# fgnt/pb_chime5

Measured on AMD Instinct MI355X. Metric: utterance-seconds enhanced/sec/GPU (24ch, 20 EM iters), higher is better.
Workload: dtype f64

## Files before the change

### pb_chime5_amd/csrc/cacgmm.hip

```cpp
#include <algorithm>
#include <cmath>
#include <cstdlib>

#include "gss_internal.h"
#include "dense_wave.h"
#include "jacobi.h"

namespace {

#ifndef GSS_CHOL_PRIO
#define GSS_CHOL_PRIO 1
#endif
#ifndef GSS_ESTEP_PRIO
#define GSS_ESTEP_PRIO 1
#endif
constexpr int EM_TILE = 64;
constexpr int EM_TS = EM_TILE + 1;

enum { MODE_FIRST = 0, MODE_EM = 1, MODE_PREDICT = 2 };

__device__ __forceinline__ void set_progress_priority(int done, int total) {
    const int q4 = 4 * done / total;
    if (q4 <= 0) __builtin_amdgcn_s_setprio(3);
    else if (q4 == 1) __builtin_amdgcn_s_setprio(2);
    else if (q4 == 2) __builtin_amdgcn_s_setprio(1);
    else __builtin_amdgcn_s_setprio(0);
}

struct MsegPlan {
    int S, ntile, base, rem, maxseg;
};
__host__ __device__ __forceinline__ int mseg_begin(const MsegPlan &p, int slot) {
    return slot * p.base + (slot < p.rem ? slot : p.rem);
}
__host__ __device__ __forceinline__ int mseg_slot_of(const MsegPlan &p, int item) {
    const int head = p.rem * (p.base + 1);
    return item < head ? item / (p.base + 1) : p.rem + (item - head) / p.base;
}
__host__ __device__ __forceinline__ int mseg_count(const MsegPlan &p, int f) {
    return mseg_slot_of(p, f * p.ntile + p.ntile - 1) - mseg_slot_of(p, f * p.ntile) + 1;
}

struct EmArgs {
    const cplx *Y;
    const uint8_t *act;
    int64_t act_stride, act_fstride;
    const double *init;
    int64_t init_stride, init_fstride;
    const double *logdet;
    const double *pi;
    double *W;
    cplx *Bp;
    double *Sg;
    double *gamma;
    int64_t T;
    int F, D, NE, nch, chunk_frames;
    int masked;
    double aff_eps;
    MsegPlan mseg;
};

template <bool NORMALISE, int NV = 8>
__device__ __forceinline__ void load_tile(const cplx *Yf, int D, int64_t t0, int64_t c1, int tl,
                                          int g, cplx *ys, double *scratch) {
    const int tid = g * EM_TILE + tl;
    const int nfr = (int)min((int64_t)EM_TILE, c1 - t0);
    const int total = nfr * D;
    const cplx *src = Yf + t0 * D;
    const int qf = 256 / D, rf = 256 - qf * D;
    cplx v[NV];
#pragma unroll
    for (int j = 0; j < NV; ++j) {
        const int idx = tid + 256 * j;
        v[j] = idx < total ? src[idx] : c_make(0.0, 0.0);
    }
    {
        int fr = tid / D, d = tid - fr * D;
#pragma unroll
        for (int j = 0; j < NV; ++j) {
            if (tid + 256 * j < EM_TILE * D) ys[d * EM_TS + fr] = v[j];
            fr += qf;
            d += rf;
            if (d >= D) {
                d -= D;
                ++fr;
            }
        }
    }
    if (NORMALISE) {
        __syncthreads();
        double nrm = 0.0;
#pragma unroll
        for (int j = 0; j < NV; ++j) {
            const int d = g + 4 * j;
            nrm += d < D ? c_abs2(ys[d * EM_TS + tl]) : 0.0;
        }
        scratch[g * EM_TILE + tl] = nrm;
        __syncthreads();
        nrm = scratch[tl] + scratch[EM_TILE + tl] + scratch[2 * EM_TILE + tl] +
              scratch[3 * EM_TILE + tl];
        nrm = sqrt(nrm);
        if (nrm < GSS_TINY) nrm = GSS_TINY;
#pragma unroll
        for (int j = 0; j < NV; ++j) {
            const int d = g + 4 * j;
            if (d < D) {
                const cplx y = ys[d * EM_TS + tl];
                ys[d * EM_TS + tl] = c_make(y.x / nrm, y.y / nrm);
            }
        }
    }
}

template <int K, int MODE>
__global__ __launch_bounds__(256) void em_estep_kernel(EmArgs a, const cplx *__restrict__ Mq) {
    extern __shared__ __attribute__((aligned(16))) char smem[];
    const int D = a.D, NE = a.NE;
    cplx *ys = reinterpret_cast<cplx *>(smem);
    double *qpart = reinterpret_cast<double *>(ys + D * EM_TS);
    double *lpS = qpart + 4 * K * EM_TILE;
    double *qqS = lpS + K * EM_TILE;
    double *ldet = qqS + K * EM_TILE;
    double *pis = ldet + K;
    double *vvS = qpart;

    int f, chunk;
    if (!xcd_group_map(a.nch, a.F, f, chunk)) return;
    const int tid = threadIdx.x;
    const int tl = tid & 63;
    const int g = __builtin_amdgcn_readfirstlane(tid >> 6);
    const int64_t T = a.T;
    const int64_t c0 = (int64_t)chunk * a.chunk_frames;
    const int64_t c1 = c0 + a.chunk_frames < T ? c0 + a.chunk_frames : T;
    const cplx *Yf = a.Y + (int64_t)f * T * D;
    const cplx *Mf = Mq + (int64_t)f * NE * K;
    const uint8_t *actf = a.act + (int64_t)f * a.act_fstride;

    if (MODE != MODE_FIRST && tid < K) {
        ldet[tid] = a.logdet[f * K + tid];
        pis[tid] = a.pi[f * K + tid];
    }
    constexpr int NS = (K + 3) / 4;
    double sg[NS];
#pragma unroll
    for (int s = 0; s < NS; ++s) sg[s] = 0.0;

    for (int64_t t0 = c0; t0 < c1; t0 += EM_TILE) {
        const int64_t t = t0 + tl;
        const bool valid = t < c1;
        if (MODE == MODE_FIRST) {
            if (a.init != nullptr) {
                const double *initf = a.init + (int64_t)f * a.init_fstride;
#pragma unroll
                for (int s = 0; s < NS; ++s) {
                    const int k = g + 4 * s;
                    if (k < K && valid) {
                        const double gk = initf[(int64_t)k * a.init_stride + t];
                        sg[s] += gk;
                        a.W[((int64_t)f * K + k) * T + t] = gk;
                    }
                }
                continue;
            }
            double ssum = 0.0;
#pragma unroll
            for (int k = 0; k < K; ++k)
                ssum += (valid && actf[(int64_t)k * a.act_stride + t]) ? 1.0 : 1e-10;
#pragma unroll
            for (int s = 0; s < NS; ++s) {
                const int k = g + 4 * s;
                if (k < K && valid) {
                    const double v = actf[(int64_t)k * a.act_stride + t] ? 1.0 : 1e-10;
                    const double gk = v / ssum;
                    sg[s] += gk;
                    a.W[((int64_t)f * K + k) * T + t] = gk;
                }
            }
            continue;
        }
        __syncthreads();
        load_tile<true>(Yf, D, t0, c1, tl, g, ys, qpart);
        __syncthreads();

        double q[K];
#pragma unroll
        for (int k = 0; k < K; ++k) q[k] = 0.0;
        const int npairs = (D + 1) / 2;
        for (int p = g; p < npairs; p += 4) {
#pragma unroll 1
            for (int side = 0; side < 2; ++side) {
                const int r = side == 0 ? p : D - 1 - p;
                if (side == 1 && r == p) break;
                const cplx y1 = ys[r * EM_TS + tl];
                const cplx *mrow = Mf + (int64_t)tri_index(r, r, D) * K;
                {
                    const double pr = y1.x * y1.x + y1.y * y1.y;
#pragma unroll
                    for (int k = 0; k < K; ++k) q[k] = fma(mrow[k].x, pr, q[k]);
                }
                for (int d2 = r + 1; d2 < D; ++d2) {
                    mrow += K;
                    const cplx y2 = ys[d2 * EM_TS + tl];
                    const double pr = y1.x * y2.x + y1.y * y2.y;
                    const double pim = y1.y * y2.x - y1.x * y2.y;
#pragma unroll
                    for (int k = 0; k < K; ++k) {
                        const cplx m = mrow[k];
                        q[k] = fma(m.x, pr, q[k]);
                        q[k] = fma(m.y, pim, q[k]);
                    }
                }
            }
        }
#pragma unroll
        for (int k = 0; k < K; ++k) qpart[(g * K + k) * EM_TILE + tl] = q[k];
        __syncthreads();
        double myq[NS];
#pragma unroll
        for (int s = 0; s < NS; ++s) myq[s] = 1.0;
#pragma unroll
        for (int s = 0; s < NS; ++s) {
            const int k = g + 4 * s;
            if (k < K) {
                double qv = qpart[k * EM_TILE + tl] + qpart[(K + k) * EM_TILE + tl] +
                            qpart[(2 * K + k) * EM_TILE + tl] + qpart[(3 * K + k) * EM_TILE + tl];
                qv = fmax(fabs(qv), GSS_TINY);
                myq[s] = qv;
                lpS[k * EM_TILE + tl] = -(double)D * log(qv) - ldet[k];
            }
        }
        __syncthreads();
        double mx = -INFINITY;
#pragma unroll
        for (int k = 0; k < K; ++k) mx = fmax(mx, lpS[k * EM_TILE + tl]);
#pragma unroll
        for (int s = 0; s < NS; ++s) {
            const int k = g + 4 * s;
            if (k < K) {
                double v = exp(lpS[k * EM_TILE + tl] - mx) * pis[k];
                if (a.masked) v *= (valid && actf[(int64_t)k * a.act_stride + t]) ? 1.0 : 0.0;
                vvS[k * EM_TILE + tl] = v;
            }
        }
        __syncthreads();
        double ssum = 0.0;
#pragma unroll
        for (int k = 0; k < K; ++k) ssum += vvS[k * EM_TILE + tl];
        ssum = fmax(ssum, GSS_TINY);
#pragma unroll
        for (int s = 0; s < NS; ++s) {
            const int k = g + 4 * s;
            if (k < K && valid) {
                double gam = vvS[k * EM_TILE + tl] / ssum;
                if (a.aff_eps != 0.0) gam = fmin(fmax(gam, a.aff_eps), 1.0 - a.aff_eps);
                if (MODE == MODE_PREDICT) {
                    a.gamma[((int64_t)f * K + k) * T + t] = gam;
                } else {
                    sg[s] += gam;
                    a.W[((int64_t)f * K + k) * T + t] = gam / fmax(myq[s], 10.0 * GSS_TINY);
                }
            }
        }
    }
    if (MODE == MODE_PREDICT) return;
#pragma unroll
    for (int s = 0; s < NS; ++s) {
        const int k = g + 4 * s;
        const double tot = wave_sum(sg[s]);
        if (k < K && tl == 0) a.Sg[((int64_t)f * a.nch + chunk) * K + k] = tot;
    }
}

template <int NV>
__global__ __launch_bounds__(256) void em_prepare_kernel(const cplx *__restrict__ Y, int F,
                                                         int64_t T, int D,
                                                         cplx *__restrict__ Yn,
                                                         int *__restrict__ zero_tiles) {
    extern __shared__ __attribute__((aligned(16))) char smem[];
    cplx *ys = reinterpret_cast<cplx *>(smem);
    double *scratch = reinterpret_cast<double *>(ys + D * EM_TS);
    int f, tile;
    const int ntile = (int)((T + EM_TILE - 1) / EM_TILE);
    if (!xcd_group_map(ntile, F, f, tile)) return;
    const int tid = threadIdx.x, tl = tid & 63, g = tid >> 6;
    const int64_t t0 = (int64_t)tile * EM_TILE;
    load_tile<true, NV>(Y + (int64_t)f * T * D, D, t0, T, tl, g, ys, scratch);
    __syncthreads();
    const int64_t t = t0 + tl;
    bool nonzero = false;
    if (t < T)
        for (int d = g; d < D; d += 4) {
            const cplx v = ys[d * EM_TS + tl];
            Yn[((int64_t)f * D + d) * T + t] = v;
            nonzero = nonzero || v.x != 0.0 || v.y != 0.0;
        }
    scratch[g * EM_TILE + tl] = nonzero ? 1.0 : 0.0;
    __syncthreads();
    const bool zero_frame = t < T && g == 0 &&
                            scratch[tl] + scratch[EM_TILE + tl] + scratch[2 * EM_TILE + tl] +
                                    scratch[3 * EM_TILE + tl] == 0.0;
    const int any_zero = __syncthreads_or(zero_frame ? 1 : 0);
    if (tid == 0) zero_tiles[(int64_t)f * ntile + tile] = any_zero;
}

__device__ __forceinline__ bool frequency_has_zero_frames(const int *__restrict__ zero_tiles,
                                                          int ntile, int f, int lane) {
    int z = 0;
    for (int i = lane; i < ntile; i += 64) z |= zero_tiles[(int64_t)f * ntile + i];
    return __any(z != 0);
}

template <int K, int D, int MODE>
__global__ __launch_bounds__(256) void em_estep_reg_kernel(EmArgs a, const cplx *__restrict__ Mq,
                                                           const cplx *__restrict__ Yn) {
    constexpr int NE = D * (D + 1) / 2;
    const int64_t T = a.T;
    const int wpb = blockDim.x >> 6;
    const int ntile = (int)((T + 64 * wpb - 1) / (64 * wpb));
    int f, tile;
    if (!xcd_group_map(ntile, a.F, f, tile)) return;
    const int lane = threadIdx.x & 63;
    const int wave = __builtin_amdgcn_readfirstlane(threadIdx.x >> 6);
    const int64_t t = ((int64_t)tile * wpb + wave) * 64 + lane;
    const bool valid = t < T;
    const int64_t tc = valid ? t : T - 1;
    const cplx *Mf = Mq + (int64_t)f * NE * K;
    const cplx *yf = Yn + (int64_t)f * D * T + tc;

#if GSS_ESTEP_PRIO
    __builtin_amdgcn_s_setprio(3);
#endif
    cplx y[D];
#pragma unroll
    for (int d = 0; d < D; ++d) y[d] = yf[(int64_t)d * T];

    double q[K];
#pragma unroll
    for (int k = 0; k < K; ++k) q[k] = 0.0;
    constexpr int P = 2, RING = P + 1;
    cplx ring[RING][K];
#pragma unroll
    for (int j = 0; j < P; ++j)
#pragma unroll
        for (int k = 0; k < K; ++k) ring[j][k] = Mf[j * K + k];
    int e = 0;
#pragma unroll
    for (int d1 = 0; d1 < D; ++d1) {
#pragma unroll
        for (int d2 = d1; d2 < D; ++d2) {
            if (e + P < NE) {
#pragma unroll
                for (int k = 0; k < K; ++k) ring[(e + P) % RING][k] = Mf[(e + P) * K + k];
            }
            const double pr = y[d1].x * y[d2].x + y[d1].y * y[d2].y;
            if (d1 == d2) {
#pragma unroll
                for (int k = 0; k < K; ++k) q[k] = fma(ring[e % RING][k].x, pr, q[k]);
            } else {
                const double pim = y[d1].y * y[d2].x - y[d1].x * y[d2].y;
#pragma unroll
                for (int k = 0; k < K; ++k) {
                    const cplx m = ring[e % RING][k];
                    q[k] = fma(m.x, pr, q[k]);
                    q[k] = fma(m.y, pim, q[k]);
                }
            }
            __builtin_amdgcn_sched_barrier(0);
            ++e;
#if GSS_ESTEP_PRIO
            if (e == NE / 4) __builtin_amdgcn_s_setprio(2);
            if (e == NE / 2) __builtin_amdgcn_s_setprio(1);
            if (e == 3 * NE / 4) __builtin_amdgcn_s_setprio(0);
#endif
        }
    }
    const int dep = q[0] != q[0] ? 1 : 0;
    const int tcl = (int)tc - dep;
    auto lane_bcast = [](double x, int k) {
        const unsigned long long u = __double_as_longlong(x);
        const unsigned lo = __builtin_amdgcn_readlane((int)(unsigned)u, k);
        const unsigned hi = __builtin_amdgcn_readlane((int)(unsigned)(u >> 32), k);
        return __longlong_as_double(((unsigned long long)hi << 32) | lo);
    };
    double cls, ldl, pil;
    {
        const int kk = (lane < K ? lane : K - 1) - (lane > 0 ? dep : 0);
        ldl = a.logdet[f * K + kk];
        pil = a.pi[f * K + kk];
        double ldmin = INFINITY;
#pragma unroll
        for (int k = 0; k < K; ++k) ldmin = fmin(ldmin, lane_bcast(ldl, k));
        cls = pil * exp(ldmin - ldl);
    }
    double qmin = INFINITY;
#pragma unroll
    for (int k = 0; k < K; ++k) {
        q[k] = fmax(fabs(q[k]), GSS_TINY);
        qmin = fmin(qmin, q[k]);
    }
    uint8_t act[K];
#pragma unroll
    for (int k = 0; k < K; ++k)
        act[k] = a.act[(int64_t)f * a.act_fstride + (int64_t)k * a.act_stride + (tcl < 0 ? 0 : tcl)];
    double v[K], iq[K], ssum = 0.0;
#pragma unroll
    for (int k = 0; k < K; ++k) {
        iq[k] = 1.0 / q[k];
        const double r = qmin * iq[k];
        double p = 1.0, b = r;
#pragma unroll
        for (int bit = D; bit > 0; bit >>= 1) {
            if (bit & 1) p = p * b;
            b = b * b;
        }
        v[k] = p * lane_bcast(cls, k);
        v[k] = (!a.masked || (valid && act[k])) ? v[k] : 0.0;
        ssum += v[k];
    }
    if (ssum < 1e-280) {
        double lp[K], mx = -INFINITY;
        ssum = 0.0;
#pragma unroll
        for (int k = 0; k < K; ++k) {
            lp[k] = -(double)D * log(q[k]) - lane_bcast(ldl, k);
            mx = fmax(mx, lp[k]);
        }
#pragma unroll
        for (int k = 0; k < K; ++k) {
            v[k] = exp(lp[k] - mx) * lane_bcast(pil, k);
            v[k] = (!a.masked || (valid && act[k])) ? v[k] : 0.0;
            ssum += v[k];
        }
    }
    const double is = 1.0 / fmax(ssum, GSS_TINY);
#pragma unroll
    for (int k = 0; k < K; ++k) {
        double gam = v[k] * is;
        if (a.aff_eps != 0.0) gam = fmin(fmax(gam, a.aff_eps), 1.0 - a.aff_eps);
        if (MODE == MODE_PREDICT) {
            if (valid) a.gamma[((int64_t)f * K + k) * T + t] = gam;
        } else {
            if (valid)
                a.W[((int64_t)f * K + k) * T + t] =
                    gam * (q[k] < 10.0 * GSS_TINY ? 1.0 / (10.0 * GSS_TINY) : iq[k]);
            const double tot = wave_sum(valid ? gam : 0.0);
            if (lane == 0) a.Sg[(((int64_t)f * ntile + tile) * wpb + wave) * K + k] = tot;
        }
    }
}

struct WcovLds {
    int Dp, nblk, nfg, red_groups;
    size_t ys, wk, scratch, blk, total;
};

__host__ __device__ inline WcovLds wcov_lds_layout(int D, int KW) {
    WcovLds L;
    L.Dp = D + (D & 1);
    const int nb2 = L.Dp / 2;
    L.nblk = nb2 * (nb2 + 1) / 2;
    int nfg = 256 / L.nblk;
    if (nfg > EM_TILE) nfg = EM_TILE;
    if (nfg < 1) nfg = 1;
    L.nfg = nfg;
    size_t off = 0;
    const size_t ys_bytes = sizeof(cplx) * (size_t)L.Dp * EM_TS;
    const size_t group_bytes = sizeof(cplx) * (size_t)L.nblk * 4 * KW;
    int rg = (int)((32 * 1024) / group_bytes);
    if (rg > nfg - 1) rg = nfg - 1;
    if (rg < 1) rg = 1;
    L.red_groups = rg;
    const size_t red_bytes = group_bytes * rg;
    L.ys = off;
    off += ys_bytes > red_bytes ? ys_bytes : red_bytes;
    L.wk = off;      off += sizeof(double) * KW * EM_TILE;
    L.scratch = off; off += sizeof(double) * 4 * EM_TILE;
    L.blk = off;     off += 2 * (size_t)L.nblk;
    L.total = (off + 15) / 16 * 16;
    return L;
}

#ifdef GSS_WCOV_TRACE
__device__ long long g_wcov_phase[8192 * 6];
extern "C" int gss_debug_wcov_phase(long long *host, int entries) {
    return (int)hipMemcpyFromSymbol(host, HIP_SYMBOL(g_wcov_phase), sizeof(long long) * 6 * entries);
}
#define WCOV_T(var) const long long var = __builtin_readcyclecounter()
#else
#define WCOV_T(var)
#endif

template <int KW, bool NORMALISE, bool SRC_FDT, bool PREFETCH = false, int YP = 8, bool YEXACT = false>
__global__ __launch_bounds__(256) void wcov_kernel(const cplx *__restrict__ Y,
                                                   const double *__restrict__ W, int F,
                                                   int64_t T, int D, int NE, int nch,
                                                   int chunk_frames, cplx *__restrict__ part,
                                                   int Ktot, int k0, MsegPlan plan) {
    extern __shared__ __attribute__((aligned(16))) char smem[];
    const WcovLds L = wcov_lds_layout(D, KW);
    const int Dp = L.Dp;
    cplx *ys = reinterpret_cast<cplx *>(smem + L.ys);
    double *wk = reinterpret_cast<double *>(smem + L.wk);
    double *scratch = reinterpret_cast<double *>(smem + L.scratch);
    unsigned char *blk = reinterpret_cast<unsigned char *>(smem + L.blk);

    int f = 0, chunk = 0, item = 0, item_end = 1;
    if (plan.S > 0) {
        item = mseg_begin(plan, blockIdx.x);
        item_end = mseg_begin(plan, blockIdx.x + 1);
    }
    const int item_begin = item;
    if (plan.S > 0) {
    } else if (!xcd_group_map(nch, F, f, chunk)) {
        return;
    }
    W += (int64_t)blockIdx.y * F * Ktot * T;
    part += (int64_t)blockIdx.y * F * nch * Ktot * NE;
    const int tid = threadIdx.x;
    const int tl = tid & 63, g = tid >> 6;
#ifdef GSS_WCOV_TRACE
    long long tr_stage = 0, tr_acc = 0;
    const long long tr_wall0 = __builtin_amdgcn_s_memrealtime();
#endif
    WCOV_T(tr_c0);
#ifdef GSS_WCOV_TRACE
    long long tr_red = 0;
#endif

    {
        const int nb2 = Dp / 2;
        for (int bi = tid; bi < nb2; bi += blockDim.x) {
            int idx = bi * nb2 - (bi * (bi - 1)) / 2;
            for (int bj = bi; bj < nb2; ++bj, ++idx) {
                blk[2 * idx] = (unsigned char)bi;
                blk[2 * idx + 1] = (unsigned char)bj;
            }
        }
    }
    const int mb = tid % L.nblk, fg = tid / L.nblk;
    const bool m_active = fg < L.nfg;
  for (bool first_seg = true; item < item_end; first_seg = false) {
    if (Dp != D) {
        if (!first_seg) __syncthreads();
        for (int j = tid; j < EM_TS; j += blockDim.x) ys[D * EM_TS + j] = c_make(0.0, 0.0);
    }
    int64_t c0, c1;
    int nch_f = nch;
    if (plan.S > 0) {
        f = item / plan.ntile;
        const int tile0 = item - f * plan.ntile;
        const int ntl = min(plan.ntile - tile0, item_end - item);
        c0 = (int64_t)tile0 * EM_TILE;
        c1 = min(T, (int64_t)(tile0 + ntl) * EM_TILE);
        chunk = (int)blockIdx.x - mseg_slot_of(plan, f * plan.ntile);
        nch_f = plan.maxseg;
        item += ntl;
    } else {
        c0 = (int64_t)chunk * chunk_frames;
        c1 = c0 + chunk_frames < T ? c0 + chunk_frames : T;
        item = item_end;
    }
    const cplx *Yf = Y + (int64_t)f * T * D;
    const double *Wf = W + ((int64_t)f * Ktot + k0) * T;
    cplx acc[4][KW];
#pragma unroll
    for (int s = 0; s < 4; ++s)
#pragma unroll
        for (int k = 0; k < KW; ++k) acc[s][k] = c_make(0.0, 0.0);

    constexpr int WPRE = (KW * EM_TILE + 255) / 256;
    cplx ypre[YP];
    double wpre[WPRE];
    auto prefetch = [&](int64_t t0) {
        const cplx *src = Y + (int64_t)f * D * T;
#pragma unroll
        for (int j = 0; j < YP; ++j) {
            const int d = g + 4 * j;
            ypre[j] = ((YEXACT || d < D) && t0 + tl < c1) ? src[(int64_t)d * T + t0 + tl] : c_make(0.0, 0.0);
        }
#pragma unroll
        for (int j = 0; j < WPRE; ++j) {
            const int idx = tid + 256 * j;
            const int k = idx / EM_TILE, jj = idx - k * EM_TILE;
            wpre[j] = (idx < KW * EM_TILE && t0 + jj < c1) ? Wf[(int64_t)k * T + t0 + jj] : 0.0;
        }
    };
    if (SRC_FDT && PREFETCH) prefetch(c0);
    for (int64_t t0 = c0; t0 < c1; t0 += EM_TILE) {
        WCOV_T(tr_a);
        if (plan.S > 0) {
            set_progress_priority(item - (int)((c1 - t0 + EM_TILE - 1) / EM_TILE) - item_begin,
                                  item_end - item_begin);
        }
        __syncthreads();
        if (SRC_FDT) {
            if (!PREFETCH) prefetch(t0);
#pragma unroll
            for (int j = 0; j < YP; ++j) {
                const int d = g + 4 * j;
                if (YEXACT || d < D) ys[d * EM_TS + tl] = ypre[j];
            }
#pragma unroll
            for (int j = 0; j < WPRE; ++j) {
                const int idx = tid + 256 * j;
                if (idx < KW * EM_TILE) wk[idx] = wpre[j];
            }
            __syncthreads();
            if (PREFETCH && t0 + EM_TILE < c1) prefetch(t0 + EM_TILE);
        } else {
            load_tile<NORMALISE, YP>(Yf, D, t0, c1, tl, g, ys, scratch);
            for (int idx = tid; idx < KW * EM_TILE; idx += blockDim.x) {
                const int k = idx / EM_TILE, j = idx - k * EM_TILE;
                wk[idx] = t0 + j < c1 ? Wf[(int64_t)k * T + t0 + j] : 0.0;
            }
            __syncthreads();
        }
        WCOV_T(tr_b);
        if (m_active) {
            const int nfr = (int)min((int64_t)EM_TILE, c1 - t0);
            const int bi = blk[2 * mb], bj = blk[2 * mb + 1];
            const cplx *ra0 = ys + (2 * bi) * EM_TS, *ra1 = ra0 + EM_TS;
            const cplx *rb0 = ys + (2 * bj) * EM_TS, *rb1 = rb0 + EM_TS;
            for (int j = fg; j < nfr; j += L.nfg) {
                const cplx a0 = ra0[j], a1 = ra1[j], b0 = rb0[j], b1 = rb1[j];
                double pr[4], pim[4];
                pr[0] = a0.x * b0.x + a0.y * b0.y;  pim[0] = a0.y * b0.x - a0.x * b0.y;
                pr[1] = a0.x * b1.x + a0.y * b1.y;  pim[1] = a0.y * b1.x - a0.x * b1.y;
                pr[2] = a1.x * b0.x + a1.y * b0.y;  pim[2] = a1.y * b0.x - a1.x * b0.y;
                pr[3] = a1.x * b1.x + a1.y * b1.y;  pim[3] = a1.y * b1.x - a1.x * b1.y;
#pragma unroll
                for (int k = 0; k < KW; ++k) {
                    const double w = wk[k * EM_TILE + j];
#pragma unroll
                    for (int s = 0; s < 4; ++s) {
                        acc[s][k].x = fma(w, pr[s], acc[s][k].x);
                        acc[s][k].y = fma(w, pim[s], acc[s][k].y);
                    }
                }
            }
        }
#ifdef GSS_WCOV_TRACE
        {
            WCOV_T(tr_c);
            tr_stage += tr_b - tr_a;
            tr_acc += tr_c - tr_b;
        }
#endif
    }
    WCOV_T(tr_c1);
    cplx *red = reinterpret_cast<cplx *>(smem + L.ys);
    const int gstride = L.nblk * 4 * KW;
    for (int r0 = 1; r0 < L.nfg; r0 += L.red_groups) {
        __syncthreads();
        if (m_active && fg >= r0 && fg < r0 + L.red_groups) {
            cplx *dst = red + (size_t)(fg - r0) * gstride;
#pragma unroll
            for (int s = 0; s < 4; ++s)
#pragma unroll
                for (int k = 0; k < KW; ++k) dst[(mb * 4 + s) * KW + k] = acc[s][k];
        }
        __syncthreads();
        if (fg == 0) {
            for (int r = r0; r < r0 + L.red_groups && r < L.nfg; ++r) {
                const cplx *src = red + (size_t)(r - r0) * gstride;
#pragma unroll
                for (int s = 0; s < 4; ++s)
#pragma unroll
                    for (int k = 0; k < KW; ++k)
                        acc[s][k] = c_add(acc[s][k], src[(mb * 4 + s) * KW + k]);
            }
        }
    }
    if (fg == 0) {
        cplx *pp = part + (((int64_t)f * nch_f + chunk) * Ktot + k0) * NE;
        const int bi = blk[2 * mb], bj = blk[2 * mb + 1];
#pragma unroll
        for (int s = 0; s < 4; ++s) {
            const int d1 = 2 * bi + (s >> 1), d2 = 2 * bj + (s & 1);
            if (d1 <= d2 && d2 < D) {
                const int e = tri_index(d1, d2, D);
#pragma unroll
                for (int k = 0; k < KW; ++k) pp[k * NE + e] = acc[s][k];
            }
        }
    }
#ifdef GSS_WCOV_TRACE
    {
        WCOV_T(tr_c2s);
        tr_red += tr_c2s - tr_c1;
    }
#endif
  }
#ifdef GSS_WCOV_TRACE
    {
        WCOV_T(tr_c2);
        if (tid == 0 && blockIdx.x < 8192) {
            long long *o = g_wcov_phase + 6 * blockIdx.x;
            o[0] = tr_wall0;
            o[1] = __builtin_amdgcn_s_memrealtime();
            o[2] = tr_stage;
            o[3] = tr_acc;
            o[4] = tr_red;
            o[5] = tr_c2 - tr_c0;
        }
    }
#endif
}

template <int K, int D>
__global__ __launch_bounds__(64) void mstep_reg_kernel(const cplx *__restrict__ Yn,
                                                       const double *__restrict__ W, int F,
                                                       int64_t T, int nch, int chunk_frames,
                                                       cplx *__restrict__ part) {
    constexpr int NE = D * (D + 1) / 2;
    int f, chunk;
    if (!xcd_group_map(nch, F, f, chunk)) return;
    const int lane = threadIdx.x;
    const int64_t c0 = (int64_t)chunk * chunk_frames;
    const int64_t c1 = c0 + chunk_frames < T ? c0 + chunk_frames : T;
    const cplx *yf = Yn + (int64_t)f * D * T;
    const double *wf = W + (int64_t)f * K * T;

    double are[K][NE], aim[K][NE];
#pragma unroll
    for (int k = 0; k < K; ++k)
#pragma unroll
        for (int e = 0; e < NE; ++e) are[k][e] = aim[k][e] = 0.0;

    cplx y[D], yn[D];
    double w[K], wn[K];
    auto fetch = [&](int64_t t, cplx (&yy)[D], double (&ww)[K]) {
        const bool ok = t < c1;
        const int64_t tc = ok ? t : c1 - 1;
#pragma unroll
        for (int d = 0; d < D; ++d) yy[d] = yf[(int64_t)d * T + tc];
#pragma unroll
        for (int k = 0; k < K; ++k) ww[k] = ok ? wf[(int64_t)k * T + tc] : 0.0;
    };
    fetch(c0 + lane, yn, wn);
    for (int64_t tb = c0; tb < c1; tb += 64) {
#pragma unroll
        for (int d = 0; d < D; ++d) y[d] = yn[d];
#pragma unroll
        for (int k = 0; k < K; ++k) w[k] = wn[k];
        if (tb + 64 < c1) fetch(tb + 64 + lane, yn, wn);
        int e = 0;
#pragma unroll
        for (int d1 = 0; d1 < D; ++d1) {
#pragma unroll
            for (int d2 = d1; d2 < D; ++d2, ++e) {
                const double pr = y[d1].x * y[d2].x + y[d1].y * y[d2].y;
#pragma unroll
                for (int k = 0; k < K; ++k) are[k][e] = fma(w[k], pr, are[k][e]);
                if (d2 != d1) {
                    const double pim = y[d1].y * y[d2].x - y[d1].x * y[d2].y;
#pragma unroll
                    for (int k = 0; k < K; ++k) aim[k][e] = fma(w[k], pim, aim[k][e]);
                }
            }
        }
    }
// ... 679 lines not shown
                }
            }
#ifdef GSS_EM4_TRACE
            {
                EM4_T(c_e);
                EM4_ADD(0, c_b - c_a);
                EM4_ADD(2, c_d - c_b);
                EM4_ADD(3, c_e - c_d);
            }
#endif
        }
        if (predict) break;
        EM4_T(c_f);

#pragma unroll
        for (int k = 0; k < K; ++k) {
            const double tot = quad_sum(acc[k]);
            if (msl == 0) (&ldsS[wave][0][0])[k * NP + mi] = tot;
            const double g = wave_sum(sg[k]);
            if (lane == 0) sgS[wave][k] = g;
        }
        __syncthreads();
        static_assert(K * NP <= 2 * OC_LD, "the wave sums fit the first rows");
        if (tid < K * NP) {
            const int k = tid / NP;
            const double sgk = (sgS[0][k] + sgS[1][k]) + (sgS[2][k] + sgS[3][k]);
            const double tot = ((&ldsS[0][0][0])[tid] + (&ldsS[1][0][0])[tid]) +
                               ((&ldsS[2][0][0])[tid] + (&ldsS[3][0][0])[tid]);
            bS[k][tid % NP] = ((double)D * tot) / fmax(sgk, GSS_TINY);
        }
        if (tid == 0) flagS = 0;
        __syncthreads();
        EM4_T(c_u0);
        if (wave == 0 && lane < K) {
            const int k = lane;
            const double sgk = (sgS[0][k] + sgS[1][k]) + (sgS[2][k] + sgS[3][k]);
            piS[k] = sgk / (double)T;
            double b[NP], m[NP], ld;
#pragma unroll
            for (int i = 0; i < NP; ++i) b[i] = bS[k][i];
            const bool fast = class_update4_lane(b, a.eig_floor, m, ld) && !force_exact;
            if (fast) {
#pragma unroll
                for (int i = 0; i < NP; ++i) mR[i][k] = m[i];
                logdetS[k] = ld;
            } else {
                atomicOr(&flagS, 1 << k);
            }
        }
#ifdef GSS_EM4_TRACE
        {
            EM4_T(c_u1);
            EM4_ADD(1, c_u1 - c_u0);
        }
#endif
        __syncthreads();
        if (flagS != 0) {
            const int flags = flagS;
            for (int k = wave; k < K; k += 4) {
                if (!(flags >> k & 1)) continue;
                cplx vals[COV_SLOTS];
#pragma unroll
                for (int s2 = 0; s2 < COV_SLOTS; ++s2) vals[s2] = c_make(0.0, 0.0);
                int d1 = 0, d2 = 0;
                if (lane < NE) {
                    const int p = ts.d12[0];
                    d1 = p >> 8, d2 = p & 255;
                    if (d1 == d2) {
                        vals[0] = c_make(bS[k][d1], 0.0);
                    } else {
                        const int off = lane - d1 - 1;
                        vals[0] = c_make(bS[k][D + off], bS[k][D + 6 + off]);
                    }
                }
                cplx *A = reinterpret_cast<cplx *>(&ldsS[wave][0][0]);
                cplx *basis = A + 80;
                cplx *basis_g = a.basis + ((int64_t)f * K + k) * 16;
                if (!a.cold_eigh && basis_validS[k] && lane < 16) basis[lane] = basis_g[lane];
                wave_sync();
                class_update_eigh(vals, D, K, a.eig_floor, A, lane, MqS + k, logdetS + k, ts,
                                  a.cold_eigh ? nullptr : basis, basis_validS + k);
                if (!a.cold_eigh && lane < 16) basis_g[lane] = basis[lane];
                wave_sync();
                if (lane < NE) {
                    const cplx v = MqS[lane * K + k];
                    if (d1 == d2) {
                        mR[d1][k] = v.x;
                    } else {
                        mR[D + lane - d1 - 1][k] = v.x;
                        mR[D + 6 + lane - d1 - 1][k] = v.y;
                    }
                }
            }
            __syncthreads();
        }
        if (tid < K) {
            double ldmin = INFINITY;
            for (int k = 0; k < K; ++k) ldmin = fmin(ldmin, logdetS[k]);
            cS[tid] = piS[tid] * exp(ldmin - logdetS[tid]);
        }
        __syncthreads();
#ifdef GSS_EM4_TRACE
        {
            EM4_T(c_g);
            EM4_ADD(4, c_g - c_f);
        }
#endif
    }
#ifdef GSS_EM4_TRACE
    {
        EM4_T(c_end);
        EM4_ADD(5, c_end - c_start);
        if (tid == 0 && blockIdx.x < 1024)
            for (int i = 0; i < 6; ++i) g_em4_phase[blockIdx.x * 6 + i] = em4_acc[i];
    }
#endif
}

template <int K>
int launch_onchip4(gss_ctx *ctx, const OnchipArgs &a) {
    GSS_PROF(ctx, "em_onchip");
    hipLaunchKernelGGL(em_onchip4_kernel<K>, dim3(a.F), dim3(256), 0, ctx->stream, a);
    GSS_LAUNCH_CHECK(ctx, "em_onchip4_kernel");
    return GSS_OK;
}

size_t em_estep_lds(int D, int K) {
    size_t b = sizeof(cplx) * (size_t)D * EM_TS;
    b += sizeof(double) * ((size_t)4 * K * EM_TILE + 2 * (size_t)K * EM_TILE + 2 * K);
    return (b + 15) / 16 * 16;
}

int em_chunks(int F, int64_t T, int D, int *chunk_frames) {
    int64_t tiles = (T + EM_TILE - 1) / EM_TILE;
    const int forced = gss_variant("em_wgs", 0);
    const int target = forced > 0 ? forced : (D <= 12 ? 1536 : 3072);
    int64_t want = (target + F - 1) / F;
    if (want < 1) want = 1;
    int64_t tiles_per_chunk = (tiles + want - 1) / want;
    if (tiles_per_chunk < 1) tiles_per_chunk = 1;
    *chunk_frames = (int)(tiles_per_chunk * EM_TILE);
    return (int)((tiles + tiles_per_chunk - 1) / tiles_per_chunk);
}

template <typename Kern>
int raise_lds_limit(gss_ctx *ctx, Kern kern, size_t lds) {
    if (lds > 64 * 1024)
        GSS_HIP_CHECK(ctx, hipFuncSetAttribute(reinterpret_cast<const void *>(kern),
                                               hipFuncAttributeMaxDynamicSharedMemorySize,
                                               (int)lds));
    return GSS_OK;
}

template <int K>
int launch_estep(gss_ctx *ctx, int mode, const EmArgs &a, const cplx *Mq, int F) {
    const size_t lds = em_estep_lds(a.D, K);
    dim3 grid(xcd_grid(a.nch, F)), block(256);
    if (mode == MODE_FIRST) {
        GSS_PROF(ctx, "em_estep");
        hipLaunchKernelGGL((em_estep_kernel<K, MODE_FIRST>), grid, block, 0, ctx->stream, a, Mq);
    } else if (mode == MODE_EM) {
        GSS_TRY(raise_lds_limit(ctx, em_estep_kernel<K, MODE_EM>, lds));
        GSS_PROF(ctx, "em_estep");
        hipLaunchKernelGGL((em_estep_kernel<K, MODE_EM>), grid, block, lds, ctx->stream, a, Mq);
    } else {
        GSS_TRY(raise_lds_limit(ctx, em_estep_kernel<K, MODE_PREDICT>, lds));
        GSS_PROF(ctx, "em_predict");
        hipLaunchKernelGGL((em_estep_kernel<K, MODE_PREDICT>), grid, block, lds, ctx->stream, a,
                           Mq);
    }
    GSS_LAUNCH_CHECK(ctx, "em_estep_kernel");
    return GSS_OK;
}

int estep_waves_per_block(int F, int64_t T) {
    auto eff = [&](int wpb) {
        const double wgs = (double)((T + 64 * wpb - 1) / (64 * wpb)) * F;
        const double rounds = wgs / (256.0 * (16 / wpb));
        return rounds / std::ceil(rounds);
    };
    const int forced = gss_variant("estep_wpb", 0);
    if (forced == 1 || forced == 4) return forced;
    return eff(1) > eff(4) ? 1 : 4;
}

template <int K, int D>
int launch_estep_reg(gss_ctx *ctx, int mode, const EmArgs &a, const cplx *Mq, const cplx *Yn,
                     int F) {
    const int wpb = estep_waves_per_block(F, a.T);
    const dim3 grid(xcd_grid((int)((a.T + 64 * wpb - 1) / (64 * wpb)), F)), block(64 * wpb);
    if (mode == MODE_EM) {
        GSS_PROF(ctx, "em_estep");
        hipLaunchKernelGGL((em_estep_reg_kernel<K, D, MODE_EM>), grid, block, 0, ctx->stream, a,
                           Mq, Yn);
    } else {
        GSS_PROF(ctx, "em_predict");
        hipLaunchKernelGGL((em_estep_reg_kernel<K, D, MODE_PREDICT>), grid, block, 0, ctx->stream,
                           a, Mq, Yn);
    }
    GSS_LAUNCH_CHECK(ctx, "em_estep_reg_kernel");
    return GSS_OK;
}

bool estep_reg_supported(int D, int K) {
    return (D == 24 || D == 20 || D == 12 || D == 10 || D == 4) && K >= 2 && K <= 6;
}

template <int D>
int launch_estep_reg_k(gss_ctx *ctx, int K, int mode, const EmArgs &a, const cplx *Mq,
                       const cplx *Yn, int F) {
    switch (K) {
        case 2: return launch_estep_reg<2, D>(ctx, mode, a, Mq, Yn, F);
        case 3: return launch_estep_reg<3, D>(ctx, mode, a, Mq, Yn, F);
        case 4: return launch_estep_reg<4, D>(ctx, mode, a, Mq, Yn, F);
        case 5: return launch_estep_reg<5, D>(ctx, mode, a, Mq, Yn, F);
        case 6: return launch_estep_reg<6, D>(ctx, mode, a, Mq, Yn, F);
    }
    return gss_fail(ctx, GSS_ERR_UNSUPPORTED, "cacgmm: K=%d", K);
}

static int mstep_prefetch_max_d();
using wcov_fn_t = void (*)(const cplx *, const double *, int, int64_t, int, int, int, int, cplx *, int,
                           int, MsegPlan);
template <int KW>
wcov_fn_t mstep_kernel(int D) {
    const bool generic = gss_variant_set("mstep_generic");
    if (D <= mstep_prefetch_max_d()) {
        if (D == 12 && !generic) return wcov_kernel<KW, false, true, true, 3, true>;
        if (D <= 12 && !generic) return wcov_kernel<KW, false, true, true, 3>;
        return wcov_kernel<KW, false, true, true>;
    }
    if (D == 24 && !generic) return wcov_kernel<KW, false, true, false, 6, true>;
    if (D == 20 && !generic) return wcov_kernel<KW, false, true, false, 5, true>;
    return wcov_kernel<KW, false, true>;
}

template <int KW>
int mstep_resident_slots(gss_ctx *ctx, int D, int *slots) {
    const size_t lds = wcov_lds_layout(D, KW).total;
    const void *fn = reinterpret_cast<const void *>(mstep_kernel<KW>(D));
    if (lds > 64 * 1024)
        GSS_HIP_CHECK(ctx, hipFuncSetAttribute(fn, hipFuncAttributeMaxDynamicSharedMemorySize, (int)lds));
    int per_cu = 0, cus = 0;
    GSS_HIP_CHECK(ctx, hipOccupancyMaxActiveBlocksPerMultiprocessor(&per_cu, fn, 256, lds));
    GSS_HIP_CHECK(ctx, hipDeviceGetAttribute(&cus, hipDeviceAttributeMultiprocessorCount, ctx->device));
    *slots = std::max(per_cu, 1) * cus;
    return GSS_OK;
}
static int mstep_prefetch_max_d() {
    const int v = gss_variant("mstep_prefetch_d", 12);
    return v;
}

template <int KW>
int launch_mstep(gss_ctx *ctx, const EmArgs &a, const cplx *Yn, int F, int K, int k0) {
    const size_t lds = wcov_lds_layout(a.D, KW).total;
    GSS_PROF(ctx, "em_mstep");
    if (Yn && a.D == 4 && KW == K && K >= 2 && K <= 6 && !gss_variant_set("mstep_tiled")) {
        hipLaunchKernelGGL((mstep_reg_kernel<(KW >= 2 && KW <= 6 ? KW : 2), 4>),
                           dim3(xcd_grid(a.nch, F)), dim3(64), 0, ctx->stream, Yn, a.W, F, a.T,
                           a.nch, a.chunk_frames, a.Bp);
        GSS_LAUNCH_CHECK(ctx, "mstep_reg_kernel");
        return GSS_OK;
    }
    if (Yn) {
        const wcov_fn_t fn = mstep_kernel<KW>(a.D);
        GSS_TRY(raise_lds_limit(ctx, fn, lds));
        hipLaunchKernelGGL(fn, dim3(a.mseg.S > 0 ? a.mseg.S : xcd_grid(a.nch, F)), dim3(256), lds,
                           ctx->stream, Yn, a.W, F, a.T, a.D, a.NE, a.nch, a.chunk_frames, a.Bp, K, k0,
                           a.mseg);
        GSS_LAUNCH_CHECK(ctx, "wcov_kernel");
        return GSS_OK;
    }
    GSS_TRY(raise_lds_limit(ctx, wcov_kernel<KW, true, false>, lds));
    hipLaunchKernelGGL((wcov_kernel<KW, true, false>), dim3(xcd_grid(a.nch, F)), dim3(256), lds,
                       ctx->stream, a.Y, a.W, F, a.T, a.D, a.NE, a.nch, a.chunk_frames, a.Bp, K, k0,
                       MsegPlan{});
    GSS_LAUNCH_CHECK(ctx, "wcov_kernel");
    return GSS_OK;
}

#define GSS_K_CASE(N, CALL) case N: { constexpr int KK = N; return CALL; }
#define GSS_K_SWITCH8(K, CALL)                                             \
    switch (K) {                                                           \
        GSS_K_CASE(1, CALL) GSS_K_CASE(2, CALL) GSS_K_CASE(3, CALL) GSS_K_CASE(4, CALL)     \
        GSS_K_CASE(5, CALL) GSS_K_CASE(6, CALL) GSS_K_CASE(7, CALL) GSS_K_CASE(8, CALL)     \
    }
#define GSS_K_SWITCH19(K, CALL)                                            \
    switch (K) {                                                           \
        GSS_K_CASE(1, CALL) GSS_K_CASE(2, CALL) GSS_K_CASE(3, CALL) GSS_K_CASE(4, CALL)     \
        GSS_K_CASE(5, CALL) GSS_K_CASE(6, CALL) GSS_K_CASE(7, CALL) GSS_K_CASE(8, CALL)     \
        GSS_K_CASE(9, CALL) GSS_K_CASE(10, CALL) GSS_K_CASE(11, CALL) GSS_K_CASE(12, CALL) \
        GSS_K_CASE(13, CALL) GSS_K_CASE(14, CALL) GSS_K_CASE(15, CALL) GSS_K_CASE(16, CALL) \
        GSS_K_CASE(17, CALL) GSS_K_CASE(18, CALL) GSS_K_CASE(19, CALL)                     \
    }

int launch_estep_k(gss_ctx *ctx, int K, int mode, const EmArgs &a, const cplx *Mq, int F) {
    GSS_K_SWITCH19(K, launch_estep<KK>(ctx, mode, a, Mq, F));
    return gss_fail(ctx, GSS_ERR_UNSUPPORTED, "cacgmm: K=%d", K);
}

int launch_mstep_group(gss_ctx *ctx, int KW, const EmArgs &a, const cplx *Yn, int F, int K,
                       int k0) {
    GSS_K_SWITCH8(KW, launch_mstep<KK>(ctx, a, Yn, F, K, k0));
    return gss_fail(ctx, GSS_ERR_UNSUPPORTED, "cacgmm: class group of %d", KW);
}

int launch_mstep_k(gss_ctx *ctx, int K, const EmArgs &a, const cplx *Yn, int F) {
    const int ngroups = (K + 7) / 8, per = (K + ngroups - 1) / ngroups;
    for (int k0 = 0; k0 < K; k0 += per)
        GSS_TRY(launch_mstep_group(ctx, std::min(per, K - k0), a, Yn, F, K, k0));
    return GSS_OK;
}

int mstep_resident_slots_k(gss_ctx *ctx, int KW, int D, int *slots) {
    GSS_K_SWITCH8(KW, mstep_resident_slots<KK>(ctx, D, slots));
    return gss_fail(ctx, GSS_ERR_UNSUPPORTED, "cacgmm: KW=%d", KW);
}

static int mstep_maxseg_limit() { return std::min(std::max(gss_variant("mstep_maxseg", 8), 1), 32); }

int mstep_plan(gss_ctx *ctx, int F, int64_t T, int D, int K, MsegPlan *plan) {
    *plan = MsegPlan{};
    const int min_d = gss_variant("mstep_plan_min_d", 5);
    if (D < min_d || D <= 4 || gss_variant_set("mstep_chunked")) return GSS_OK;
    const int ngroups = (K + 7) / 8, per = (K + ngroups - 1) / ngroups;
    int slots = 0;
    GSS_TRY(mstep_resident_slots_k(ctx, per, D, &slots));
    if (gss_variant("mstep_slots", 0) > 0) slots = gss_variant("mstep_slots", 0);
    const int64_t ntile = (T + EM_TILE - 1) / EM_TILE, N = ntile * F;
    if (N >= (1LL << 30) || ntile < 1) return GSS_OK;
    plan->ntile = (int)ntile;
    plan->S = (int)std::min<int64_t>(slots, N);
    plan->base = (int)(N / plan->S);
    plan->rem = (int)(N % plan->S);
    for (int f = 0; f < F; ++f) plan->maxseg = std::max(plan->maxseg, mseg_count(*plan, f));
    if (plan->maxseg > mstep_maxseg_limit()) *plan = MsegPlan{};
    return GSS_OK;
}


struct EmBlockPlan {
    int fb, nblocks, streams;
};
EmBlockPlan em_block_plan(int F, int64_t T, int D, int K) {
    EmBlockPlan p{F, 1, 1};
    const double per_f = (16.0 * D + 8.0 * K) * (double)T;
    const double mb = 1024.0 * 1024.0;
    const int fit = gss_variant("em_l3_fit_mb", 230), budget = gss_variant("em_l3_mb", 0);
    if (budget <= 0 || F <= 8 || per_f * F <= fit * mb) return p;
    p.streams = gss_variant("em_streams", 2) >= 2 ? 2 : 1;
    int fb = (int)(budget * mb / p.streams / per_f) / 8 * 8;
    if (fb < 8) fb = 8;
    int nb = (F + fb - 1) / fb;
    if (p.streams == 2 && (nb & 1)) ++nb;
    fb = ((F + nb - 1) / nb + 7) / 8 * 8;
    nb = (F + fb - 1) / fb;
    if (nb <= 1) return EmBlockPlan{F, 1, 1};
    p.fb = fb;
    p.nblocks = nb;
    return p;
}
int em_block_size(const EmBlockPlan &p, int F, int b) { return std::min(p.fb, F - b * p.fb); }

struct EmStrides {
    int nch, bp_nch, reg_nch;
};
EmStrides em_strides(const EmBlockPlan &p, int F, int64_t T, int D) {
    EmStrides s{0, 0, 0};
    for (int b : {0, p.nblocks - 1}) {
        const int Fb = em_block_size(p, F, b);
        int cf;
        const int nch = em_chunks(Fb, T, D, &cf);
        const int wpb = estep_waves_per_block(Fb, T);
        s.nch = std::max(s.nch, nch);
        s.reg_nch = std::max(s.reg_nch, wpb * (int)((T + 64 * wpb - 1) / (64 * wpb)));
    }
    s.bp_nch = std::max(s.nch, mstep_maxseg_limit());
    return s;
}

}

int psd_partials_run(gss_ctx *ctx, const cplx *Y, int F, int64_t T, int D, const double *W2,
                     int nch, int chunk_frames, cplx *part, int S) {
    const size_t lds = wcov_lds_layout(D, 2).total;
    const wcov_fn_t fn = D <= 4 ? wcov_kernel<2, false, false, false, 1>
                         : D <= 12 ? wcov_kernel<2, false, false, false, 3>
                         : D <= 24 ? wcov_kernel<2, false, false, false, 6> : wcov_kernel<2, false, false>;
    GSS_TRY(raise_lds_limit(ctx, fn, lds));
    hipLaunchKernelGGL(fn, dim3(xcd_grid(nch, F), S), dim3(256), lds,
                       ctx->stream, Y, W2, F, T, D, tri_count(D), nch, chunk_frames, part, 2, 0,
                       MsegPlan{});
    GSS_LAUNCH_CHECK(ctx, "wcov_kernel");
    return GSS_OK;
}

size_t cacgmm_workspace_bytes(int F, int64_t T, int D, int K) {
    const size_t NE = tri_count(D);
    const EmBlockPlan bp = em_block_plan(F, T, D, K);
    const EmStrides st = em_strides(bp, F, T, D);
    size_t b = 0;
    b += align_up(sizeof(cplx) * (size_t)F * NE * K);
    b += 2 * align_up(sizeof(double) * (size_t)F * K);
    b += align_up(sizeof(double) * (size_t)F * K * T);
    b += align_up(sizeof(cplx) * (size_t)F * st.bp_nch * K * NE);
    b += align_up(sizeof(double) * (size_t)F * st.nch * K);
    b += align_up(sizeof(int) * (size_t)F * K);
    b += align_up(sizeof(int) * 2 * NE);
    b += align_up(sizeof(cplx) * (size_t)F * D * T);
    b += align_up(sizeof(double) * (size_t)F * st.reg_nch * K);
    b += align_up(sizeof(cplx) * (size_t)F * K * 16);
    b += align_up(sizeof(int) * (size_t)F * ((T + EM_TILE - 1) / EM_TILE));
    return b + 4096;
}

namespace {
struct EmBlock {
    EmArgs a;
    int F;
    cplx *Mq, *Yn;
    int *need_eigh, *zero_tiles;
    double *Sg_lds, *Sg_reg;
    int nch_lds, reg_nch, bp_nch, sg_nch;
    hipStream_t stream;
};
struct StreamRestore {
    gss_ctx *ctx;
    hipStream_t s;
    ~StreamRestore() { ctx->stream = s; }
};
}

int cacgmm_run(gss_ctx *ctx, const cplx *Y, int F, int64_t T, int D, const EmGuide &guide, int K,
               int iterations, int iterations_post, double *gamma) {
    const int NE = tri_count(D);
    const bool reg = estep_reg_supported(D, K) && !gss_variant_set("estep_lds");
    const bool onchip = D == 4 && K >= 2 && K <= 6 && reg && iterations > 0 &&
                        !gss_variant_set("em_unfused");
    const EmBlockPlan bplan = onchip ? EmBlockPlan{F, 1, 1} : em_block_plan(F, T, D, K);
    const EmStrides st = em_strides(bplan, F, T, D);

    cplx *Mq = arena_alloc_t<cplx>(ctx, (size_t)F * NE * K);
    double *logdet = arena_alloc_t<double>(ctx, (size_t)F * K);
    double *pi = arena_alloc_t<double>(ctx, (size_t)F * K);
    double *W = arena_alloc_t<double>(ctx, (size_t)F * K * T);
    cplx *Bp = arena_alloc_t<cplx>(ctx, (size_t)F * st.bp_nch * K * NE);
    double *Sg_lds = arena_alloc_t<double>(ctx, (size_t)F * st.nch * K);
    cplx *Yn = arena_alloc_t<cplx>(ctx, (size_t)F * D * T);
    double *Sg_reg = arena_alloc_t<double>(ctx, (size_t)F * st.reg_nch * K);
    int *need_eigh = arena_alloc_t<int>(ctx, (size_t)F * K);
    const int ntile = (int)((T + EM_TILE - 1) / EM_TILE);
    int *zero_tiles = arena_alloc_t<int>(ctx, (size_t)F * ntile);
    int *tri_tab = arena_alloc_t<int>(ctx, 2 * (size_t)NE);
    GSS_REQUIRE(ctx, Mq && logdet && pi && W && Bp && Sg_lds && Yn && Sg_reg && need_eigh && tri_tab &&
                         zero_tiles,
                GSS_ERR_NOMEM, "cacgmm workspace");
    GSS_REQUIRE(ctx, em_estep_lds(D, K) <= 160 * 1024 &&
                         wcov_lds_layout(D, std::min(K, 8)).total <= 160 * 1024,
                GSS_ERR_UNSUPPORTED, "cacgmm: D=%d K=%d LDS", D, K);
    const bool has_mask = guide.mask != nullptr;
    const uint8_t *const act = has_mask ? guide.mask : reinterpret_cast<const uint8_t *>(Yn);
    const int64_t act_stride = has_mask ? guide.mask_k_stride : 0;
    const int64_t act_fstride = has_mask ? guide.mask_f_stride : 0;
    const int m = D + (D & 1);
    const size_t eigh_lds = (sizeof(cplx) * 2 * m * m + sizeof(double) * m + 15) / 16 * 16;
    const int force_eigh = gss_variant_set("force_eigh");
    if (!onchip) {
        hipLaunchKernelGGL(tri_table_kernel, dim3(1), dim3(256), 0, ctx->stream, D, tri_tab);
        GSS_LAUNCH_CHECK(ctx, "tri_table_kernel");
    }

    auto make_block = [&](int f0, int Fb, hipStream_t stream, EmBlock *blk) -> int {
        EmBlock &b = *blk;
        b = EmBlock{};
        b.F = Fb;
        b.stream = stream;
        EmArgs &a = b.a;
        a.Y = Y + (int64_t)f0 * T * D;
        a.act = act + (int64_t)f0 * act_fstride;
        a.act_stride = act_stride;
        a.act_fstride = act_fstride;
        a.init = guide.init ? guide.init + (int64_t)f0 * guide.init_f_stride : nullptr;
        a.init_stride = guide.init_k_stride;
        a.init_fstride = guide.init_f_stride;
        a.T = T;
        a.F = Fb;
        a.D = D;
        a.NE = NE;
        a.nch = em_chunks(Fb, T, D, &a.chunk_frames);
        GSS_TRY(mstep_plan(ctx, Fb, T, D, K, &a.mseg));
        b.bp_nch = a.mseg.S > 0 ? a.mseg.maxseg : a.nch;
        b.nch_lds = a.nch;
        const int wpb = estep_waves_per_block(Fb, T);
        b.reg_nch = wpb * (int)((T + 64 * wpb - 1) / (64 * wpb));
        GSS_REQUIRE(ctx, b.bp_nch <= st.bp_nch && b.nch_lds <= st.nch && b.reg_nch <= st.reg_nch,
                    GSS_ERR_INVALID, "cacgmm: block strides");
        b.Mq = Mq + (int64_t)f0 * NE * K;
        a.logdet = logdet + (int64_t)f0 * K;
        a.pi = pi + (int64_t)f0 * K;
        a.W = W + (int64_t)f0 * K * T;
        a.Bp = Bp + (int64_t)f0 * st.bp_nch * K * NE;
        b.Sg_lds = Sg_lds + (int64_t)f0 * st.nch * K;
        b.Sg_reg = Sg_reg + (int64_t)f0 * st.reg_nch * K;
        a.Sg = b.Sg_lds;
        a.gamma = gamma + (int64_t)f0 * K * T;
        b.Yn = Yn + (int64_t)f0 * D * T;
        b.need_eigh = need_eigh + (int64_t)f0 * K;
        b.zero_tiles = zero_tiles + (int64_t)f0 * ntile;
        b.sg_nch = b.nch_lds;
        return GSS_OK;
    };
    auto prepare = [&](EmBlock &b) -> int {
        GSS_PROF(ctx, "em_prepare");
        const size_t plds = sizeof(cplx) * (size_t)D * EM_TS + sizeof(double) * 4 * EM_TILE;
        const auto prep = D <= 4 ? em_prepare_kernel<1> : D <= 12 ? em_prepare_kernel<3>
                          : D <= 24 ? em_prepare_kernel<6> : em_prepare_kernel<8>;
        hipLaunchKernelGGL(prep,
                           dim3(xcd_grid((int)((T + EM_TILE - 1) / EM_TILE), b.F)), dim3(256), plds,
                           ctx->stream, b.a.Y, b.F, T, D, b.Yn, b.zero_tiles);
        GSS_LAUNCH_CHECK(ctx, "em_prepare_kernel");
        return GSS_OK;
    };
    auto estep = [&](EmBlock &b, int mode) -> int {
        EmArgs &a = b.a;
        if (reg && mode != MODE_FIRST) {
            a.Sg = b.Sg_reg;
            switch (D) {
                case 24: return launch_estep_reg_k<24>(ctx, K, mode, a, b.Mq, b.Yn, b.F);
                case 20: return launch_estep_reg_k<20>(ctx, K, mode, a, b.Mq, b.Yn, b.F);
                case 12: return launch_estep_reg_k<12>(ctx, K, mode, a, b.Mq, b.Yn, b.F);
                case 10: return launch_estep_reg_k<10>(ctx, K, mode, a, b.Mq, b.Yn, b.F);
                default: return launch_estep_reg_k<4>(ctx, K, mode, a, b.Mq, b.Yn, b.F);
            }
        }
        a.Sg = b.Sg_lds;
        return launch_estep_k(ctx, K, mode, a, b.Mq, b.F);
    };
    auto eig = [&](EmBlock &b) -> int {
        EmArgs &a = b.a;
        {
            GSS_PROF(ctx, "em_chol");
            const int nr = (D + 7) / 8;
            const size_t lds = sizeof(cplx) * (size_t)D * (8 * nr + 1) + sizeof(double) * D;
            auto kern = nr <= 1 ? em_chol_kernel<1> : nr == 2 ? em_chol_kernel<2>
                        : nr == 3 ? em_chol_kernel<3> : em_chol_kernel<4>;
            hipLaunchKernelGGL(kern, dim3(K, b.F), dim3(64), lds, ctx->stream, a.Bp, a.Sg, b.bp_nch,
                               b.sg_nch, D, K, T, 1e-10, force_eigh, b.Mq,
                               const_cast<double *>(a.logdet), const_cast<double *>(a.pi),
                               b.need_eigh, tri_tab, a.mseg, b.zero_tiles, ntile);
            GSS_LAUNCH_CHECK(ctx, "em_chol_kernel");
        }
        {
            GSS_PROF(ctx, "em_eigh");
            hipLaunchKernelGGL(em_eigh_kernel, dim3(K, b.F), dim3(64), eigh_lds, ctx->stream, a.Bp,
                               a.Sg, b.bp_nch, b.sg_nch, D, K, 1e-10, b.need_eigh, b.Mq,
                               const_cast<double *>(a.logdet), tri_tab, a.mseg);
            GSS_LAUNCH_CHECK(ctx, "em_eigh_kernel");
        }
        return GSS_OK;
    };

    if (onchip) {
        EmBlock b;
        GSS_TRY(make_block(0, F, ctx->stream, &b));
        GSS_TRY(prepare(b));
        OnchipArgs o{};
        o.basis = arena_alloc_t<cplx>(ctx, (size_t)F * K * 16);
        GSS_REQUIRE(ctx, o.basis, GSS_ERR_NOMEM, "cacgmm workspace");
        o.Yn = Yn;
        o.act = act;
        o.act_stride = act_stride;
        o.act_fstride = act_fstride;
        o.init = guide.init;
        o.init_stride = guide.init_k_stride;
        o.init_fstride = guide.init_f_stride;
        o.unmasked = has_mask ? 0 : 1;
        o.T = T;
        o.F = F;
        o.iterations = iterations;
        o.iterations_post = iterations_post;
        o.force_eigh = force_eigh;
        o.zero_tiles = b.zero_tiles;
        o.ntile = ntile;
        o.cold_eigh = gss_variant_set("em4_cold_eigh");
        o.eig_floor = 1e-10;
        o.gamma = gamma;
        switch (K) {
            case 2: return launch_onchip4<2>(ctx, o);
            case 3: return launch_onchip4<3>(ctx, o);
            case 4: return launch_onchip4<4>(ctx, o);
            case 5: return launch_onchip4<5>(ctx, o);
            default: return launch_onchip4<6>(ctx, o);
        }
    }

    auto em_iteration = [&](EmBlock &b, bool first) -> int {
        GSS_TRY(estep(b, first ? MODE_FIRST : MODE_EM));
        b.sg_nch = (reg && !first) ? b.reg_nch : b.nch_lds;
        GSS_TRY(launch_mstep_k(ctx, K, b.a, b.Yn, b.F));
        return eig(b);
    };

    hipStream_t const main_stream = ctx->stream;
    StreamRestore restore{ctx, main_stream};
    const int group = bplan.streams;
    if (group > 1) {
        GSS_TRY(aux_stream_ready(ctx));
        GSS_HIP_CHECK(ctx, hipEventRecord(ctx->ev_fork, main_stream));
        GSS_HIP_CHECK(ctx, hipStreamWaitEvent(ctx->aux_stream, ctx->ev_fork, 0));
    }
    for (int b0 = 0; b0 < bplan.nblocks; b0 += group) {
        EmBlock blk[2];
        const int nb = std::min(group, bplan.nblocks - b0);
        for (int j = 0; j < nb; ++j)
            GSS_TRY(make_block((b0 + j) * bplan.fb, em_block_size(bplan, F, b0 + j),
                               j == 0 ? main_stream : ctx->aux_stream, &blk[j]));
        auto each = [&](auto &&fn) -> int {
            for (int j = 0; j < nb; ++j) {
                ctx->stream = blk[j].stream;
                GSS_TRY(fn(blk[j]));
            }
            return GSS_OK;
        };
        GSS_TRY(each([&](EmBlock &b) { return prepare(b); }));
        for (int it = 0; it < iterations; ++it)
            GSS_TRY(each([&](EmBlock &b) {
                b.a.masked = has_mask ? 1 : 0;
                b.a.aff_eps = 1e-10;
                return em_iteration(b, it == 0);
            }));
        for (int it = 0; it < iterations_post - 1; ++it)
            GSS_TRY(each([&](EmBlock &b) {
                b.a.masked = 0;
                b.a.aff_eps = 1e-10;
                return em_iteration(b, false);
            }));
        GSS_TRY(each([&](EmBlock &b) {
            b.a.masked = has_mask && iterations_post == 0 ? 1 : 0;
// ... 12 lines not shown
```

### pb_chime5_amd/csrc/gss_api.hip

```cpp
#include <cmath>
#include <cstdarg>
#include <cstdlib>
#include <cstring>
#include <mutex>

#include "gss_internal.h"

#define GSS_ENTER(ctx)                                   \
    if (!(ctx)) return GSS_ERR_INVALID;                  \
    GSS_HIP_CHECK((ctx), hipSetDevice((ctx)->device))
#define GSS_ENTER_VARIANTS(ctx) \
    GSS_ENTER(ctx);             \
    GSS_TRY(variant_refresh(ctx))
static int variant_refresh(gss_ctx *ctx);

static std::mutex g_error_lock;

int gss_fail(gss_ctx *ctx, int code, const char *fmt, ...) {
    char buf[1024];
    va_list ap;
    va_start(ap, fmt);
    vsnprintf(buf, sizeof(buf), fmt, ap);
    va_end(ap);
    if (ctx) {
        std::lock_guard<std::mutex> guard(g_error_lock);
        ctx->error = buf;
    }
    return code;
}

static thread_local std::string g_create_error;

namespace {
const char *const kVariantKeys[] = {
    "corr_ts", "corr_nw", "corr_blocked", "corr_p_tiles", "chol_diag_unfolded", "apply_ph",
    "apply_generic", "prof_detail", "corr_stg8", "corr_ksplit", "apply_gglobal", "wpe_halves",
    "em_wgs", "estep_wpb", "estep_lds", "mstep_prefetch_d", "mstep_tiled", "mstep_plan_min_d",
    "mstep_chunked", "mstep_slots", "force_eigh", "em_unfused", "em_l3_mb", "em_l3_fit_mb",
    "em_streams", "mstep_maxseg", "em4_cold_eigh", "mstep_generic"};
struct VariantTable {
    std::mutex lock;
    std::string text;
    bool parsed = false;
    std::map<std::string, int> values;
};
VariantTable &variant_table() {
    static VariantTable t;
    return t;
}
}

static int variant_refresh(gss_ctx *ctx) {
    const char *env = getenv("GSS_VARIANT");
    VariantTable &t = variant_table();
    std::lock_guard<std::mutex> guard(t.lock);
    if (t.parsed && t.text == (env ? env : "")) return GSS_OK;
    t.text = env ? env : "";
    t.parsed = true;
    t.values.clear();
    std::string unknown;
    size_t pos = 0;
    while (pos < t.text.size()) {
        size_t end = t.text.find_first_of(", ", pos);
        if (end == std::string::npos) end = t.text.size();
        const std::string tok = t.text.substr(pos, end - pos);
        pos = end + 1;
        if (tok.empty()) continue;
        const size_t eq = tok.find('=');
        const std::string name = tok.substr(0, eq);
        bool known = false;
        for (const char *k : kVariantKeys) known = known || name == k;
        if (!known) {
            unknown = name;
            continue;
        }
        t.values[name] = eq == std::string::npos ? 1 : atoi(tok.c_str() + eq + 1);
    }
    if (!unknown.empty()) {
        t.values.clear();
        t.parsed = false;
        return gss_fail(ctx, GSS_ERR_INVALID, "GSS_VARIANT names no switch '%s'", unknown.c_str());
    }
    return GSS_OK;
}

int gss_variant(const char *key, int dflt) {
    VariantTable &t = variant_table();
    std::lock_guard<std::mutex> guard(t.lock);
    const auto it = t.values.find(key);
    return it == t.values.end() ? dflt : it->second;
}

extern "C" const char *gss_last_error(gss_ctx *ctx) {
    if (!ctx) return g_create_error.c_str();
    static thread_local std::string copy;
    std::lock_guard<std::mutex> guard(g_error_lock);
    copy = ctx->error;
    return copy.c_str();
}

extern "C" const char *gss_version(void) {
#ifdef GSS_EXPERIMENT_BUILD
    return "pb_chime5_amd/libgss_hip 0.4 EXPERIMENT BUILD (gfx950, f64)";
#else
    return "pb_chime5_amd/libgss_hip 0.4 (gfx950, f64)";
#endif
}

extern "C" int gss_abi_version(void) { return GSS_ABI_VERSION; }

extern "C" int gss_device_count(void) {
    int count = 0;
    if (hipGetDeviceCount(&count) != hipSuccess) return 0;
    return count;
}

extern "C" int gss_device_pci_bus_id(int device_id, char *buf, int len) {
    if (!buf || len < 16) return GSS_ERR_INVALID;
    buf[0] = 0;
    int count = 0;
    if (hipGetDeviceCount(&count) != hipSuccess || device_id < 0 || device_id >= count)
        return GSS_ERR_INVALID;
    return hipDeviceGetPCIBusId(buf, len, device_id) == hipSuccess ? GSS_OK : GSS_ERR_HIP;
}

extern "C" int gss_create(int device_id, gss_ctx **out) {
    if (!out) return GSS_ERR_INVALID;
    *out = nullptr;
    int count = 0;
    hipError_t e = hipGetDeviceCount(&count);
    if (e != hipSuccess || count == 0) {
        g_create_error = "no HIP device available: ";
        g_create_error += hipGetErrorString(e);
        return GSS_ERR_HIP;
    }
    if (device_id < 0 || device_id >= count) {
        g_create_error = "device_id out of range";
        return GSS_ERR_INVALID;
    }
    e = hipSetDevice(device_id);
    if (e != hipSuccess) {
        g_create_error = hipGetErrorString(e);
        return GSS_ERR_HIP;
    }
    gss_ctx *ctx = new gss_ctx();
    ctx->device = device_id;
    e = hipStreamCreateWithFlags(&ctx->own_stream, hipStreamNonBlocking);
    if (e != hipSuccess) {
        g_create_error = hipGetErrorString(e);
        delete ctx;
        return GSS_ERR_HIP;
    }
    ctx->stream = ctx->own_stream;
    e = hipHostMalloc(reinterpret_cast<void **>(&ctx->status_host), GSS_STATUS_BYTES,
                      hipHostMallocMapped);
    if (e == hipSuccess)
        e = hipHostGetDevicePointer(reinterpret_cast<void **>(&ctx->status_dev), ctx->status_host, 0);
    if (e != hipSuccess) {
        g_create_error = hipGetErrorString(e);
        (void)hipStreamDestroy(ctx->own_stream);
        delete ctx;
        return GSS_ERR_HIP;
    }
    ctx->status_host[0] = INT32_MIN;
    ctx->status_host[2] = 0;
    *out = ctx;
    return GSS_OK;
}

static void free_tables(gss_ctx *ctx) {
    if (ctx->win_analysis) (void)hipFree(ctx->win_analysis);
    if (ctx->win_synthesis) (void)hipFree(ctx->win_synthesis);
    if (ctx->twiddle) (void)hipFree(ctx->twiddle);
    ctx->win_analysis = ctx->win_synthesis = nullptr;
    ctx->twiddle = nullptr;
}

extern "C" int gss_destroy(gss_ctx *ctx) {
    if (!ctx) return GSS_OK;
    (void)hipSetDevice(ctx->device);
    (void)hipStreamSynchronize(ctx->stream);
    free_tables(ctx);
    if (ctx->arena) (void)hipFree(ctx->arena);
    if (ctx->wpe_tiles) (void)hipFree(ctx->wpe_tiles);
    if (ctx->status_host) (void)hipHostFree(ctx->status_host);
    for (auto &p : ctx->prof_pending) {
        (void)hipEventDestroy(p.start);
        (void)hipEventDestroy(p.stop);
    }
    for (auto ev : ctx->event_pool) (void)hipEventDestroy(ev);
    if (ctx->ev_fork) (void)hipEventDestroy(ctx->ev_fork);
    if (ctx->ev_join) (void)hipEventDestroy(ctx->ev_join);
    if (ctx->aux_stream) {
        (void)hipStreamSynchronize(ctx->aux_stream);
        (void)hipStreamDestroy(ctx->aux_stream);
    }
    if (ctx->own_stream) (void)hipStreamDestroy(ctx->own_stream);
    delete ctx;
    return GSS_OK;
}

int aux_stream_ready(gss_ctx *ctx) {
    if (!ctx->aux_stream)
        GSS_HIP_CHECK(ctx, hipStreamCreateWithFlags(&ctx->aux_stream, hipStreamNonBlocking));
    if (!ctx->ev_fork) GSS_HIP_CHECK(ctx, hipEventCreateWithFlags(&ctx->ev_fork, hipEventDisableTiming));
    if (!ctx->ev_join) GSS_HIP_CHECK(ctx, hipEventCreateWithFlags(&ctx->ev_join, hipEventDisableTiming));
    return GSS_OK;
}

extern "C" int gss_set_stream(gss_ctx *ctx, void *hip_stream) {
    GSS_ENTER(ctx);
    GSS_HIP_CHECK(ctx, hipStreamSynchronize(ctx->stream));
    ctx->stream = hip_stream ? reinterpret_cast<hipStream_t>(hip_stream) : ctx->own_stream;
    return GSS_OK;
}

extern "C" int gss_set_utterances_in_flight(gss_ctx *ctx, int n) {
    if (!ctx) return GSS_ERR_INVALID;
    GSS_REQUIRE(ctx, n >= 0, GSS_ERR_INVALID, "gss_set_utterances_in_flight: n=%d", n);
    ctx->utterances_in_flight = n;
    return GSS_OK;
}

extern "C" int gss_synchronize(gss_ctx *ctx) {
    if (!ctx) return GSS_ERR_INVALID;
    GSS_HIP_CHECK(ctx, hipSetDevice(ctx->device));
    GSS_HIP_CHECK(ctx, hipStreamSynchronize(ctx->stream));
    return GSS_OK;
}

extern "C" int gss_dev_malloc(gss_ctx *ctx, size_t bytes, void **dev_ptr) {
    if (!ctx || !dev_ptr) return GSS_ERR_INVALID;
    GSS_HIP_CHECK(ctx, hipSetDevice(ctx->device));
    *dev_ptr = nullptr;
    if (bytes == 0) bytes = 16;
    hipError_t e = hipMalloc(dev_ptr, bytes);
    if (e != hipSuccess)
        return gss_fail(ctx, GSS_ERR_NOMEM, "hipMalloc(%zu) failed: %s", bytes,
                        hipGetErrorString(e));
    return GSS_OK;
}

extern "C" int gss_dev_free(gss_ctx *ctx, void *dev_ptr) {
    if (!ctx) return GSS_ERR_INVALID;
    if (!dev_ptr) return GSS_OK;
    GSS_HIP_CHECK(ctx, hipSetDevice(ctx->device));
    GSS_HIP_CHECK(ctx, hipStreamSynchronize(ctx->stream));
    GSS_HIP_CHECK(ctx, hipFree(dev_ptr));
    return GSS_OK;
}

extern "C" int gss_memcpy_h2d(gss_ctx *ctx, void *dst, const void *src, size_t bytes) {
    GSS_ENTER(ctx);
    if (bytes == 0) return GSS_OK;
    GSS_HIP_CHECK(ctx, hipMemcpyAsync(dst, src, bytes, hipMemcpyHostToDevice, ctx->stream));
    GSS_HIP_CHECK(ctx, hipStreamSynchronize(ctx->stream));
    return GSS_OK;
}

extern "C" int gss_memcpy_d2h(gss_ctx *ctx, void *dst, const void *src, size_t bytes) {
    GSS_ENTER(ctx);
    if (bytes == 0) return GSS_OK;
    GSS_HIP_CHECK(ctx, hipMemcpyAsync(dst, src, bytes, hipMemcpyDeviceToHost, ctx->stream));
    GSS_HIP_CHECK(ctx, hipStreamSynchronize(ctx->stream));
    return GSS_OK;
}

extern "C" int gss_host_malloc(gss_ctx *ctx, size_t bytes, void **host_ptr) {
    if (!ctx || !host_ptr) return GSS_ERR_INVALID;
    GSS_HIP_CHECK(ctx, hipSetDevice(ctx->device));
    *host_ptr = nullptr;
    if (bytes == 0) bytes = 16;
    hipError_t e = hipHostMalloc(host_ptr, bytes, hipHostMallocDefault);
    if (e != hipSuccess)
        return gss_fail(ctx, GSS_ERR_NOMEM, "hipHostMalloc(%zu) failed: %s", bytes,
                        hipGetErrorString(e));
    return GSS_OK;
}

extern "C" int gss_host_free(gss_ctx *ctx, void *host_ptr) {
    if (!ctx) return GSS_ERR_INVALID;
    if (!host_ptr) return GSS_OK;
    GSS_HIP_CHECK(ctx, hipSetDevice(ctx->device));
    GSS_HIP_CHECK(ctx, hipHostFree(host_ptr));
    return GSS_OK;
}

extern "C" int gss_memcpy_h2d_async(gss_ctx *ctx, void *dst, const void *src, size_t bytes) {
    GSS_ENTER(ctx);
    if (bytes == 0) return GSS_OK;
    GSS_HIP_CHECK(ctx, hipMemcpyAsync(dst, src, bytes, hipMemcpyHostToDevice, ctx->stream));
    return GSS_OK;
}

extern "C" int gss_memcpy_d2h_async(gss_ctx *ctx, void *dst, const void *src, size_t bytes) {
    GSS_ENTER(ctx);
    if (bytes == 0) return GSS_OK;
    GSS_HIP_CHECK(ctx, hipMemcpyAsync(dst, src, bytes, hipMemcpyDeviceToHost, ctx->stream));
    return GSS_OK;
}

extern "C" int gss_memset(gss_ctx *ctx, void *dst, int value, size_t bytes) {
    GSS_ENTER(ctx);
    if (bytes == 0) return GSS_OK;
    GSS_HIP_CHECK(ctx, hipMemsetAsync(dst, value, bytes, ctx->stream));
    return GSS_OK;
}

void arena_reset(gss_ctx *ctx) { ctx->arena_off = 0; }

int arena_reserve(gss_ctx *ctx, size_t bytes) {
    bytes = align_up(bytes + 4096, 1 << 20);
    ctx->arena_off = 0;
    if (bytes <= ctx->arena_size) return GSS_OK;
    GSS_HIP_CHECK(ctx, hipStreamSynchronize(ctx->stream));
    if (ctx->arena) {
        GSS_HIP_CHECK(ctx, hipFree(ctx->arena));
        ctx->arena = nullptr;
        ctx->arena_size = 0;
    }
    hipError_t e = hipMalloc(reinterpret_cast<void **>(&ctx->arena), bytes);
    if (e != hipSuccess)
        return gss_fail(ctx, GSS_ERR_NOMEM, "workspace hipMalloc(%zu) failed: %s", bytes,
                        hipGetErrorString(e));
    ctx->arena_size = bytes;
    return GSS_OK;
}

void *arena_alloc(gss_ctx *ctx, size_t bytes) {
    size_t off = align_up(ctx->arena_off, 256);
    if (off + bytes > ctx->arena_size) return nullptr;
    ctx->arena_off = off + bytes;
    if (ctx->arena_off > ctx->arena_peak) ctx->arena_peak = ctx->arena_off;
    return ctx->arena + off;
}

extern "C" size_t gss_workspace_bytes(gss_ctx *ctx) { return ctx ? ctx->arena_peak : 0; }
// ... 384 lines not shown
                    reinterpret_cast<cplx *>(Xhat), nullptr, 1);
}

extern "C" int gss_selftest_mfma(gss_ctx *ctx) {
    GSS_ENTER(ctx);
    return selftest_mfma_run(ctx);
}

static int check_params(gss_ctx *ctx, const gss_params *p) {
    GSS_REQUIRE(ctx, p, GSS_ERR_INVALID, "params is NULL");
    GSS_REQUIRE(ctx, p->stft_size == ctx->stft_size && p->stft_shift == ctx->stft_shift,
                GSS_ERR_INVALID, "params stft %d/%d differ from gss_set_windows() %d/%d",
                p->stft_size, p->stft_shift, ctx->stft_size, ctx->stft_shift);
    GSS_REQUIRE(ctx, p->bf >= 0 && p->bf <= 3, GSS_ERR_UNSUPPORTED, "bf=%d", p->bf);
    GSS_REQUIRE(ctx, p->postfilter >= 0 && p->postfilter <= 1, GSS_ERR_UNSUPPORTED,
                "postfilter=%d", p->postfilter);
    GSS_REQUIRE(ctx, p->wpe_psd_context >= 0, GSS_ERR_INVALID, "wpe_psd_context=%d",
                p->wpe_psd_context);
    return GSS_OK;
}

static int wpe_arrays_of(const gss_params *p) { return p->wpe_arrays > 1 ? p->wpe_arrays : 1; }

static int check_wpe_arrays(gss_ctx *ctx, const gss_params *p, int D) {
    GSS_REQUIRE(ctx, p->wpe_arrays >= 0 && D % wpe_arrays_of(p) == 0, GSS_ERR_INVALID,
                "wpe_arrays=%d does not divide the %d channels into arrays of equal size",
                p->wpe_arrays, D);
    return GSS_OK;
}

static int pipeline_wpe(gss_ctx *ctx, const gss_params *p, const cplx *Y, int Fv, int64_t T,
                        int Dv, cplx *X) {
    const int array_bins = wpe_arrays_of(p) > 1 ? Fv : 0;
    const int halves = gss_variant("wpe_halves", ctx->utterances_in_flight == 1 ? 1 : 0);
    if (!(halves > 0 && Fv >= 32 && p->wpe_iterations > 0))
        return wpe_run(ctx, Y, Fv, T, Dv, p->wpe_taps, p->wpe_delay, p->wpe_iterations,
                       p->wpe_psd_context, X, -1, array_bins);
    GSS_TRY(aux_stream_ready(ctx));
    hipStream_t const main_stream = ctx->stream;
    const int F0 = halves > 1 ? std::min(halves * 8, Fv - 8) : (Fv / 2 + 7) / 8 * 8, F1 = Fv - F0;
    const size_t off = (size_t)F0 * T * Dv;
    int st = wpe_run(ctx, Y, F0, T, Dv, p->wpe_taps, p->wpe_delay, p->wpe_iterations,
                     p->wpe_psd_context, X, 0, array_bins);
    if (st == GSS_OK) {
        GSS_HIP_CHECK(ctx, hipStreamWaitEvent(ctx->aux_stream, ctx->ev_fork, 0));
        ctx->stream = ctx->aux_stream;
        st = wpe_run(ctx, Y + off, F1, T, Dv, p->wpe_taps, p->wpe_delay, p->wpe_iterations,
                     p->wpe_psd_context, X + off, 1, array_bins);
        ctx->stream = main_stream;
        GSS_HIP_CHECK(ctx, hipEventRecord(ctx->ev_join, ctx->aux_stream));
        GSS_HIP_CHECK(ctx, hipStreamWaitEvent(main_stream, ctx->ev_join, 0));
    }
    GSS_TRY(st);
    return wpe_copy_zero_pivots(ctx);
}

static size_t front_buffer_bytes(int F, int64_t T, int64_t T_act, int D, int K) {
    size_t b = 0;
    size_t ftd = align_up(sizeof(cplx) * (size_t)F * T * D);
    b += 2 * ftd;
    b += align_up((size_t)K * T_act);
    b += align_up(sizeof(double) * (size_t)F * K * T);
    return b;
}

static size_t front_stage_bytes(const gss_params *p, int F, int64_t T, int D, int K) {
    const int A = wpe_arrays_of(p);
    size_t stage = 0;
    if (p->wpe)
        stage = std::max(stage, wpe_workspace_bytes(F * A, T, D / A, p->wpe_taps, p->wpe_delay) + (1 << 16));
    stage = std::max(stage, cacgmm_workspace_bytes(F, T, D, K));
    return stage;
}

static size_t pipeline_workspace(const gss_params *p, int F, int64_t T, int64_t T_act, int D,
                                 int K) {
    size_t b = front_buffer_bytes(F, T, T_act, D, K);
    b += 2 * align_up(sizeof(double) * (size_t)F * T);
    b += align_up(sizeof(cplx) * (size_t)F * T);
    b += 4096;
    size_t stage = front_stage_bytes(p, F, T, D, K);
    stage = std::max(stage, mvdr_workspace_bytes(F, T, D));
    stage = std::max(stage, stft_workspace_bytes(T, p->stft_size));
    return b + stage + (1 << 16);
}

static size_t targets_workspace(const gss_params *p, int F, int64_t T, int64_t T_act, int D,
                                int K, int S) {
    size_t b = front_buffer_bytes(F, T, T_act, D, K);
    b += 2 * align_up(sizeof(double) * (size_t)S * F * T);
    b += align_up(sizeof(cplx) * (size_t)S * F * T);
    b += align_up(sizeof(int32_t) * 4 * (size_t)S);
    b += 4096;
    size_t stage = front_stage_bytes(p, F, T, D, K);
    stage = std::max(stage, mvdr_workspace_bytes(F, T, D, S));
    stage = std::max(stage, align_up(sizeof(cplx) * (size_t)F * T) + 4096);
    stage = std::max(stage, stft_workspace_bytes((int64_t)S * T, p->stft_size));
    return b + stage + (1 << 16);
}

static int check_pipeline_front(gss_ctx *ctx, const gss_params *p, const void *obs, int D,
                                int64_t N, const void *act, const void *out, const char *what) {
    GSS_TRY(check_windows(ctx));
    GSS_TRY(check_params(ctx, p));
    GSS_REQUIRE(ctx, obs && act && out && N >= 1, GSS_ERR_INVALID, "%s: bad arguments", what);
    GSS_REQUIRE(ctx, D >= 1 && D <= GSS_MAX_CHANNELS, GSS_ERR_UNSUPPORTED, "D=%d", D);
    return GSS_OK;
}

static int check_pipeline_rest(gss_ctx *ctx, const gss_params *p, int D, int64_t N, int K,
                               int64_t N_act, int64_t *T_out, int64_t *T_act_out) {
    GSS_TRY(check_cacgmm_args(ctx, D, K, p->bss_iterations, p->bss_iterations_post));
    if (p->wpe) GSS_TRY(check_wpe_arrays(ctx, p, D));
    if (p->bf == 0 || p->bf == 3)
        GSS_REQUIRE(ctx, D < 30, GSS_ERR_INVALID, "assert D < 30 failed: D=%d", D);
    if (p->bf == 1)
        GSS_REQUIRE(ctx, D > 2, GSS_ERR_INVALID, "bf='ch2' needs more than 2 channels");

    const int size = p->stft_size, shift = p->stft_shift, fading = p->stft_fading;
    const int F = size / 2 + 1;
    const int64_t T = gss_stft_num_frames(N, size, shift, fading);
    const int64_t T_act = gss_stft_num_frames(N_act, size, shift, fading);
    GSS_REQUIRE(ctx, T_act >= T, GSS_ERR_INVALID,
                "activity covers %lld frames but the observation has %lld",
                (long long)T_act, (long long)T);

    GSS_REQUIRE(ctx, (int64_t)F * T * D < (1LL << 31), GSS_ERR_UNSUPPORTED,
                "F * T * D = %lld STFT bins: 2^31 or more are not supported (some kernels index "
                "the tensor with 32 bits)", (long long)((int64_t)F * T * D));
    *T_out = T;
    *T_act_out = T_act;
    return GSS_OK;
}

struct PipelineFront {
    cplx *Y, *X;
    uint8_t *actf;
    double *gamma;
};

static int alloc_front(gss_ctx *ctx, const gss_params *p, int F, int64_t T, int64_t T_act, int D,
                       int K, PipelineFront *fr) {
    fr->Y = arena_alloc_t<cplx>(ctx, (size_t)F * T * D);
    fr->X = p->wpe ? arena_alloc_t<cplx>(ctx, (size_t)F * T * D) : fr->Y;
    fr->actf = arena_alloc_t<uint8_t>(ctx, (size_t)K * T_act);
    fr->gamma = arena_alloc_t<double>(ctx, (size_t)F * K * T);
    GSS_REQUIRE(ctx, fr->Y && fr->X && fr->actf && fr->gamma, GSS_ERR_NOMEM, "workspace sizing bug");
    return GSS_OK;
}

static int run_front(gss_ctx *ctx, const gss_params *p, const void *obs, int obs_type, int D,
                     int64_t N, const uint8_t *act, int K, int64_t N_act, int F, int64_t T,
                     int64_t T_act, const PipelineFront &fr, size_t mark,
                     const EmGuide *guide = nullptr) {
    cplx *const Y = fr.Y, *const X = fr.X;
    GSS_TRY(stft_run(ctx, obs, obs_type, D, N, p->stft_fading, Y));
    if (!p->wpe)
        GSS_HIP_CHECK(ctx, hipMemsetAsync(ctx->status_dev + 2, 0, sizeof(int32_t), ctx->stream));
    const int A = wpe_arrays_of(p);
    if (p->wpe && A == 1) {
        GSS_TRY(pipeline_wpe(ctx, p, Y, F, T, D, X));
        ctx->arena_off = mark;
    } else if (p->wpe) {
        GSS_TRY(wpe_arrays_regroup_run(ctx, Y, F, T, A, D / A, true, X));
        GSS_TRY(pipeline_wpe(ctx, p, X, F * A, T, D / A, Y));
        GSS_TRY(wpe_arrays_regroup_run(ctx, Y, F, T, A, D / A, false, X));
        ctx->arena_off = mark;
    }
    if (!guide) GSS_TRY(activity_run(ctx, act, K, N_act, p->stft_fading, fr.actf));
    GSS_TRY(cacgmm_run(ctx, X, F, T, D, guide ? *guide : em_guide_from_activity(fr.actf, T_act), K,
                       p->bss_iterations, p->bss_iterations_post, fr.gamma));
    ctx->arena_off = mark;
    return GSS_OK;
}

static int copy_tap(gss_ctx *ctx, void *dst, const void *src, size_t bytes) {
    if (!dst) return GSS_OK;
    GSS_HIP_CHECK(ctx, hipMemcpyAsync(dst, src, bytes, hipMemcpyDeviceToDevice, ctx->stream));
    return GSS_OK;
}

static int copy_front_taps(gss_ctx *ctx, const gss_debug_taps *taps, const PipelineFront &fr,
                           int F, int64_t T, int64_t T_act, int D, int K) {
    GSS_TRY(copy_tap(ctx, taps->Obs_ftd, fr.X, sizeof(cplx) * (size_t)F * T * D));
    if (taps->act_frames)
        GSS_HIP_CHECK(ctx, hipMemcpy2DAsync(taps->act_frames, (size_t)T, fr.actf, (size_t)T_act,
                                            (size_t)T, (size_t)K, hipMemcpyDeviceToDevice,
                                            ctx->stream));
    GSS_TRY(copy_tap(ctx, taps->gamma, fr.gamma, sizeof(double) * (size_t)F * K * T));
    return GSS_OK;
}

static int enhance_observation_impl(gss_ctx *ctx, const gss_params *p, const void *obs,
                                    int obs_type, int D, int64_t N, const uint8_t *act, int K,
                                    int64_t N_act, int target, int64_t start_ctx, int64_t end_ctx,
                                    double *out, const gss_debug_taps *taps,
                                    bool guided = false,
                                    const gss_guidance *guidance = nullptr) {
    GSS_REQUIRE(ctx, !guided || guidance, GSS_ERR_INVALID,
                "gss_enhance_observation_guided: guidance is NULL");
    GSS_TRY(check_pipeline_front(ctx, p, obs, D, N, guided ? (const void *)guidance : act, out,
                                 guided ? "gss_enhance_observation_guided"
                                        : "gss_enhance_observation"));
    GSS_REQUIRE(ctx, !guided || !taps || !taps->act_frames, GSS_ERR_INVALID,
                "gss_enhance_observation_guided: taps->act_frames must be NULL (a guided call "
                "has no frame activity)");
    GSS_REQUIRE(ctx, target >= 0 && target < K, GSS_ERR_INVALID,
                "target_index %d outside [0, %d)", target, K);
    GSS_REQUIRE(ctx, start_ctx >= 0 && end_ctx >= 0, GSS_ERR_INVALID,
                "assert context samples >= 0 failed: %lld %lld", (long long)start_ctx,
                (long long)end_ctx);
    int64_t T, T_act;
    GSS_TRY(check_pipeline_rest(ctx, p, D, N, K, N_act, &T, &T_act));
    const int size = p->stft_size, shift = p->stft_shift, fading = p->stft_fading;
    const int F = size / 2 + 1;
    EmGuide guide{};
    if (guided) GSS_TRY(check_guidance(ctx, guidance, K, T, &guide));

    GSS_TRY(arena_reserve(ctx, pipeline_workspace(p, F, T, T_act, D, K)));
    PipelineFront fr;
    GSS_TRY(alloc_front(ctx, p, F, T, T_act, D, K, &fr));
    double *mx = arena_alloc_t<double>(ctx, (size_t)F * T);
    double *mn = arena_alloc_t<double>(ctx, (size_t)F * T);
    cplx *Xhat = arena_alloc_t<cplx>(ctx, (size_t)F * T);
    int32_t *ref = arena_alloc_t<int32_t>(ctx, 4);
    GSS_REQUIRE(ctx, mx && mn && Xhat && ref, GSS_ERR_NOMEM, "workspace sizing bug");
    const size_t mark = ctx->arena_off;
    GSS_TRY(run_front(ctx, p, obs, obs_type, D, N, act, K, N_act, F, T, T_act, fr, mark,
                      guided ? &guide : nullptr));
    cplx *const X = fr.X;

    int64_t sf = 0, ef = 0;
    if (p->bf_drop_context) {
        sf = gss_samples_to_stft_frames(start_ctx, size, shift, fading);
        ef = gss_samples_to_stft_frames(end_ctx, size, shift, fading);
    }
    GSS_TRY(masks_from_posteriors_run(ctx, fr.gamma, F, K, T, target, p->bf_drop_context, sf, ef,
                                      mx, mn));
    if (p->bf == 0 || p->bf == 3) {
        GSS_TRY(mvdr_run(ctx, X, F, T, D, mx, mn, 1, Xhat, ref, p->bf == 3));
        ctx->arena_off = mark;
    } else {
        GSS_TRY(channel_pick_run(ctx, X, F, T, D, p->bf, Xhat));
    }
    if (p->postfilter == 1) GSS_TRY(mask_mul_run(ctx, Xhat, mx, F, T));
    GSS_TRY(istft_run(ctx, Xhat, T, fading, out));

    if (taps) {
        GSS_TRY(copy_front_taps(ctx, taps, fr, F, T, T_act, D, K));
        GSS_TRY(copy_tap(ctx, taps->target_mask, mx, sizeof(double) * (size_t)F * T));
        GSS_TRY(copy_tap(ctx, taps->distortion_mask, mn, sizeof(double) * (size_t)F * T));
        GSS_TRY(copy_tap(ctx, taps->Xhat, Xhat, sizeof(cplx) * (size_t)F * T));
        if (p->bf == 0 || p->bf == 3) GSS_TRY(copy_tap(ctx, taps->ref_channel, ref, sizeof(int32_t)));
    }
    return GSS_OK;
}

static int enhance_observation_targets_impl(gss_ctx *ctx, const gss_params *p, const void *obs,
                                            int obs_type, int D, int64_t N, const uint8_t *act,
                                            int K, int64_t N_act, int S, const int32_t *targets,
                                            const int64_t *start_ctx, const int64_t *end_ctx,
                                            double *out, const gss_debug_taps *taps) {
    ctx->last_targets = 0;
    GSS_TRY(check_pipeline_front(ctx, p, obs, D, N, act, out, "gss_enhance_observation_targets"));
    GSS_REQUIRE(ctx, targets && start_ctx && end_ctx, GSS_ERR_INVALID,
                "gss_enhance_observation_targets: NULL target or context array");
    GSS_REQUIRE(ctx, K >= 1 && K <= GSS_MAX_CLASSES, GSS_ERR_INVALID,
                "cacgmm: assert 1 <= K < 20 failed: K=%d", K);
    GSS_REQUIRE(ctx, S >= 1 && S <= K, GSS_ERR_INVALID,
                "%d targets of %d classes: need 1 <= S <= K", S, K);
    uint32_t seen = 0;
    for (int s = 0; s < S; ++s) {
        GSS_REQUIRE(ctx, targets[s] >= 0 && targets[s] < K, GSS_ERR_INVALID,
                    "target_index[%d] = %d outside [0, %d)", s, targets[s], K);
        GSS_REQUIRE(ctx, !(seen >> targets[s] & 1u), GSS_ERR_INVALID,
                    "target_index[%d] = %d is given twice", s, targets[s]);
        seen |= 1u << targets[s];
        GSS_REQUIRE(ctx, start_ctx[s] >= 0 && end_ctx[s] >= 0, GSS_ERR_INVALID,
                    "assert context samples >= 0 failed: %lld %lld (target %d)",
                    (long long)start_ctx[s], (long long)end_ctx[s], s);
    }
    int64_t T, T_act;
    GSS_TRY(check_pipeline_rest(ctx, p, D, N, K, N_act, &T, &T_act));
    const int size = p->stft_size, shift = p->stft_shift, fading = p->stft_fading;
    const int F = size / 2 + 1;

    GSS_TRY(arena_reserve(ctx, targets_workspace(p, F, T, T_act, D, K, S)));
    PipelineFront fr;
    GSS_TRY(alloc_front(ctx, p, F, T, T_act, D, K, &fr));
    double *mx = arena_alloc_t<double>(ctx, (size_t)S * F * T);
    double *mn = arena_alloc_t<double>(ctx, (size_t)S * F * T);
    cplx *Xhat = arena_alloc_t<cplx>(ctx, (size_t)S * F * T);
    int32_t *ref = arena_alloc_t<int32_t>(ctx, 4 * (size_t)S);
    GSS_REQUIRE(ctx, mx && mn && Xhat && ref, GSS_ERR_NOMEM, "workspace sizing bug");
    const size_t mark = ctx->arena_off;
    GSS_TRY(run_front(ctx, p, obs, obs_type, D, N, act, K, N_act, F, T, T_act, fr, mark));
    cplx *const X = fr.X;

    int64_t sf[GSS_MAX_CLASSES] = {}, ef[GSS_MAX_CLASSES] = {};
    if (p->bf_drop_context) {
        for (int s = 0; s < S; ++s) {
            sf[s] = gss_samples_to_stft_frames(start_ctx[s], size, shift, fading);
            ef[s] = gss_samples_to_stft_frames(end_ctx[s], size, shift, fading);
        }
    }
    GSS_TRY(masks_targets_run(ctx, fr.gamma, F, K, T, S, targets, p->bf_drop_context, sf, ef, mx,
                              mn));
    const bool beamformer = p->bf == 0 || p->bf == 3;
    if (beamformer) {
        GSS_TRY(mvdr_run(ctx, X, F, T, D, mx, mn, 1, Xhat, ref, p->bf == 3,
                         -1, S, true));
        ctx->arena_off = mark;
        if (p->postfilter == 1)
            GSS_TRY(mask_mul_targets_run(ctx, Xhat, (int64_t)F * T, Xhat, mx, F, T, S, 1));
    } else {
        cplx *X1 = arena_alloc_t<cplx>(ctx, (size_t)F * T);
        GSS_REQUIRE(ctx, X1, GSS_ERR_NOMEM, "workspace sizing bug");
        GSS_TRY(channel_pick_run(ctx, X, F, T, D, p->bf, X1));
        GSS_TRY(mask_mul_targets_run(ctx, X1, 0, Xhat, mx, F, T, S, p->postfilter == 1));
        ctx->arena_off = mark;
    }
    GSS_TRY(istft_run(ctx, Xhat, T, fading, out, S));

    if (taps) {
        GSS_TRY(copy_front_taps(ctx, taps, fr, F, T, T_act, D, K));
        GSS_TRY(copy_tap(ctx, taps->target_mask, mx, sizeof(double) * (size_t)S * F * T));
        GSS_TRY(copy_tap(ctx, taps->distortion_mask, mn, sizeof(double) * (size_t)S * F * T));
        GSS_TRY(copy_tap(ctx, taps->Xhat, Xhat, sizeof(cplx) * (size_t)S * F * T));
        if (beamformer && taps->ref_channel)
            GSS_HIP_CHECK(ctx, hipMemcpyAsync(taps->ref_channel, ref, sizeof(int32_t) * S,
                                              hipMemcpyDeviceToDevice, ctx->stream));
    }
    return GSS_OK;
}

extern "C" int gss_enhance_observation(gss_ctx *ctx, const gss_params *p, const double *obs,
                                       int D, int64_t N, const uint8_t *act, int K,
                                       int64_t N_act, int target, int64_t start_ctx,
                                       int64_t end_ctx, double *out,
                                       const gss_debug_taps *taps) {
    GSS_ENTER_VARIANTS(ctx);
    return enhance_observation_impl(ctx, p, obs, 0, D, N, act, K, N_act, target, start_ctx, end_ctx,
                                    out, taps);
}

extern "C" int gss_enhance_observation_guided(gss_ctx *ctx, const gss_params *p,
                                              const double *obs, int D, int64_t N,
                                              const gss_guidance *guidance, int K, int target,
                                              int64_t start_ctx, int64_t end_ctx, double *out,
                                              const gss_debug_taps *taps) {
    GSS_ENTER_VARIANTS(ctx);
    return enhance_observation_impl(ctx, p, obs, 0, D, N, nullptr, K, N, target, start_ctx,
                                    end_ctx, out, taps, true, guidance);
}

extern "C" int gss_enhance_observation_pcm16(gss_ctx *ctx, const gss_params *p,
                                             const int16_t *obs, int D, int64_t N,
                                             const uint8_t *act, int K, int64_t N_act, int target,
                                             int64_t start_ctx, int64_t end_ctx, double *out,
                                             const gss_debug_taps *taps) {
    GSS_ENTER_VARIANTS(ctx);
    return enhance_observation_impl(ctx, p, obs, 1, D, N, act, K, N_act, target, start_ctx, end_ctx,
                                    out, taps);
}

extern "C" int gss_enhance_observation_targets(gss_ctx *ctx, const gss_params *p,
                                               const double *obs, int D, int64_t N,
                                               const uint8_t *act, int K, int64_t N_act, int S,
                                               const int32_t *targets, const int64_t *start_ctx,
                                               const int64_t *end_ctx, double *out,
                                               const gss_debug_taps *taps) {
    GSS_ENTER_VARIANTS(ctx);
    return enhance_observation_targets_impl(ctx, p, obs, 0, D, N, act, K, N_act, S, targets,
                                            start_ctx, end_ctx, out, taps);
}

extern "C" int gss_enhance_observation_targets_pcm16(gss_ctx *ctx, const gss_params *p,
                                                     const int16_t *obs, int D, int64_t N,
                                                     const uint8_t *act, int K, int64_t N_act,
                                                     int S, const int32_t *targets,
                                                     const int64_t *start_ctx,
                                                     const int64_t *end_ctx, double *out,
                                                     const gss_debug_taps *taps) {
    GSS_ENTER_VARIANTS(ctx);
    return enhance_observation_targets_impl(ctx, p, obs, 1, D, N, act, K, N_act, S, targets,
                                            start_ctx, end_ctx, out, taps);
}

extern "C" int gss_enhance_observation_host(gss_ctx *ctx, const gss_params *p,
                                            const double *obs, int D, int64_t N,
                                            const uint8_t *act, int K, int64_t N_act,
                                            int target, int64_t start_ctx, int64_t end_ctx,
                                            double *out) {
    GSS_ENTER_VARIANTS(ctx);
    GSS_REQUIRE(ctx, p && obs && act && out && N >= 1 && D >= 1 && K >= 1, GSS_ERR_INVALID,
                "gss_enhance_observation_host: bad arguments");
    const int64_t T = gss_stft_num_frames(N, p->stft_size, p->stft_shift, p->stft_fading);
    const int64_t n_out = gss_istft_num_samples(T, p->stft_size, p->stft_shift, p->stft_fading);
    double *obs_d = nullptr, *out_d = nullptr;
    uint8_t *act_d = nullptr;
    int st = gss_dev_malloc(ctx, sizeof(double) * (size_t)D * N, (void **)&obs_d);
    if (st == GSS_OK) st = gss_dev_malloc(ctx, (size_t)K * N_act, (void **)&act_d);
    if (st == GSS_OK) st = gss_dev_malloc(ctx, sizeof(double) * (size_t)n_out, (void **)&out_d);
    if (st == GSS_OK) st = gss_memcpy_h2d(ctx, obs_d, obs, sizeof(double) * (size_t)D * N);
    if (st == GSS_OK) st = gss_memcpy_h2d(ctx, act_d, act, (size_t)K * N_act);
    if (st == GSS_OK)
        st = gss_enhance_observation(ctx, p, obs_d, D, N, act_d, K, N_act, target, start_ctx,
                                     end_ctx, out_d, nullptr);
    if (st == GSS_OK) st = gss_memcpy_d2h(ctx, out, out_d, sizeof(double) * (size_t)n_out);
    std::string keep = ctx->error;
    (void)hipStreamSynchronize(ctx->stream);
    if (obs_d) (void)hipFree(obs_d);
    if (act_d) (void)hipFree(act_d);
    if (out_d) (void)hipFree(out_d);
    ctx->error = keep;
    return st;
}
```

### pb_chime5_amd/csrc/gss_internal.h

```cpp
#pragma once
#include <hip/hip_runtime.h>

#include <cstdint>
#include <cstdio>
#include <map>
#include <string>
#include <vector>

#include "../../include/gss_hip.h"

typedef double2 cplx;

int gss_variant(const char *key, int dflt);
inline bool gss_variant_set(const char *key) { return gss_variant(key, 0) != 0; }

#if (defined(GSS_CORR_TRACE) || defined(GSS_WCOV_TRACE) || defined(GSS_EM4_TRACE) || \
     defined(GSS_CHOL_TRACE)) && !defined(GSS_EXPERIMENT_BUILD)
#error "trace instrumentation needs -DGSS_EXPERIMENT_BUILD=1 (tools/build_variant.sh)"
#endif

#define GSS_TINY 2.2250738585072014e-308

__device__ __forceinline__ cplx c_make(double r, double i) { return make_double2(r, i); }
__device__ __forceinline__ cplx c_add(cplx a, cplx b) { return make_double2(a.x + b.x, a.y + b.y); }
__device__ __forceinline__ cplx c_sub(cplx a, cplx b) { return make_double2(a.x - b.x, a.y - b.y); }
__device__ __forceinline__ cplx c_mul(cplx a, cplx b) {
    return make_double2(a.x * b.x - a.y * b.y, a.x * b.y + a.y * b.x);
}
__device__ __forceinline__ cplx c_mulc(cplx a, cplx b) {
    return make_double2(a.x * b.x + a.y * b.y, a.y * b.x - a.x * b.y);
}
__device__ __forceinline__ cplx c_cmul(cplx a, cplx b) {
    return make_double2(a.x * b.x + a.y * b.y, a.x * b.y - a.y * b.x);
}
__device__ __forceinline__ cplx c_scale(cplx a, double s) { return make_double2(a.x * s, a.y * s); }
__device__ __forceinline__ cplx c_conj(cplx a) { return make_double2(a.x, -a.y); }
__device__ __forceinline__ double c_abs2(cplx a) { return a.x * a.x + a.y * a.y; }
__device__ __forceinline__ void c_fma(cplx &acc, cplx a, cplx b) {
    acc.x = fma(a.x, b.x, acc.x);
    acc.x = fma(-a.y, b.y, acc.x);
    acc.y = fma(a.x, b.y, acc.y);
    acc.y = fma(a.y, b.x, acc.y);
}
__device__ __forceinline__ void c_fmac(cplx &acc, cplx a, cplx b) {
    acc.x = fma(a.x, b.x, acc.x);
    acc.x = fma(a.y, b.y, acc.x);
    acc.y = fma(a.y, b.x, acc.y);
    acc.y = fma(-a.x, b.y, acc.y);
}
__device__ __forceinline__ void c_cfma(cplx &acc, cplx a, cplx b) {
    acc.x = fma(a.x, b.x, acc.x);
    acc.x = fma(a.y, b.y, acc.x);
    acc.y = fma(a.x, b.y, acc.y);
    acc.y = fma(-a.y, b.x, acc.y);
}

__device__ __forceinline__ void wave_sync() {
    __builtin_amdgcn_fence(__ATOMIC_RELEASE, "wavefront");
    __builtin_amdgcn_wave_barrier();
    __builtin_amdgcn_fence(__ATOMIC_ACQUIRE, "wavefront");
}

template <int CTRL, int ROW_MASK, int BANK_MASK>
__device__ __forceinline__ double dpp_shifted(double v) {
    const unsigned long long u = __double_as_longlong(v);
    const int lo = __builtin_amdgcn_update_dpp(0, (int)(unsigned)u, CTRL, ROW_MASK, BANK_MASK, true);
    const int hi = __builtin_amdgcn_update_dpp(0, (int)(unsigned)(u >> 32), CTRL, ROW_MASK, BANK_MASK, true);
    return __longlong_as_double(((unsigned long long)(unsigned)hi << 32) | (unsigned)lo);
}
__device__ __forceinline__ double wave_sum(double v) {
    double s = v + dpp_shifted<0x111, 0xf, 0xf>(v);
    s += dpp_shifted<0x112, 0xf, 0xf>(v);
    s += dpp_shifted<0x113, 0xf, 0xf>(v);
    s += dpp_shifted<0x114, 0xf, 0xe>(s);
    s += dpp_shifted<0x118, 0xf, 0xc>(s);
    s += dpp_shifted<0x142, 0xa, 0xf>(s);
    s += dpp_shifted<0x143, 0xc, 0xf>(s);
    const unsigned long long u = __double_as_longlong(s);
    const unsigned lo = __builtin_amdgcn_readlane((int)(unsigned)u, 63);
    const unsigned hi = __builtin_amdgcn_readlane((int)(unsigned)(u >> 32), 63);
    return __longlong_as_double(((unsigned long long)hi << 32) | lo);
}
__device__ __forceinline__ double wave_max(double v) {
#pragma unroll
    for (int o = 32; o > 0; o >>= 1) v = fmax(v, __shfl_xor(v, o, 64));
    return v;
}

__device__ __forceinline__ bool xcd_group_map(int nsub, int F, int &f, int &sub) {
    const int L = blockIdx.x;
    const int sg = L / (8 * nsub), rem = L - sg * 8 * nsub;
    sub = rem >> 3;
    f = sg * 8 + (rem & 7);
    return f < F;
}
static inline unsigned xcd_grid(int nsub, int F) { return (unsigned)(nsub * ((F + 7) / 8 * 8)); }

__host__ __device__ __forceinline__ int tri_index(int d1, int d2, int D) {
    return d1 * D - (d1 * (d1 - 1)) / 2 + (d2 - d1);
}
__host__ __device__ __forceinline__ int tri_count(int D) { return D * (D + 1) / 2; }

struct ProfEntry {
    std::string name;
    hipEvent_t start, stop;
};

struct gss_ctx {
    int device = 0;
    hipStream_t own_stream = nullptr;
    hipStream_t stream = nullptr;
    hipStream_t aux_stream = nullptr;
    hipEvent_t ev_fork = nullptr, ev_join = nullptr;
    int utterances_in_flight = 0;
    std::string error;

    char *arena = nullptr;
    size_t arena_size = 0;
    size_t arena_off = 0;
    size_t arena_peak = 0;

    int stft_size = 0, stft_shift = 0;
    double *win_analysis = nullptr;
    double *win_synthesis = nullptr;
    cplx *twiddle = nullptr;

    int32_t *status_host = nullptr;
    int32_t *status_dev = nullptr;
    int last_targets = 0;

    void *wpe_tiles = nullptr;
    int wpe_tiles_key[4] = {-1, -1, -1, -1};

    bool profiling = false;
    std::vector<ProfEntry> prof_pending;
    std::vector<hipEvent_t> event_pool;
    std::map<std::string, std::pair<long, double>> prof_acc;
    std::string prof_filter;
};

#define GSS_STATUS_TARGETS 16
#define GSS_STATUS_BYTES (4 * (GSS_STATUS_TARGETS + GSS_MAX_CLASSES + 1))

int gss_fail(gss_ctx *ctx, int code, const char *fmt, ...);

#define GSS_HIP_CHECK(ctx, expr)                                                   \
    do {                                                                           \
        hipError_t _e = (expr);                                                    \
        if (_e != hipSuccess)                                                      \
            return gss_fail((ctx), GSS_ERR_HIP, "%s failed: %s (%s:%d)", #expr,    \
                            hipGetErrorString(_e), __FILE__, __LINE__);            \
    } while (0)

#define GSS_REQUIRE(ctx, cond, code, ...)                      \
    do {                                                       \
        if (!(cond)) return gss_fail((ctx), (code), __VA_ARGS__); \
    } while (0)

#define GSS_TRY(expr)              \
    do {                           \
        int _s = (expr);           \
        if (_s != GSS_OK) return _s; \
    } while (0)

int arena_reserve(gss_ctx *ctx, size_t bytes);
void arena_reset(gss_ctx *ctx);
void *arena_alloc(gss_ctx *ctx, size_t bytes);
template <typename T>
static inline T *arena_alloc_t(gss_ctx *ctx, size_t count) {
    return reinterpret_cast<T *>(arena_alloc(ctx, count * sizeof(T)));
}
static inline size_t align_up(size_t v, size_t a = 256) { return (v + a - 1) / a * a; }

struct ProfScope {
    gss_ctx *ctx;
    ProfEntry e;
    bool active;
    ProfScope(gss_ctx *c, const char *name);
    ~ProfScope();
};
#define GSS_PROF(ctx, name) ProfScope _prof_scope_##__LINE__((ctx), (name))

#define GSS_LAUNCH_CHECK(ctx, name)                                               \
    do {                                                                          \
        hipError_t _e = hipGetLastError();                                        \
        if (_e != hipSuccess)                                                     \
            return gss_fail((ctx), GSS_ERR_HIP, "launch of %s failed: %s", (name), \
                            hipGetErrorString(_e));                               \
    } while (0)

size_t wpe_workspace_bytes(int F, int64_t T, int D, int taps, int delay);
int wpe_inverse_power_run(gss_ctx *ctx, const cplx *Y, int F, int64_t T, int D, int psd_context,
                          double *w);
int wpe_run(gss_ctx *ctx, const cplx *Y, int F, int64_t T, int D, int taps, int delay,
            int iterations, int psd_context, cplx *X, int part = -1, int array_bins = 0);
int wpe_copy_zero_pivots(gss_ctx *ctx);
int wpe_arrays_regroup_run(gss_ctx *ctx, const cplx *src, int F, int64_t T, int A, int C,
                           bool to_arrays, cplx *dst);
int aux_stream_ready(gss_ctx *ctx);

size_t cacgmm_workspace_bytes(int F, int64_t T, int D, int K);
struct EmGuide {
    const double *init;
    const uint8_t *mask;
    int64_t init_f_stride, init_k_stride, mask_f_stride, mask_k_stride;
};
static inline EmGuide em_guide_from_activity(const uint8_t *act, int64_t act_stride) {
    return EmGuide{nullptr, act, 0, 0, 0, act_stride};
}
int cacgmm_run(gss_ctx *ctx, const cplx *Y, int F, int64_t T, int D, const EmGuide &guide, int K,
               int iterations, int iterations_post, double *gamma);

int psd_partials_run(gss_ctx *ctx, const cplx *Y, int F, int64_t T, int D, const double *W2,
                     int nch, int chunk_frames, cplx *part, int S = 1);

size_t mvdr_workspace_bytes(int F, int64_t T, int D, int S = 1);
int mvdr_run(gss_ctx *ctx, const cplx *Y, int F, int64_t T, int D, const double *mx,
             const double *mn, int ban, cplx *Xhat, int32_t *ref_channel, int gev = 0,
             int forced_ref = -1, int S = 1, bool targets = false);
struct TargetMaskArgs {
    int S;
    int target[GSS_MAX_CLASSES];
    int64_t zero_lo_end[GSS_MAX_CLASSES], zero_hi_begin[GSS_MAX_CLASSES];
};
int masks_targets_run(gss_ctx *ctx, const double *gamma, int F, int K, int64_t T, int S,
                      const int32_t *targets, int drop, const int64_t *sf, const int64_t *ef,
                      double *mx, double *mn);
int masks_from_posteriors_run(gss_ctx *ctx, const double *gamma, int F, int K, int64_t T,
                              int target, int drop, int64_t start_frames,
                              int64_t end_frames, double *mx, double *mn);

size_t stft_workspace_bytes(int64_t T, int size);
int stft_run(gss_ctx *ctx, const void *x, int in_type, int D, int64_t N, int fading, cplx *Y);
int istft_run(gss_ctx *ctx, const cplx *X, int64_t T, int fading, double *x, int S = 1);
int activity_run(gss_ctx *ctx, const uint8_t *act, int K, int64_t N, int fading,
                 uint8_t *out);
int channel_pick_run(gss_ctx *ctx, const cplx *Y, int F, int64_t T, int D, int mode,
                     cplx *Xhat);
int mask_mul_run(gss_ctx *ctx, cplx *Xhat, const double *mask_ft, int F, int64_t T);
int mask_mul_targets_run(gss_ctx *ctx, const cplx *src, int64_t src_stride, cplx *dst,
                         const double *mx, int F, int64_t T, int S, int apply_mask);

int selftest_mfma_run(gss_ctx *ctx);
```

### pb_chime5_amd/csrc/mvdr.hip

```cpp
#include "dense_wave.h"
#include "gss_internal.h"
#include "jacobi.h"

namespace {

constexpr int PSD_TILE = 64;

__global__ void masks_kernel(const double *__restrict__ gamma, int F, int K, int64_t T,
                             int target, int64_t zero_lo_end, int64_t zero_hi_begin,
                             double *__restrict__ mx, double *__restrict__ mn) {
    const int64_t idx = (int64_t)blockIdx.x * blockDim.x + threadIdx.x;
    if (idx >= (int64_t)F * T) return;
    const int f = idx / T;
    const int64_t t = idx - (int64_t)f * T;
    double x = 0.0, n = 0.0;
    if (t >= zero_lo_end && t < zero_hi_begin) {
        const double *g = gamma + (int64_t)f * K * T + t;
        x = g[(int64_t)target * T];
        for (int k = 0; k < K; ++k)
            if (k != target) n += g[(int64_t)k * T];
    }
    mx[idx] = x;
    mn[idx] = n;
}
// ... 506 lines not shown
        Xhat[t * F + f] = v;
    }
}

template <int SB>
__global__ __launch_bounds__(256) void mvdr_apply_targets_kernel(
    const cplx *__restrict__ Y, const cplx *__restrict__ W, const cplx *__restrict__ Phi,
    const int32_t *__restrict__ ref, int F, int64_t T, int D, int S, int ban, int chunk_frames,
    cplx *__restrict__ Xhat, int32_t *__restrict__ ref_out, int32_t *__restrict__ status,
    int32_t *__restrict__ status0) {
    __shared__ cplx w[SB][GSS_MAX_CHANNELS];
    __shared__ cplx t1[SB][GSS_MAX_CHANNELS];
    __shared__ cplx t2[SB][GSS_MAX_CHANNELS];
    __shared__ double s_norm[SB];
    __shared__ int s_ref[SB];
    const int f = blockIdx.y, tid = threadIdx.x;
    if (tid < S) {
        const int r = ref[4 * tid];
        s_ref[tid] = r;
        if (blockIdx.x == 0 && f == 0) {
            const int code = r == -2 ? -2 - ref[4 * tid + 1] : r;
            if (ref_out) ref_out[tid] = code;
            if (status) __hip_atomic_store(status + tid, code, __ATOMIC_RELAXED, __HIP_MEMORY_SCOPE_SYSTEM);
            if (status0 && tid == 0)
                __hip_atomic_store(status0, code, __ATOMIC_RELAXED, __HIP_MEMORY_SCOPE_SYSTEM);
        }
    }
    __syncthreads();
    for (int i = tid; i < SB * D; i += blockDim.x) {
        const int s = i / D, d = i - s * D;
        const int r = s < S ? s_ref[s] : -1;
        w[s][d] = r >= 0 ? W[(((int64_t)s * F + f) * D + d) * D + r] : c_make(0.0, 0.0);
    }
    __syncthreads();
    if (ban) {
        for (int i = tid; i < S * D; i += blockDim.x) {
            const int s = i / D, a = i - s * D;
            if (s_ref[s] < 0) continue;
            const cplx *PhiN = Phi + (((int64_t)s * F + f) * 2 + 1) * D * D;
            cplx v = c_make(0.0, 0.0);
            for (int e = 0; e < D; ++e) c_fma(v, PhiN[a * D + e], w[s][e]);
            t1[s][a] = v;
            cplx u = c_make(0.0, 0.0);
            for (int d = 0; d < D; ++d) c_cfma(u, w[s][d], PhiN[d * D + a]);
            t2[s][a] = u;
        }
        __syncthreads();
        if (tid < S && s_ref[tid] >= 0) {
            const int s = tid;
            cplx nom = c_make(0.0, 0.0), den = c_make(0.0, 0.0);
            for (int a = 0; a < D; ++a) {
                c_fma(nom, t2[s][a], t1[s][a]);
                c_cfma(den, w[s][a], t1[s][a]);
            }
            const double n = sqrt(hypot(nom.x, nom.y));
            const double dd = hypot(den.x, den.y);
            s_norm[s] = n / dd;
        }
        __syncthreads();
        for (int i = tid; i < S * D; i += blockDim.x) {
            const int s = i / D, d = i - s * D;
            if (s_ref[s] >= 0) w[s][d] = c_scale(w[s][d], s_norm[s]);
        }
        __syncthreads();
    }
    const int64_t c0 = (int64_t)blockIdx.x * chunk_frames;
    const int64_t c1 = c0 + chunk_frames < T ? c0 + chunk_frames : T;
    const double qnan = __longlong_as_double(0x7ff8000000000000LL);
    const cplx *Yf = Y + (int64_t)f * T * D;
    for (int64_t t = c0 + tid; t < c1; t += blockDim.x) {
        const cplx *y = Yf + t * D;
        cplx v[SB];
#pragma unroll
        for (int s = 0; s < SB; ++s) v[s] = c_make(0.0, 0.0);
        for (int d = 0; d < D; ++d) {
            const cplx yd = y[d];
#pragma unroll
            for (int s = 0; s < SB; ++s) c_cfma(v[s], w[s][d], yd);
        }
#pragma unroll
        for (int s = 0; s < SB; ++s)
            if (s < S)
                Xhat[((int64_t)s * T + t) * F + f] = s_ref[s] >= 0 ? v[s] : c_make(qnan, qnan);
    }
}

int psd_chunks(int F, int64_t T, int *chunk_frames) {
    int64_t tiles = (T + PSD_TILE - 1) / PSD_TILE;
    int64_t want = (2048 + F - 1) / F;
    int64_t tpc = (tiles + want - 1) / want;
    if (tpc < 1) tpc = 1;
    *chunk_frames = (int)(tpc * PSD_TILE);
    return (int)((tiles + tpc - 1) / tpc);
}

}

int masks_from_posteriors_run(gss_ctx *ctx, const double *gamma, int F, int K, int64_t T,
                              int target, int drop, int64_t sf, int64_t ef, double *mx,
                              double *mn) {
    int64_t lo_end = 0, hi_begin = T;
    if (drop) {
        lo_end = sf >= 0 ? (sf < T ? sf : T) : (T + sf > 0 ? T + sf : 0);
        if (ef > 0) hi_begin = T - ef > 0 ? T - ef : 0;
    }
    GSS_PROF(ctx, "masks");
    const int64_t total = (int64_t)F * T;
    hipLaunchKernelGGL(masks_kernel, dim3((unsigned)((total + 255) / 256)), dim3(256), 0,
                       ctx->stream, gamma, F, K, T, target, lo_end, hi_begin, mx, mn);
    GSS_LAUNCH_CHECK(ctx, "masks_kernel");
    return GSS_OK;
}

int masks_targets_run(gss_ctx *ctx, const double *gamma, int F, int K, int64_t T, int S,
                      const int32_t *targets, int drop, const int64_t *sf, const int64_t *ef,
                      double *mx, double *mn) {
    TargetMaskArgs a{};
    a.S = S;
    for (int s = 0; s < S; ++s) {
        int64_t lo_end = 0, hi_begin = T;
        if (drop) {
            lo_end = sf[s] >= 0 ? (sf[s] < T ? sf[s] : T) : (T + sf[s] > 0 ? T + sf[s] : 0);
            if (ef[s] > 0) hi_begin = T - ef[s] > 0 ? T - ef[s] : 0;
        }
        a.target[s] = targets[s];
        a.zero_lo_end[s] = lo_end;
        a.zero_hi_begin[s] = hi_begin;
    }
    GSS_PROF(ctx, "masks_targets");
    const int64_t total = (int64_t)F * T;
    hipLaunchKernelGGL(masks_targets_kernel, dim3((unsigned)((total + 255) / 256)), dim3(256), 0,
                       ctx->stream, gamma, F, K, T, a, mx, mn);
    GSS_LAUNCH_CHECK(ctx, "masks_targets_kernel");
    return GSS_OK;
}

size_t mvdr_workspace_bytes(int F, int64_t T, int D, int S) {
    const size_t NE = tri_count(D);
    int cf;
    const int nch = psd_chunks(F, T, &cf);
    size_t b = 0;
    b += align_up(sizeof(cplx) * (size_t)S * F * nch * 2 * NE);
    b += align_up(sizeof(double) * (size_t)S * F * 2);
    b += align_up(sizeof(double) * (size_t)S * F * 2 * T);
    b += align_up(sizeof(cplx) * (size_t)S * F * 2 * D * D);
    b += align_up(sizeof(cplx) * (size_t)S * F * D * D);
    b += align_up(sizeof(cplx) * (size_t)S * F * D * 2);
    b += align_up(sizeof(int32_t) * 4 * (size_t)S);
    return b + 4096;
}

int mvdr_run(gss_ctx *ctx, const cplx *Y, int F, int64_t T, int D, const double *mx,
             const double *mn, int ban, cplx *Xhat, int32_t *ref_channel, int gev,
             int forced_ref, int S, bool targets) {
    const int NE = tri_count(D);
    int cf;
    const int nch = psd_chunks(F, T, &cf);
    cplx *part = arena_alloc_t<cplx>(ctx, (size_t)S * F * nch * 2 * NE);
    double *msum = arena_alloc_t<double>(ctx, (size_t)S * F * 2);
    double *W2 = arena_alloc_t<double>(ctx, (size_t)S * F * 2 * T);
    cplx *Phi = arena_alloc_t<cplx>(ctx, (size_t)S * F * 2 * D * D);
    cplx *W = arena_alloc_t<cplx>(ctx, (size_t)S * F * D * D);
    cplx *snr = arena_alloc_t<cplx>(ctx, (size_t)S * F * D * 2);
    int32_t *ref = arena_alloc_t<int32_t>(ctx, 4 * (size_t)S);
    GSS_REQUIRE(ctx, part && msum && W2 && Phi && W && snr && ref, GSS_ERR_NOMEM,
                "mvdr workspace");
    ctx->last_targets = targets ? S : 0;
    {
        GSS_PROF(ctx, targets ? "psd_targets" : "psd");
        hipLaunchKernelGGL(mask_pack_kernel, dim3(F, S), dim3(256), 0, ctx->stream, mx, mn, T, W2,
                           msum);
        GSS_LAUNCH_CHECK(ctx, "mask_pack_kernel");
        GSS_TRY(psd_partials_run(ctx, Y, F, T, D, W2, nch, cf, part, S));
    }
    if (gev) {
        GSS_PROF(ctx, targets ? "gev_solve_targets" : "gev_solve");
        const int m = D + (D & 1);
        const size_t lds = (sizeof(cplx) * 4 * (size_t)m * m + 15) / 16 * 16;
        if (lds > 64 * 1024)
            GSS_HIP_CHECK(ctx, hipFuncSetAttribute(
                                   reinterpret_cast<const void *>(gev_solve_kernel),
                                   hipFuncAttributeMaxDynamicSharedMemorySize, (int)lds));
        if (S == 1) {
            GSS_HIP_CHECK(ctx, hipMemsetAsync(ref, 0, sizeof(int32_t), ctx->stream));
            GSS_HIP_CHECK(ctx, hipMemsetAsync(ref + 1, 0x7f, sizeof(int32_t), ctx->stream));
        } else {
            GSS_HIP_CHECK(ctx, hipMemset2DAsync(ref, 4 * sizeof(int32_t), 0, sizeof(int32_t), S,
                                                ctx->stream));
            GSS_HIP_CHECK(ctx, hipMemset2DAsync(ref + 1, 4 * sizeof(int32_t), 0x7f,
                                                sizeof(int32_t), S, ctx->stream));
        }
        hipLaunchKernelGGL(gev_solve_kernel, dim3(F, S), dim3(64), lds, ctx->stream, part, msum,
                           nch, D, Phi, W, ref);
        GSS_LAUNCH_CHECK(ctx, "gev_solve_kernel");
    } else {
        {
            GSS_PROF(ctx, targets ? "mvdr_solve_targets" : "mvdr_solve");
            const int m = D + (D & 1);
            const size_t lds = (sizeof(cplx) * ((size_t)D * 2 * D + 2 * (size_t)m * m) +
                                32 + 15) / 16 * 16;
            if (lds > 64 * 1024)
                GSS_HIP_CHECK(ctx, hipFuncSetAttribute(
                                       reinterpret_cast<const void *>(mvdr_solve_kernel),
                                       hipFuncAttributeMaxDynamicSharedMemorySize, (int)lds));
            hipLaunchKernelGGL(mvdr_solve_kernel, dim3(F, S), dim3(MVDR_NT), lds, ctx->stream, part,
                               msum, nch, D, 1e-10, Phi, W, snr);
            GSS_LAUNCH_CHECK(ctx, "mvdr_solve_kernel");
        }
        {
            GSS_PROF(ctx, targets ? "mvdr_ref_targets" : "mvdr_ref");
            hipLaunchKernelGGL(mvdr_ref_kernel, dim3(S), dim3(MVDR_REF_NT),
                               sizeof(cplx) * MVDR_REF_CHUNK * (size_t)D * 2, ctx->stream, snr, F, D, 1e-10,
                               forced_ref, ref);
            GSS_LAUNCH_CHECK(ctx, "mvdr_ref_kernel");
        }
    }
    const int chunk = 256;
    const dim3 grid((unsigned)((T + chunk - 1) / chunk), F);
    if (!targets) {
        GSS_PROF(ctx, "mvdr_apply");
        hipLaunchKernelGGL(mvdr_apply_kernel, grid, dim3(256), 0, ctx->stream, Y, W, Phi, ref, F, T,
                           D, ban, chunk, Xhat, ref_channel, ctx->status_dev);
        GSS_LAUNCH_CHECK(ctx, "mvdr_apply_kernel");
        return GSS_OK;
    }
    GSS_PROF(ctx, "mvdr_apply_targets");
    int32_t *const status = ctx->status_dev + GSS_STATUS_TARGETS;
#define GSS_APPLY_TARGETS(SB)                                                                    \
    hipLaunchKernelGGL(mvdr_apply_targets_kernel<SB>, grid, dim3(256), 0, ctx->stream, Y, W, Phi, \
                       ref, F, T, D, S, ban, chunk, Xhat, ref_channel, status, ctx->status_dev)
    if (S <= 2) GSS_APPLY_TARGETS(2);
    else if (S <= 4) GSS_APPLY_TARGETS(4);
    else if (S <= 8) GSS_APPLY_TARGETS(8);
    else GSS_APPLY_TARGETS(GSS_MAX_CLASSES);
#undef GSS_APPLY_TARGETS
    GSS_LAUNCH_CHECK(ctx, "mvdr_apply_targets_kernel");
    return GSS_OK;
}
```

### pb_chime5_amd/csrc/wpe.hip

```cpp
#include <algorithm>
#include <cmath>
#include <cstdlib>

#include "gss_internal.h"
#include <type_traits>
#include "dense_wave.h"

typedef double v4d __attribute__((ext_vector_type(4)));

namespace {

constexpr int POW_FRAMES = 256;
__global__ __launch_bounds__(POW_FRAMES) void wpe_power_kernel(const cplx *__restrict__ X,
                                                               int64_t T, int D, int psd_context,
                                                               double *__restrict__ raw,
                                                               double *__restrict__ w) {
    extern __shared__ __attribute__((aligned(16))) char smem[];
    double *ps = reinterpret_cast<double *>(smem);
    __shared__ double red[POW_FRAMES / 64];
    const int f = blockIdx.x, tid = threadIdx.x;
    const cplx *Xf = X + (int64_t)f * T * D;
    double *wout = w + (int64_t)f * T;
    double *wf = psd_context > 0 ? raw + (int64_t)f * T : wout;
    const int DP = D + 1;
    double mx = 0.0;
    for (int64_t t0 = 0; t0 < T; t0 += POW_FRAMES) {
        const int nfr = (int)min((int64_t)POW_FRAMES, T - t0);
        const int total = nfr * D;
        const cplx *src = Xf + t0 * D;
        __syncthreads();
        {
            constexpr int LB = 8;
            const int qf = POW_FRAMES / D, rf = POW_FRAMES - qf * D;
            int fr = tid / D, d = tid - fr * D;
            for (int base = tid; base < total; base += LB * POW_FRAMES) {
                cplx v[LB];
#pragma unroll
                for (int j = 0; j < LB; ++j) {
                    const int idx = base + j * POW_FRAMES;
                    v[j] = idx < total ? src[idx] : c_make(0.0, 0.0);
                }
#pragma unroll
                for (int j = 0; j < LB; ++j) {
                    if (base + j * POW_FRAMES < total) ps[fr * DP + d] = c_abs2(v[j]);
                    fr += qf;
                    d += rf;
                    if (d >= D) {
                        d -= D;
                        ++fr;
                    }
                }
            }
        }
        __syncthreads();
        if (tid < nfr) {
            double p = 0.0;
            for (int d = 0; d < D; ++d) p += ps[tid * DP + d];
            p = p / (double)D;
            wf[t0 + tid] = p;
            mx = fmax(mx, p);
        }
    }
    if (psd_context > 0) {
        __syncthreads();
        mx = 0.0;
        if (psd_context <= 16) {
            for (int64_t t = tid; t < T; t += POW_FRAMES) {
                const int64_t lo = t - psd_context > 0 ? t - psd_context : 0;
                const int64_t hi = t + psd_context < T - 1 ? t + psd_context : T - 1;
                double sum = 0.0;
                for (int64_t u = lo; u <= hi; ++u) sum += wf[u];
                const double p = sum / (double)(hi - lo + 1);
                wout[t] = p;
                mx = fmax(mx, p);
            }
        } else {
            const int64_t run = (T + POW_FRAMES - 1) / POW_FRAMES;
            const int64_t t_beg = (int64_t)tid * run, t_end = t_beg + run < T ? t_beg + run : T;
            double sum = 0.0, carry = 0.0;
            auto add = [&](double x) {
                const double s = sum + x;
                const double bb = s - sum;
                const double err = (sum - (s - bb)) + (x - bb);
                carry += err;
                sum = s;
            };
            int64_t lo = 0, hi = -1;
            for (int64_t t = t_beg; t < t_end; ++t) {
                const int64_t nlo = t - psd_context > 0 ? t - psd_context : 0;
                const int64_t nhi = t + psd_context < T - 1 ? t + psd_context : T - 1;
                if (t == t_beg) {
                    for (int64_t u = nlo; u <= nhi; ++u) add(wf[u]);
                } else {
                    if (nhi > hi) add(wf[nhi]);
                    if (nlo > lo) add(-wf[lo]);
                }
                lo = nlo;
                hi = nhi;
                const double p = (sum + carry) / (double)(hi - lo + 1);
                wout[t] = p;
                mx = fmax(mx, p);
            }
        }
    }
    mx = wave_max(mx);
    if ((tid & 63) == 0) red[tid >> 6] = mx;
    __syncthreads();
    mx = fmax(fmax(red[0], red[1]), fmax(red[2], red[3]));
    const double eps = 1e-10 * mx;
    for (int64_t t = tid; t < T; t += POW_FRAMES) wout[t] = 1.0 / fmax(wout[t], eps);
}

#ifndef GSS_CORR_KT
#define GSS_CORR_KT 64
#endif
constexpr int CORR_KT = GSS_CORR_KT;
constexpr int CORR_FINE_MAX_SUBTILES = 48;

struct CorrTile {
    int row_off, col_off, is_p, mask;
};

template <int TS, int MASK, int KSTEPS = CORR_KT / 4>
__device__ __forceinline__ void corr_chunk(const cplx *S, const double *wS, int D,
                                           const CorrTile &tl, v4d (&t1)[TS][TS],
                                           v4d (&t2)[TS][TS], v4d (&t3)[TS][TS]) {
    const int lane = threadIdx.x & 63;
    const int li = lane & 15, lk = lane >> 4;
    auto need = [](int a, int b) { return ((MASK >> (a * TS + b)) & 1) != 0; };
    auto need_row = [&](int a) {
        bool r = false;
        for (int b = 0; b < TS; ++b) r = r || need(a, b);
        return r;
    };
    auto need_col = [&](int b) {
        bool r = false;
        for (int a = 0; a < TS; ++a) r = r || need(a, b);
        return r;
    };
    const int ksteps = KSTEPS;
    cplx a_cur[TS], b_cur[TS], a_nxt[TS], b_nxt[TS];
    double w_cur, w_nxt = 0.0;
    {
        const cplx *base = S + lk * D + li;
        w_cur = wS[lk];
#pragma unroll
        for (int m = 0; m < TS; ++m) {
            a_cur[m] = base[tl.row_off + 16 * m];
            b_cur[m] = base[tl.col_off + 16 * m];
        }
    }
    constexpr int KU = TS == 1 || KSTEPS < 16 ? 4 : 16;
#pragma unroll KU
    for (int ks = 0; ks < ksteps; ++ks) {
        if (ks + 1 < ksteps) {
            const int kf = 4 * (ks + 1) + lk;
            const cplx *base = S + kf * D + li;
            w_nxt = wS[kf];
#pragma unroll
            for (int m = 0; m < TS; ++m) {
                a_nxt[m] = need_row(m) ? base[tl.row_off + 16 * m] : c_make(0.0, 0.0);
                b_nxt[m] = need_col(m) ? base[tl.col_off + 16 * m] : c_make(0.0, 0.0);
            }
        }
        double ar[TS], ai[TS], as[TS], br[TS], bi[TS], bd[TS];
#pragma unroll
        for (int m = 0; m < TS; ++m) {
            ar[m] = a_cur[m].x * w_cur;
            ai[m] = a_cur[m].y * w_cur;
            as[m] = ar[m] + ai[m];
            br[m] = b_cur[m].x;
            bi[m] = b_cur[m].y;
            bd[m] = b_cur[m].x - b_cur[m].y;
// ... 126 lines not shown
    double *wS = reinterpret_cast<double *>(S + frames_lds * D);

    int f, grp;
    if (!xcd_group_map((ntiles + NW - 1) / NW, F, f, grp)) return;
    const int wave = __builtin_amdgcn_readfirstlane(threadIdx.x >> 6);
    const int tile_id = grp * NW + wave;
    const bool active = tile_id < ntiles;
    const CorrTile tl = tiles[active ? tile_id : 0];
    const cplx *Yf = Y + (int64_t)f * T * D;
    const double *wf = w + (int64_t)f * T;
    constexpr int FULL = (1 << (TS * TS)) - 1;
    const int mask = __builtin_amdgcn_readfirstlane(active ? tl.mask : 1);
#define CORR_CASE(M) \
    case M: corr_tile_body<TS, M, NW, STG1>(Yf, wf, T, D, n, c, frames_lds, S, wS, tl, active, f, R, P); break
    if (TS == 2) {
        switch (mask) {
            CORR_CASE(1);
            CORR_CASE(3);
            CORR_CASE(5);
            CORR_CASE(11);
            default:
                corr_tile_body<TS, FULL, NW, STG1>(Yf, wf, T, D, n, c, frames_lds, S, wS, tl, active, f, R, P);
        }
    } else {
        corr_tile_body<TS, FULL, NW, STG1>(Yf, wf, T, D, n, c, frames_lds, S, wS, tl, active, f, R, P);
    }
#undef CORR_CASE
}

template <int KS, int STG>
__global__ __launch_bounds__(64 * KS, 4) void wpe_corr_ksplit_kernel(
    const cplx *__restrict__ Y, const double *__restrict__ w, int F, int64_t T, int D, int n,
    int c, int padf, const CorrTile *__restrict__ tiles, int ntiles, cplx *__restrict__ R,
    cplx *__restrict__ P) {
    extern __shared__ __attribute__((aligned(16))) char smem[];
    const int frames_lds = CORR_KT + c + padf;
    const int total = frames_lds * D;
    const size_t wbytes = sizeof(cplx) * (size_t)total + sizeof(double) * CORR_KT;
    int f, tile_id;
    if (!xcd_group_map(ntiles, F, f, tile_id)) return;
    const int lane = threadIdx.x & 63;
    const int wave = __builtin_amdgcn_readfirstlane(threadIdx.x >> 6);
    cplx *S = reinterpret_cast<cplx *>(smem + wave * wbytes);
    double *wS = reinterpret_cast<double *>(S + total);
    const CorrTile tl = tiles[tile_id];
    const cplx *Yf = Y + (int64_t)f * T * D;
    const double *wf = w + (int64_t)f * T;
    v4d t1[1][1], t2[1][1], t3[1][1];
    corr_zero<1>(t1, t2, t3);

    const int nchunk = (int)((T + CORR_KT - 1) / CORR_KT);
    const int ch0 = (int)((int64_t)wave * nchunk / KS), ch1 = (int)((int64_t)(wave + 1) * nchunk / KS);
    cplx stg[STG];
    double stg_w = 0.0;
    auto stage_load = [&](int64_t t0) {
        const int64_t fr0 = t0 - c;
#pragma unroll
        for (int s = 0; s < STG; ++s) {
            const int idx = lane + 64 * s;
            const int64_t fr = fr0 + idx / D;
            stg[s] = c_make(0.0, 0.0);
            if (idx < total && fr >= 0 && fr < T) stg[s] = Yf[fr0 * D + idx];
        }
        stg_w = (t0 + lane < T) ? wf[t0 + lane] : 0.0;
    };
    if (ch0 < ch1) stage_load((int64_t)ch0 * CORR_KT);
    for (int ch = ch0; ch < ch1; ++ch) {
        wave_sync();
#pragma unroll
        for (int s = 0; s < STG; ++s) {
            const int idx = lane + 64 * s;
            if (idx < total) S[idx] = stg[s];
        }
        wS[lane] = stg_w;
        wave_sync();
        if (ch + 1 < ch1) stage_load((int64_t)(ch + 1) * CORR_KT);
        corr_chunk<1, 1>(S, wS, D, tl, t1, t2, t3);
    }
    v4d re, im;
#pragma unroll
    for (int r = 0; r < 4; ++r) {
        re[r] = t1[0][0][r] + t2[0][0][r];
        im[r] = (t3[0][0][r] - t1[0][0][r]) + t2[0][0][r];
    }
    __syncthreads();
    cplx *red = reinterpret_cast<cplx *>(smem);
    if (wave > 0) {
#pragma unroll
        for (int r = 0; r < 4; ++r) red[((wave - 1) * 4 + r) * 64 + lane] = c_make(re[r], im[r]);
    }
    __syncthreads();
    if (wave == 0) {
#pragma unroll
        for (int o = 0; o < KS - 1; ++o)
#pragma unroll
            for (int r = 0; r < 4; ++r) {
                const cplx v = red[(o * 4 + r) * 64 + lane];
                re[r] += v.x;
                im[r] += v.y;
            }
        t1[0][0] = re;
        t3[0][0] = im;
        corr_store<1, 1, true>(tl, f, n, c, D, t1, t1, t3, R, P);
    }
}

using lds_void_ptr = __attribute__((address_space(3))) void *;

#ifdef GSS_CORR_TRACE
__device__ long long g_corr_trace[8192 * 6];
__device__ long long g_corr_phase[8192 * 4];
extern "C" int gss_debug_corr_trace(long long *host, int entries) {
    return (int)hipMemcpyFromSymbol(host, HIP_SYMBOL(g_corr_trace), sizeof(long long) * 6 * entries);
}
extern "C" int gss_debug_corr_phase(long long *host, int entries, int reset) {
    int rc = (int)hipMemcpyFromSymbol(host, HIP_SYMBOL(g_corr_phase), sizeof(long long) * 4 * entries);
    if (reset) {
        void *p = nullptr;
        (void)hipGetSymbolAddress(&p, HIP_SYMBOL(g_corr_phase));
        (void)hipMemset(p, 0, sizeof(long long) * 4 * 8192);
    }
    return rc;
}
#define CORR_TRACE(slot)                                                                  \
    if (threadIdx.x == 0 && blockIdx.x < 8192) g_corr_trace[blockIdx.x * 6 + (slot)] = wall_clock64()
#else
#define CORR_TRACE(slot)
#endif

struct CorrQueue {
    int ngroups, gh;
};

__device__ __forceinline__ int corr_queue_len(int F, int x) { return (F - x + 7) / 8; }

__device__ __forceinline__ int corr_queue_item(int F, int x, int q, const CorrQueue cq) {
    const int heavy = corr_queue_len(F, x) * cq.gh;
    if (q < heavy) return (x + 8 * (q / cq.gh)) * 4096 + q % cq.gh;
    q -= heavy;
    const int gl = max(cq.ngroups - cq.gh, 1);
    return (x + 8 * (q / gl)) * 4096 + cq.gh + q % gl;
}

__device__ __forceinline__ int corr_fetch(int *counters, int F, int xcd, int &live, const CorrQueue cq) {
    for (; live < 8; ++live) {
        const int x = (xcd + live) & 7;
        const int len = corr_queue_len(F, x) * cq.ngroups;
        const int q = atomicAdd(counters + 16 * x, 1);
        if (q < len) return corr_queue_item(F, x, q, cq);
    }
    return -1;
}

template <int MASK, int NW, bool BLOCKED, class Issue>
__device__ __forceinline__ void corr_item_dma(
    int64_t T, int D, int n, int c, int win, cplx *S0, double *w0, const CorrTile tl, bool active,
    int f, int f_next, int &b, Issue &issue, int *ring_slot, int fetched, cplx *__restrict__ R,
    cplx *__restrict__ P) {
    constexpr int TS = 2;
    v4d t1[TS][TS], t2[TS][TS], t3[TS][TS];
    corr_zero<TS>(t1, t2, t3);
    v4d sre[BLOCKED ? TS : 1][BLOCKED ? TS : 1], sim[BLOCKED ? TS : 1][BLOCKED ? TS : 1];
    if constexpr (BLOCKED) {
#pragma unroll
        for (int a = 0; a < TS; ++a)
#pragma unroll
            for (int bb = 0; bb < TS; ++bb) sre[a][bb] = sim[a][bb] = (v4d){0.0, 0.0, 0.0, 0.0};
    }
    auto chunk_iter = [&](int64_t t0, auto short_tag) {
        constexpr bool SHORT = decltype(short_tag)::value;
#ifdef GSS_CORR_TRACE
        const long long ta = clock64();
#endif
        if (!SHORT && t0 + CORR_KT < T)
            issue(f, t0 + CORR_KT, b ^ 1);
        else if (f_next >= 0)
            issue(f_next, 0, b ^ 1);
#ifdef GSS_CORR_TRACE
        const long long tb = clock64();
#endif
        if (active) {
            if constexpr (SHORT) {
                const int frames = (int)(T - t0);
                for (int g = 0; 16 * g < frames; ++g)
                    corr_chunk<TS, MASK, 4>(S0 + b * win + 16 * g * D, w0 + b * CORR_KT + 16 * g, D,
                                            tl, t1, t2, t3);
            } else {
                corr_chunk<TS, MASK>(S0 + b * win, w0 + b * CORR_KT, D, tl, t1, t2, t3);
            }
        }
        if constexpr (BLOCKED) if (active) {
#pragma unroll
            for (int a = 0; a < TS; ++a)
#pragma unroll
                for (int bb = 0; bb < TS; ++bb) {
                    if (!((MASK >> (a * TS + bb)) & 1)) continue;
#pragma unroll
                    for (int r = 0; r < 4; ++r) {
                        sre[a][bb][r] += t1[a][bb][r] + t2[a][bb][r];
                        sim[a][bb][r] += (t3[a][bb][r] - t1[a][bb][r]) + t2[a][bb][r];
                    }
                    t1[a][bb] = t2[a][bb] = t3[a][bb] = (v4d){0.0, 0.0, 0.0, 0.0};
                }
        }
        if (t0 == 0 && threadIdx.x == 0) *ring_slot = fetched;
#ifdef GSS_CORR_TRACE
        const long long tc = clock64();
        asm volatile("s_waitcnt vmcnt(0)" ::: "memory");
        const long long td = clock64();
#endif
        __syncthreads();
#ifdef GSS_CORR_TRACE
        if (threadIdx.x == 0 && blockIdx.x < 8192) {
            const long long te = clock64();
            g_corr_phase[blockIdx.x * 4 + 0] += tb - ta;
            g_corr_phase[blockIdx.x * 4 + 1] += tc - tb;
            g_corr_phase[blockIdx.x * 4 + 2] += td - tc;
            g_corr_phase[blockIdx.x * 4 + 3] += te - td;
        }
#endif
        b ^= 1;
    };
    int64_t t0 = 0;
    for (; T - t0 > CORR_KT - 16; t0 += CORR_KT) chunk_iter(t0, std::false_type{});
    if (t0 < T) chunk_iter(t0, std::true_type{});
    if (active)
    {
        if constexpr (BLOCKED) corr_store<TS, MASK, true>(tl, f, n, c, D, sre, sre, sim, R, P);
        else corr_store<TS, MASK>(tl, f, n, c, D, t1, t2, t3, R, P);
    }
}

template <int NW, bool BLOCKED = false>
__global__ __launch_bounds__(64 * NW) void wpe_corr_persist_kernel(
    const cplx *__restrict__ Y, const double *__restrict__ w, int F, int64_t T, int D, int n,
    int c, int pieces, const CorrTile *__restrict__ tiles, int ntiles, CorrQueue cq,
    int *__restrict__ counters, cplx *__restrict__ R, cplx *__restrict__ P) {
    extern __shared__ __attribute__((aligned(16))) char smem[];
    cplx *S0 = reinterpret_cast<cplx *>(smem);
    double *w0 = reinterpret_cast<double *>(S0 + 2 * pieces * 64);
    __shared__ int ring[3];
    const int wave = __builtin_amdgcn_readfirstlane(threadIdx.x >> 6);
    const int lane = threadIdx.x & 63;
    const int win = pieces * 64;
    const int xcd = __builtin_amdgcn_s_getreg(20 | (0 << 6) | (3 << 11)) & 7;
#ifdef GSS_CORR_TRACE
    if (threadIdx.x == 0 && blockIdx.x < 8192) {
        g_corr_trace[blockIdx.x * 6 + 0] = xcd;
        g_corr_trace[blockIdx.x * 6 + 1] = wall_clock64();
        g_corr_trace[blockIdx.x * 6 + 2] = clock64();
    }
#endif
    int live = 0;
    if (threadIdx.x == 0) {
        ring[0] = corr_fetch(counters, F, xcd, live, cq);
        ring[1] = ring[0] < 0 ? -1 : corr_fetch(counters, F, xcd, live, cq);
        ring[2] = -1;
    }
    __syncthreads();

    const uint32_t lane16 = lane * 16;
    auto issue = [&](int fq, int64_t t0, int bq) {
        const __amdgpu_buffer_rsrc_t rsrc_y = __builtin_amdgcn_make_buffer_rsrc(
            const_cast<cplx *>(Y + (int64_t)fq * T * D), 0, (int)(T * D * 16), 0x00020000);
        cplx *Sb = S0 + bq * win;
        const int64_t g0 = (t0 - c) * (int64_t)D;
        if (g0 >= 0 && g0 + win <= T * (int64_t)D) {
            for (int p = wave; p < pieces; p += NW)
                __builtin_amdgcn_raw_ptr_buffer_load_lds(rsrc_y, (lds_void_ptr)(Sb + p * 64), 16,
                                                         lane16, (int)((g0 + p * 64) * 16), 0, 0);
        } else {
            for (int p = wave; p < pieces; p += NW) {
                const int64_t gp = g0 + p * 64;
                const uint32_t voff = (uint32_t)((gp + lane) * 16);
                if (gp >= 0) {
                    __builtin_amdgcn_raw_ptr_buffer_load_lds(rsrc_y, (lds_void_ptr)(Sb + p * 64),
                                                             16, voff, 0, 0, 0);
                } else if (gp + lane < 0) {
                    Sb[p * 64 + lane] = c_make(0.0, 0.0);
                } else {
                    __builtin_amdgcn_raw_ptr_buffer_load_lds(rsrc_y, (lds_void_ptr)(Sb + p * 64),
                                                             16, voff, 0, 0, 0);
                }
            }
        }
        if (wave == NW - 1 && lane < CORR_KT / 2) {
            const __amdgpu_buffer_rsrc_t rsrc_w = __builtin_amdgcn_make_buffer_rsrc(
                const_cast<double *>(w + (int64_t)fq * T), 0, (int)(T * 8), 0x00020000);
            __builtin_amdgcn_raw_ptr_buffer_load_lds(rsrc_w, (lds_void_ptr)(w0 + bq * CORR_KT), 16,
                                                     lane16, (int)(t0 * 8), 0, 0);
        }
    };

    int item = __builtin_amdgcn_readfirstlane(ring[0]);
    if (item < 0) return;
    int b = 0;
    issue(item >> 12, 0, 0);
    __syncthreads();
    for (int k = 0; item >= 0; ++k) {
        const int next = __builtin_amdgcn_readfirstlane(ring[(k + 1) % 3]);
        int fetched = -1;
        if (threadIdx.x == 0 && next >= 0) fetched = corr_fetch(counters, F, xcd, live, cq);
        const int f = item >> 12, grp = item & 4095;
        const int tile_id = grp * NW + wave;
        const bool active = tile_id < ntiles;
        const CorrTile tl = tiles[active ? tile_id : 0];
        const int mask = __builtin_amdgcn_readfirstlane(active ? tl.mask : 1);
        int *ring_slot = &ring[(k + 2) % 3];
#define CORR_CASE(M)                                                                              \
    case M:                                                                                       \
        corr_item_dma<M, NW, BLOCKED>(T, D, n, c, win, S0, w0, tl, active, f, next < 0 ? -1 : next >> 12, \
                                 b, issue, ring_slot, fetched, R, P);                             \
        break
        switch (mask) {
            CORR_CASE(1);
            CORR_CASE(3);
            CORR_CASE(5);
            CORR_CASE(11);
            default:
                corr_item_dma<15, NW, BLOCKED>(T, D, n, c, win, S0, w0, tl, active, f,
                                          next < 0 ? -1 : next >> 12, b, issue, ring_slot, fetched,
                                          R, P);
        }
#undef CORR_CASE
        item = next;
#ifdef GSS_CORR_TRACE
        if (threadIdx.x == 0 && blockIdx.x < 8192) {
            g_corr_trace[blockIdx.x * 6 + 3] = wall_clock64();
            g_corr_trace[blockIdx.x * 6 + 4] = clock64();
            g_corr_trace[blockIdx.x * 6 + 5] = k + 1;
        }
#endif
    }
}

#ifndef GSS_UPD_PREFETCH
#define GSS_UPD_PREFETCH 1
#endif
constexpr int CH_NB = 48;
constexpr int UD_LD = CH_NB + 1;

constexpr size_t DIAG_LDS = sizeof(cplx) * 2 * UD_LD + sizeof(double) * CH_NB;

__device__ inline void chol_diag_block(cplx *A, int n, int j0, cplx *Ud, double *dinv,
                                       int32_t *zero_pivots) {
    const int tid = threadIdx.x, tx = tid & 15, ty = tid >> 4;
    const int nb = min(CH_NB, n - j0);
    cplx reg[3][3];
#pragma unroll
    for (int a = 0; a < 3; ++a)
#pragma unroll
        for (int b = 0; b < 3; ++b) {
            const int i = ty + 16 * a, k = tx + 16 * b;
            reg[a][b] = (k >= i && k < nb) ? A[(int64_t)(j0 + i) * n + j0 + k] : c_make(0.0, 0.0);
        }
    if (!chol_inverse_sweep<16, 3, false, true>(reg, nb, Ud, UD_LD, dinv, tx, ty)) {
        if (tid < nb && dinv[tid] == 0.0) atomicAdd(zero_pivots, 1);
    }
#pragma unroll
    for (int a = 0; a < 3; ++a) {
        const int i = ty + 16 * a;
        const double di = i < nb ? dinv[i] : 0.0;
#pragma unroll
        for (int b = 0; b < 3; ++b) {
            const int k = tx + 16 * b;
            if (b < a || i >= nb || k >= nb) continue;
            const cplx raw = reg[a][b];
            A[(int64_t)(j0 + i) * n + j0 + k] =
                k == i ? c_make(di > 0.0 ? sqrt(raw.x) : 0.0, 0.0) : c_scale(raw, di);
        }
    }
}

__global__ __launch_bounds__(256) void chol_diag_kernel(cplx *__restrict__ R, int n, int j0,
                                                        int32_t *__restrict__ zero_pivots) {
    __shared__ __attribute__((aligned(16))) char smem[DIAG_LDS];
    cplx *Ud = reinterpret_cast<cplx *>(smem);
    double *dinv = reinterpret_cast<double *>(Ud + 2 * UD_LD);
    chol_diag_block(R + (int64_t)blockIdx.x * n * n, n, j0, Ud, dinv, zero_pivots);
}

constexpr int UDP_SIZE = 16 * (CH_NB + 1) + 16 * (CH_NB - 16 + 1) + 16 * (CH_NB - 32 + 1);
__device__ __forceinline__ int udp_off(int row, int col) {
    const int b = row >> 4;
    const int base = b == 0 ? 0 : b == 1 ? 16 * (CH_NB + 1) : 16 * (CH_NB + 1) + 16 * (CH_NB - 16 + 1);
    return base + (row & 15) * (CH_NB - 16 * b + 1) + col - 16 * b;
}

__device__ inline void chol_panel_tile(cplx *A, cplx *Z, int n, int D, int j0, int nb, int ct,
                                       const cplx *Ud, const double *dinv, int lane) {
    const int ntrail = n - j0 - nb;
    const int li = lane & 15, lk = lane >> 4;
    const int nct_a = (ntrail + 15) / 16;
    cplx *base;
    int64_t stride;
    int ncols;
    if (ct < nct_a) {
        base = A + (int64_t)j0 * n + j0 + nb + 16 * ct;
        stride = n;
        ncols = min(16, ntrail - 16 * ct);
    } else {
        base = Z + (int64_t)j0 * D + 16 * (ct - nct_a);
        stride = D;
        ncols = min(16, D - 16 * (ct - nct_a));
    }
    cplx bv[CH_NB / 4];
#pragma unroll
    for (int ks = 0; ks < CH_NB / 4; ++ks) {
        const int row = 4 * ks + lk;
        bv[ks] = (row < nb && li < ncols) ? base[row * stride + li] : c_make(0.0, 0.0);
    }
    v4d xre[3], xim[3];
#pragma unroll
    for (int it = 0; it < 3; ++it) {
        v4d tre, tim;
#pragma unroll
        for (int r = 0; r < 4; ++r) {
            tre[r] = bv[4 * it + r].x;
            tim[r] = bv[4 * it + r].y;
        }
        const int i = 16 * it + li;
#pragma unroll
        for (int jt = 0; jt < it; ++jt)
#pragma unroll
            for (int ks = 0; ks < 4; ++ks) {
                const int k = 16 * jt + 4 * ks + lk;
                const cplx u = Ud[udp_off(k, i)];
                tre = __builtin_amdgcn_mfma_f64_16x16x4f64(-u.x, xre[jt][ks], tre, 0, 0, 0);
                tim = __builtin_amdgcn_mfma_f64_16x16x4f64(-u.x, xim[jt][ks], tim, 0, 0, 0);
                tre = __builtin_amdgcn_mfma_f64_16x16x4f64(-u.y, xim[jt][ks], tre, 0, 0, 0);
                tim = __builtin_amdgcn_mfma_f64_16x16x4f64(u.y, xre[jt][ks], tim, 0, 0, 0);
            }
        xre[it] = (v4d){0.0, 0.0, 0.0, 0.0};
        xim[it] = (v4d){0.0, 0.0, 0.0, 0.0};
#pragma unroll
        for (int ks = 0; ks < 4; ++ks) {
            const int k = 16 * it + 4 * ks + lk;
            cplx w = Ud[udp_off(i, k)];
            if (k == i) w = c_make(i < nb ? dinv[i] : 0.0, 0.0);
            if (k > i) w = c_make(0.0, 0.0);
            xre[it] = __builtin_amdgcn_mfma_f64_16x16x4f64(w.x, tre[ks], xre[it], 0, 0, 0);
            xim[it] = __builtin_amdgcn_mfma_f64_16x16x4f64(w.x, tim[ks], xim[it], 0, 0, 0);
            xre[it] = __builtin_amdgcn_mfma_f64_16x16x4f64(-w.y, tim[ks], xre[it], 0, 0, 0);
            xim[it] = __builtin_amdgcn_mfma_f64_16x16x4f64(w.y, tre[ks], xim[it], 0, 0, 0);
        }
    }
#pragma unroll
    for (int it = 0; it < 3; ++it)
#pragma unroll
        for (int r = 0; r < 4; ++r) {
            const int row = 16 * it + lk + 4 * r;
            if (row < nb && li < ncols) base[row * stride + li] = c_make(xre[it][r], xim[it][r]);
        }
}

__device__ inline void chol_stage_diag(const cplx *A, int n, int j0, int nb, cplx *Ud, double *dinv) {
    const int tid = threadIdx.x;
    constexpr int WL = CH_NB * CH_NB / 256;
    static_assert(WL * 256 == CH_NB * CH_NB, "block size");
    cplx wv[WL];
#pragma unroll
    for (int s = 0; s < WL; ++s) {
        const int idx = tid + 256 * s;
        const int i = idx / CH_NB, k = idx - i * CH_NB;
        wv[s] = c_make(0.0, 0.0);
        if (i < nb && k < nb && k >= (i & ~15)) wv[s] = A[(int64_t)(j0 + i) * n + j0 + k];
    }
#pragma unroll
    for (int s = 0; s < WL; ++s) {
        const int idx = tid + 256 * s;
        const int i = idx / CH_NB, k = idx - i * CH_NB;
        if (k >= (i & ~15)) Ud[udp_off(i, k)] = wv[s];
        if (k == i) dinv[i] = wv[s].x > 0.0 ? 1.0 / wv[s].x : 0.0;
    }
}

__global__ __launch_bounds__(256) void chol_trsm_kernel(cplx *__restrict__ R,
                                                        cplx *__restrict__ P, int F, int n,
                                                        int D, int j0) {
    extern __shared__ __attribute__((aligned(16))) char smem[];
    cplx *Ud = reinterpret_cast<cplx *>(smem);
    double *dinv = reinterpret_cast<double *>(Ud + UDP_SIZE);
    const int tid = threadIdx.x;
    const int nb = min(CH_NB, n - j0);
    const int ntrail = n - j0 - nb;
    const int npanel = (ntrail + 15) / 16 + (D + 15) / 16;
// ... 658 lines not shown
            }
            __builtin_amdgcn_sched_barrier(0);
            double gr[NT], gi[NT];
#pragma unroll
            for (int b = 0; b < NT; ++b) {
                gr[b] = g_cur[b].x;
                gi[b] = g_cur[b].y;
            }
            mfma(u_cur.x, u_cur.y, gr, gi);
            __builtin_amdgcn_sched_barrier(0);
            u_cur = u_nxt;
#pragma unroll
            for (int b = 0; b < NT; ++b) g_cur[b] = g_nxt[b];
        }
    }
    for (int ks = ks_tail; ks < ksteps; ++ks) checked_step();
#pragma unroll
    for (int b = 0; b < NT; ++b)
#pragma unroll
        for (int reg = 0; reg < 4; ++reg) {
            const int r = 16 * wave + lk + 4 * reg;
            const int fl = PH * r + colp[b];
            const int64_t t = t0 + fl;
            if (colv[b] && t < T) {
                const int fw = fl + c;
                const cplx y = S[fw * DP + fw / PH + cold[b]];
                const double pre = acc_re[b][reg] + acc_t2[b][reg];
                const double pim = (acc_im[b][reg] - acc_re[b][reg]) + acc_t2[b][reg];
                X[((int64_t)f * T + t) * D + cold[b]] = c_make(y.x - pre, y.y - pim);
            }
        }
}

__global__ void mfma_selftest_kernel(double *out) {
    const int lane = threadIdx.x;
    const int li = lane & 15, lk = lane >> 4;
    const double a = lk == 0 ? (double)(li + 1) : 0.0;
    const double b = lk == 0 ? 100.0 * (double)(li + 1) : 0.0;
    v4d acc = {0.0, 0.0, 0.0, 0.0};
    acc = __builtin_amdgcn_mfma_f64_16x16x4f64(a, b, acc, 0, 0, 0);
    for (int reg = 0; reg < 4; ++reg) {
        const int row = lk + 4 * reg, col = li;
        out[row * 16 + col] = acc[reg];
    }
}

constexpr int REGROUP_FRAMES = 32;
constexpr int REGROUP_THREADS = 256;

template <bool to_arrays>
__global__ __launch_bounds__(REGROUP_THREADS) void wpe_arrays_regroup_kernel(
    const cplx *__restrict__ src, int64_t T, int A, int C, cplx *__restrict__ dst) {
    __shared__ cplx tile[REGROUP_FRAMES * GSS_MAX_CHANNELS];
    const int D = A * C;
    const int64_t f = blockIdx.y;
    const int64_t t0 = (int64_t)blockIdx.x * REGROUP_FRAMES;
    const int nt = (int)std::min<int64_t>(REGROUP_FRAMES, T - t0);
    const int64_t ftd0 = (f * T + t0) * D;
    const int n_ftd = nt * D;
    if (to_arrays) {
        for (int k = threadIdx.x; k < n_ftd; k += REGROUP_THREADS) tile[k] = src[ftd0 + k];
    } else {
        for (int k = threadIdx.x; k < n_ftd; k += REGROUP_THREADS) {
            const int a = k / (nt * C), r = k - a * nt * C;
            const int t = r / C, c = r - t * C;
            tile[t * D + a * C + c] = src[((f * A + a) * T + t0) * C + r];
        }
    }
    __syncthreads();
    if (to_arrays) {
        for (int k = threadIdx.x; k < n_ftd; k += REGROUP_THREADS) {
            const int a = k / (nt * C), r = k - a * nt * C;
            const int t = r / C, c = r - t * C;
            dst[((f * A + a) * T + t0) * C + r] = tile[t * D + a * C + c];
        }
    } else {
        for (int k = threadIdx.x; k < n_ftd; k += REGROUP_THREADS) dst[ftd0 + k] = tile[k];
    }
}

}

int wpe_arrays_regroup_run(gss_ctx *ctx, const cplx *src, int F, int64_t T, int A, int C,
                           bool to_arrays, cplx *dst) {
    GSS_REQUIRE(ctx, A * C <= GSS_MAX_CHANNELS, GSS_ERR_UNSUPPORTED, "regroup: D=%d", A * C);
    const dim3 grid((unsigned)((T + REGROUP_FRAMES - 1) / REGROUP_FRAMES), (unsigned)F);
    GSS_PROF(ctx, "wpe_arrays_regroup");
    if (to_arrays)
        hipLaunchKernelGGL(wpe_arrays_regroup_kernel<true>, grid, dim3(REGROUP_THREADS), 0,
                           ctx->stream, src, T, A, C, dst);
    else
        hipLaunchKernelGGL(wpe_arrays_regroup_kernel<false>, grid, dim3(REGROUP_THREADS), 0,
                           ctx->stream, src, T, A, C, dst);
    GSS_LAUNCH_CHECK(ctx, "wpe_arrays_regroup_kernel");
    return GSS_OK;
}

static int corr_tiles(int n, int D, int c, int ct, std::vector<CorrTile> &tiles) {
    const int ts = ct / 16;
    auto mask_of = [&](int r0, int c0, int ncols_limit, bool upper_only) {
        int m = 0;
        for (int a = 0; a < ts; ++a)
            for (int b = 0; b < ts; ++b) {
                const int rr = r0 + 16 * a, cc = c0 + 16 * b;
                bool needed = rr < n && cc < ncols_limit;
                if (upper_only && cc + 15 < rr) needed = false;
                if (needed) m |= 1 << (a * ts + b);
            }
        return m;
    };
    const int last_col = (n - 1) / ct;
    const bool p_folded = ct == 16 && (c * D) / ct == last_col && (c * D + D - 1) / ct == last_col &&
                          !gss_variant_set("corr_p_tiles");
    for (int r0 = 0; r0 < n; r0 += ct)
        for (int c0 = 0; c0 < n; c0 += ct)
            if (c0 + ct > r0) {
                const bool with_p = p_folded && c0 / ct == last_col;
                tiles.push_back({r0, c0, with_p ? 2 : 0,
                                 mask_of(r0, c0, with_p ? std::max(n, c * D + D) : n, true)});
            }
    if (!p_folded)
        for (int r0 = 0; r0 < n; r0 += ct)
            for (int c0 = 0; c0 < D; c0 += ct)
                tiles.push_back({r0, c * D + c0, 1, mask_of(r0, c0, D, false)});
    std::stable_sort(tiles.begin(), tiles.end(), [](const CorrTile &x, const CorrTile &y) {
        return __builtin_popcount(x.mask) > __builtin_popcount(y.mask);
    });
    return (int)tiles.size();
}

static int corr_tiles_pairs(int n, int D, int c, std::vector<CorrTile> &tiles) {
    for (int r0 = 0; r0 < n; r0 += 16)
        for (int c0 = r0; c0 < n; c0 += 32) tiles.push_back({r0, c0, 0, c0 + 16 < n ? 3 : 1});
    for (int r0 = 0; r0 < n; r0 += 32)
        for (int c0 = 0; c0 < D; c0 += 16) tiles.push_back({r0, c * D + c0, 1, r0 + 16 < n ? 5 : 1});
    std::stable_sort(tiles.begin(), tiles.end(), [](const CorrTile &x, const CorrTile &y) {
        return __builtin_popcount(x.mask) > __builtin_popcount(y.mask);
    });
    return (int)tiles.size();
}

static int corr_padf(int D, int ct) { return (ct + D - 1) / D + 1; }

size_t wpe_workspace_bytes(int F, int64_t T, int D, int taps, int delay) {
    const size_t n = (size_t)taps * D;
    size_t b = 0;
    b += 2 * align_up(sizeof(double) * (size_t)F * T);
    b += align_up(sizeof(cplx) * (size_t)F * n * n);
    b += align_up(sizeof(cplx) * (size_t)F * n * D);
    return b + 4096;
}

static int wpe_power_launch(gss_ctx *ctx, const cplx *cur, int F, int64_t T, int D,
                            int psd_context, double *raw, double *w) {
    const size_t pow_lds = sizeof(double) * POW_FRAMES * (D + 1);
    if (pow_lds > 64 * 1024)
        GSS_HIP_CHECK(ctx, hipFuncSetAttribute(reinterpret_cast<const void *>(wpe_power_kernel),
                                               hipFuncAttributeMaxDynamicSharedMemorySize,
                                               (int)pow_lds));
    hipLaunchKernelGGL(wpe_power_kernel, dim3(F), dim3(POW_FRAMES), pow_lds, ctx->stream,
                       cur, T, D, psd_context, raw, w);
    GSS_LAUNCH_CHECK(ctx, "wpe_power_kernel");
    return GSS_OK;
}

int wpe_inverse_power_run(gss_ctx *ctx, const cplx *Y, int F, int64_t T, int D, int psd_context,
                          double *w) {
    double *raw = psd_context > 0 ? arena_alloc_t<double>(ctx, (size_t)F * T) : nullptr;
    GSS_REQUIRE(ctx, raw || psd_context == 0, GSS_ERR_NOMEM, "wpe power workspace");
    return wpe_power_launch(ctx, Y, F, T, D, psd_context, raw, w);
}

int wpe_run(gss_ctx *ctx, const cplx *Y, int F, int64_t T, int D, int taps, int delay,
            int iterations, int psd_context, cplx *X, int part, int array_bins) {
    const int n = taps * D;
    const int c = delay + taps - 1;
    if (iterations == 0) {
        GSS_HIP_CHECK(ctx, hipMemsetAsync(ctx->status_dev + 2, 0, sizeof(int32_t), ctx->stream));
        if (X != Y)
            GSS_HIP_CHECK(ctx, hipMemcpyAsync(X, Y, sizeof(cplx) * (size_t)F * T * D,
                                              hipMemcpyDeviceToDevice, ctx->stream));
        return GSS_OK;
    }
    GSS_REQUIRE(ctx, X != Y, GSS_ERR_INVALID, "gss_wpe: X must not alias Y");
    double *w = arena_alloc_t<double>(ctx, (size_t)F * T);
    double *raw = psd_context > 0 ? arena_alloc_t<double>(ctx, (size_t)F * T) : nullptr;
    cplx *R = arena_alloc_t<cplx>(ctx, (size_t)F * n * n);
    cplx *P = arena_alloc_t<cplx>(ctx, (size_t)F * n * D);
    GSS_REQUIRE(ctx, w && (raw || psd_context == 0) && R && P, GSS_ERR_NOMEM, "wpe workspace");

    std::vector<CorrTile> tiles;
    const int sub16 = (n + 15) / 16;
    int corr_ts = sub16 * (sub16 + 1) / 2 + sub16 * ((D + 15) / 16) <= CORR_FINE_MAX_SUBTILES ? 1 : 2;
    bool corr_pairs = false;
    if (const int e = gss_variant("corr_ts", 0)) {
        corr_ts = e == 1 ? 1 : 2;
        corr_pairs = e == 3;
    }
    const int ntiles = corr_pairs ? corr_tiles_pairs(n, D, c, tiles) : corr_tiles(n, D, c, 16 * corr_ts, tiles);
    constexpr int tm16 = 16, tn16 = 16;
    std::vector<UpdTile> upd;
    std::vector<int> upd_start, upd_count, upd_j0, upd_k, upd_ndiag;
    const bool fold_diag = !gss_variant_set("chol_diag_unfolded");
    {
        const int nblk = (n + CH_NB - 1) / CH_NB;
        for (int J = 0; J < nblk; ++J) {
            upd_start.push_back((int)upd.size());
            const int rs = (J + 1) * CH_NB;
            const bool narrow = J % 2 == 0;
            const int r_end = narrow ? std::min(rs + CH_NB, n) : n;
            const int d_end = std::min(rs + CH_NB, n);
            for (int r0 = rs; r0 < d_end; r0 += tm16)
                for (int c0 = rs; c0 < d_end; c0 += tn16)
                    if (c0 + tn16 > r0) upd.push_back({r0, c0, 0, 0});
            upd_ndiag.push_back(fold_diag ? (int)upd.size() - upd_start.back() : 0);
            for (int r0 = rs; r0 < r_end; r0 += tm16) {
                for (int c0 = rs; c0 < n; c0 += tn16)
                    if (c0 + tn16 > r0 && !(r0 < d_end && c0 < d_end)) upd.push_back({r0, c0, 0, 0});
                for (int cc = 0; cc < D; cc += tn16) upd.push_back({r0, cc, 1, 0});
            }
            upd_count.push_back((int)upd.size() - upd_start.back());
            const bool wide = J % 2 == 1;
            upd_j0.push_back(wide ? (J - 1) * CH_NB : J * CH_NB);
            upd_k.push_back(wide ? 2 * CH_NB : CH_NB);
        }
    }
    GSS_REQUIRE(ctx, ntiles <= 1024 && upd.size() <= 4096, GSS_ERR_UNSUPPORTED,
                "wpe: taps*D=%d too large", n);
    static_assert(sizeof(CorrTile) == sizeof(UpdTile), "tile structs share one buffer");
    if (ctx->wpe_tiles_key[0] != taps || ctx->wpe_tiles_key[1] != delay ||
        ctx->wpe_tiles_key[2] != D || ctx->wpe_tiles_key[3] != corr_ts + (fold_diag ? 0 : 16) + (corr_pairs ? 32 : 0)) {
        GSS_HIP_CHECK(ctx, hipStreamSynchronize(ctx->stream));
        if (!ctx->wpe_tiles)
            GSS_HIP_CHECK(ctx, hipMalloc(&ctx->wpe_tiles, sizeof(CorrTile) * (1024 + 4096 + 1 + 64)));
        GSS_HIP_CHECK(ctx, hipMemcpy(ctx->wpe_tiles, tiles.data(), sizeof(CorrTile) * ntiles,
                                     hipMemcpyHostToDevice));
        if (!upd.empty())
            GSS_HIP_CHECK(ctx, hipMemcpy(reinterpret_cast<CorrTile *>(ctx->wpe_tiles) + 1024,
                                         upd.data(), sizeof(UpdTile) * upd.size(),
                                         hipMemcpyHostToDevice));
        ctx->wpe_tiles_key[0] = taps;
        ctx->wpe_tiles_key[1] = delay;
        ctx->wpe_tiles_key[2] = D;
        ctx->wpe_tiles_key[3] = corr_ts + (fold_diag ? 0 : 16) + (corr_pairs ? 32 : 0);
    }
    CorrTile *tiles_dev = reinterpret_cast<CorrTile *>(ctx->wpe_tiles);
    UpdTile *upd_dev = reinterpret_cast<UpdTile *>(tiles_dev + 1024);
    int32_t *zero_pivots = reinterpret_cast<int32_t *>(tiles_dev + 1024 + 4096);
    if (part <= 0) GSS_HIP_CHECK(ctx, hipMemsetAsync(zero_pivots, 0, sizeof(int32_t), ctx->stream));
    if (part == 0) GSS_HIP_CHECK(ctx, hipEventRecord(ctx->ev_fork, ctx->stream));
    int *corr_counters = reinterpret_cast<int *>(tiles_dev + 1024 + 4096 + 1) + (part == 1 ? 128 : 0);

    const int padf = corr_padf(D, 16 * corr_ts);
    const size_t corr_lds_probe = sizeof(cplx) * (size_t)(CORR_KT + c + corr_padf(D, 16 * corr_ts)) * D +
                                  sizeof(double) * CORR_KT;
    auto round_eff = [&](int nw) {
        const double wgs = (double)((ntiles + nw - 1) / nw) * F;
        const int by_regs = 16 / nw, by_lds = (int)(160 * 1024 / corr_lds_probe);
        const double rounds = wgs / (256.0 * std::max(1, std::min(by_regs, by_lds)));
        return rounds / std::ceil(rounds);
    };
    int corr_nw = corr_ts == 2 && round_eff(2) > round_eff(4) + 0.15 ? 2 : 4;
    const int nw_forced = gss_variant("corr_nw", 0);
    if (nw_forced) corr_nw = nw_forced == 2 ? 2 : nw_forced == 1 && corr_ts == 1 ? 1 : 4;
    if (corr_ts == 1 && (size_t)(CORR_KT + c + padf) * D <= 512 && !nw_forced) corr_nw = 1;
    const bool corr_stg5 = (size_t)(CORR_KT + c + padf) * D <= 320 && !gss_variant_set("corr_stg8");
    auto corr_fn = corr_ts == 1 && corr_nw == 1 ? (corr_stg5 ? wpe_corr_kernel<1, 1, 5> : wpe_corr_kernel<1, 1>)
                   : corr_ts == 1 ? (corr_nw == 2 ? wpe_corr_kernel<1, 2> : wpe_corr_kernel<1, 4>)
                                  : (corr_nw == 2 ? wpe_corr_kernel<2, 2> : wpe_corr_kernel<2, 4>);
    size_t corr_lds = sizeof(cplx) * (size_t)(CORR_KT + c + padf) * D + sizeof(double) * CORR_KT;
    const int ksplit_forced = gss_variant("corr_ksplit", 0);
    int cus = 0;
    if (array_bins > 0)
        GSS_HIP_CHECK(ctx, hipDeviceGetAttribute(&cus, hipDeviceAttributeMultiprocessorCount, ctx->device));
    const bool arrays_single_waves = array_bins > 0 && (int64_t)ntiles * array_bins >= 4LL * 16 * cus;
    const bool corr_split = ksplit_forced ? ksplit_forced != 1 : !arrays_single_waves;
    const int corr_ks = (corr_ts == 1 && corr_nw == 1 && corr_split)
                            ? (ksplit_forced == 2 ? 2 : 4) : 1;
    using corr_fn_t = void (*)(const cplx *, const double *, int, int64_t, int, int, int, int,
                               const CorrTile *, int, cplx *, cplx *);
    corr_fn_t ksplit_fn = nullptr;
    if (corr_ks > 1) {
        ksplit_fn = corr_stg5 ? (corr_ks == 2 ? wpe_corr_ksplit_kernel<2, 5> : wpe_corr_ksplit_kernel<4, 5>)
                              : (corr_ks == 2 ? wpe_corr_ksplit_kernel<2, 8> : wpe_corr_ksplit_kernel<4, 8>);
        corr_lds = std::max(corr_lds * corr_ks, sizeof(cplx) * 256 * (size_t)(corr_ks - 1));
    }
    const size_t panel_lds = sizeof(cplx) * UDP_SIZE + sizeof(double) * CH_NB;
    constexpr int apply_ta = 2;
    constexpr int apply_nwv = 4;
    const int apply_frames = 16 * apply_ta * apply_nwv;
    auto apply_fn = D <= 16 ? wpe_apply_kernel<apply_ta, 1> : wpe_apply_kernel<apply_ta, 2>;
    if (D >= 4 && !gss_variant_set("apply_generic")) {
        if (n % 8 == 0)
            apply_fn = D <= 16 ? wpe_apply_kernel<apply_ta, 1, 4, 1, false>
                               : wpe_apply_kernel<apply_ta, 2, 4, 1, false>;
        else
            apply_fn = D <= 16 ? wpe_apply_kernel<apply_ta, 1, 4, 1, true>
                               : wpe_apply_kernel<apply_ta, 2, 4, 1, true>;
    }
    const size_t apply_lds = sizeof(cplx) * (size_t)(apply_frames + c + 2) * (D | 1);
    int apply_ph = 1, apply_nt = (D + 15) / 16;
    size_t packed_lds = 0;
    {
        const int ph_env = gss_variant("apply_ph", 0);
        bool ph_env_taken = ph_env <= 1;
        double best = (double)((D + 15) / 16) * n;
        for (int ph = 2; ph <= 4; ++ph) {
            if (ph_env > 0 && ph != ph_env) continue;
            const int nt = (ph * D + 15) / 16;
            if (nt > 3 || D < 2) continue;
            const double cost = (double)nt * (n + (ph - 1) * D) / ph;
            const int fl = 64 * ph + c + 2;
            const size_t lds = sizeof(cplx) * ((size_t)fl * (D | 1) + fl / ph + 1 + (size_t)(n + 1) * (D | 1));
            if (lds > (ph_env == ph ? 160 : 64) * 1024) continue;
            if (cost < 0.75 * best || ph_env == ph) {
                ph_env_taken = ph_env_taken || ph_env == ph;
                best = cost;
                apply_ph = ph;
                apply_nt = nt;
                packed_lds = lds;
            }
        }
        if (ph_env == 1) apply_ph = 1;
        if (!ph_env_taken) {
            static bool warned = false;
            if (!warned)
                fprintf(stderr, "libgss_hip: GSS_VARIANT apply_ph=%d is not available for D=%d taps=%d "
                                "(column tiles or LDS); using the default\n", ph_env, D, taps);
            warned = true;
        }
    }
    using apply_packed_t = void (*)(const cplx *, const cplx *, int, int64_t, int, int, int, cplx *);
    apply_packed_t packed_fn = nullptr;
    const bool apply_gglobal = apply_ph == 1 && D > 16 && 2 * D <= 48 && D % 4 == 0 && n % 4 == 0 &&
                               gss_variant_set("apply_gglobal") && gss_variant("apply_ph", 0) == 0 &&
                               !gss_variant_set("apply_generic");
    if (apply_gglobal) {
        apply_ph = 2;
        apply_nt = 3;
        const int fl = 64 * 2 + c + 2;
        packed_lds = sizeof(cplx) * ((size_t)fl * (D | 1) + fl / 2 + 1);
        packed_fn = wpe_apply_packed_kernel<2, 3, false>;
    } else
    if (apply_ph > 1) {
        static const apply_packed_t table[3][3] = {
            {wpe_apply_packed_kernel<2, 1>, wpe_apply_packed_kernel<2, 2>, wpe_apply_packed_kernel<2, 3>},
            {wpe_apply_packed_kernel<3, 1>, wpe_apply_packed_kernel<3, 2>, wpe_apply_packed_kernel<3, 3>},
            {wpe_apply_packed_kernel<4, 1>, wpe_apply_packed_kernel<4, 2>, wpe_apply_packed_kernel<4, 3>}};
        packed_fn = table[apply_ph - 2][apply_nt - 1];
        static const apply_packed_t table_small[3][3] = {
            {wpe_apply_packed_kernel<2, 1, true, 4, 1>, wpe_apply_packed_kernel<2, 2, true, 4, 1>, wpe_apply_packed_kernel<2, 3, true, 4, 1>},
            {wpe_apply_packed_kernel<3, 1, true, 4, 1>, wpe_apply_packed_kernel<3, 2, true, 4, 1>, wpe_apply_packed_kernel<3, 3, true, 4, 1>},
            {wpe_apply_packed_kernel<4, 1, true, 4, 1>, wpe_apply_packed_kernel<4, 2, true, 4, 1>, wpe_apply_packed_kernel<4, 3, true, 4, 1>}};
        if ((64 * apply_ph + c + 2) * D <= 4 * 256 && n * D <= 256 && !gss_variant_set("apply_generic"))
            packed_fn = table_small[apply_ph - 2][apply_nt - 1];
        if (packed_lds > 64 * 1024)
            GSS_HIP_CHECK(ctx, hipFuncSetAttribute(reinterpret_cast<const void *>(packed_fn),
                                                   hipFuncAttributeMaxDynamicSharedMemorySize,
                                                   (int)packed_lds));
    }
    GSS_REQUIRE(ctx, corr_lds <= 160 * 1024 && apply_lds <= 160 * 1024, GSS_ERR_UNSUPPORTED,
                "wpe: taps=%d D=%d needs more LDS than a CU has", taps, D);
    if (apply_lds > 64 * 1024)
        GSS_HIP_CHECK(ctx, hipFuncSetAttribute(reinterpret_cast<const void *>(apply_fn),
                                               hipFuncAttributeMaxDynamicSharedMemorySize,
                                               (int)apply_lds));
    if (corr_lds > 64 * 1024)
        GSS_HIP_CHECK(ctx, hipFuncSetAttribute(reinterpret_cast<const void *>(corr_fn),
                                               hipFuncAttributeMaxDynamicSharedMemorySize,
                                               (int)corr_lds));
    const int corr_pieces = (int)(((size_t)(CORR_KT + c + padf) * D + 63) / 64);
    const size_t corr_dma_lds = 2 * (sizeof(cplx) * 64 * (size_t)corr_pieces + sizeof(double) * CORR_KT);
    const bool corr_persist = corr_ts == 2 && (int64_t)T * D * 16 < (1LL << 31) &&
                              corr_dma_lds <= 80 * 1024;
    if (corr_persist && !nw_forced) corr_nw = 4;
    const bool corr_blocked = corr_persist && gss_variant_set("corr_blocked");
    auto corr_persist_fn = corr_blocked ? (corr_nw == 2 ? wpe_corr_persist_kernel<2, true>
                                                        : wpe_corr_persist_kernel<4, true>)
                                        : (corr_nw == 2 ? wpe_corr_persist_kernel<2>
                                                        : wpe_corr_persist_kernel<4>);
    CorrQueue corr_queue{(ntiles + corr_nw - 1) / corr_nw, 0};
    int corr_slots = 0;
    if (corr_persist) {
        for (int g = 0; g < corr_queue.ngroups; ++g)
            if (__builtin_popcount(tiles[g * corr_nw].mask) >= 3) corr_queue.gh = g + 1;
        if (corr_dma_lds > 64 * 1024)
            GSS_HIP_CHECK(ctx, hipFuncSetAttribute(reinterpret_cast<const void *>(corr_persist_fn),
                                                   hipFuncAttributeMaxDynamicSharedMemorySize,
                                                   (int)corr_dma_lds));
        int per_cu = 0, cus = 0;
        GSS_HIP_CHECK(ctx, hipOccupancyMaxActiveBlocksPerMultiprocessor(
                               &per_cu, reinterpret_cast<const void *>(corr_persist_fn), 64 * corr_nw,
                               corr_dma_lds));
        GSS_HIP_CHECK(ctx, hipDeviceGetAttribute(&cus, hipDeviceAttributeMultiprocessorCount, ctx->device));
        corr_slots = std::min(std::max(per_cu, 1) * cus, corr_queue.ngroups * F);
    }

    for (int it = 0; it < iterations; ++it) {
        const cplx *cur = it == 0 ? Y : X;
        {
            GSS_PROF(ctx, "wpe_power");
            GSS_TRY(wpe_power_launch(ctx, cur, F, T, D, psd_context, raw, w));
        }
        if (corr_persist) {
            GSS_HIP_CHECK(ctx, hipMemsetAsync(corr_counters, 0, 8 * 16 * sizeof(int), ctx->stream));
            GSS_PROF(ctx, "wpe_corr");
            hipLaunchKernelGGL(corr_persist_fn, dim3(corr_slots), dim3(64 * corr_nw), corr_dma_lds,
                               ctx->stream, Y, w, F, T, D, n, c, corr_pieces, tiles_dev, ntiles,
                               corr_queue, corr_counters, R, P);
            GSS_LAUNCH_CHECK(ctx, "wpe_corr_persist_kernel");
        } else {
            GSS_PROF(ctx, "wpe_corr");
            if (ksplit_fn)
                hipLaunchKernelGGL(ksplit_fn, dim3(xcd_grid(ntiles, F)), dim3(64 * corr_ks), corr_lds,
                                   ctx->stream, Y, w, F, T, D, n, c, padf, tiles_dev, ntiles, R, P);
            else
                hipLaunchKernelGGL(corr_fn, dim3(xcd_grid((ntiles + corr_nw - 1) / corr_nw, F)),
                                   dim3(64 * corr_nw), corr_lds,
                                   ctx->stream, Y, w, F, T, D, n, c, padf, tiles_dev, ntiles, R, P);
            GSS_LAUNCH_CHECK(ctx, "wpe_corr_kernel");
        }
        {
            const int nblk = (n + CH_NB - 1) / CH_NB;
            const bool detail = gss_variant_set("prof_detail");
            static const char *trsm_names[] = {"wpe_chol_trsm_J0", "wpe_chol_trsm_J1", "wpe_chol_trsm_J2",
                                               "wpe_chol_trsm_J3", "wpe_chol_trsm_J4", "wpe_chol_trsm_J5+"};
            static const char *upd_names[] = {"wpe_chol_update_J0", "wpe_chol_update_J1", "wpe_chol_update_J2",
                                              "wpe_chol_update_J3", "wpe_chol_update_J4", "wpe_chol_update_J5+"};
            for (int J = 0; J < nblk; ++J) {
                const int j0 = J * CH_NB, nb = std::min(CH_NB, n - j0);
                if (J == 0 || upd_ndiag[J - 1] == 0) {
                    GSS_PROF(ctx, "wpe_chol_diag");
                    hipLaunchKernelGGL(chol_diag_kernel, dim3(F), dim3(256), 0, ctx->stream, R, n, j0,
                                       zero_pivots);
                    GSS_LAUNCH_CHECK(ctx, "chol_diag_kernel");
                }
                {
                    GSS_PROF(ctx, detail ? trsm_names[std::min(J, 5)] : "wpe_chol_trsm");
                    const int npanel = (n - j0 - nb + 15) / 16 + (D + 15) / 16;
                    hipLaunchKernelGGL(chol_trsm_kernel, dim3(xcd_grid((npanel + 3) / 4, F)),
                                       dim3(256), panel_lds, ctx->stream, R, P, F, n, D, j0);
                    GSS_LAUNCH_CHECK(ctx, "chol_trsm_kernel");
                }
                const int nupd = upd_count[J];
                if (nupd > 0) {
                    GSS_PROF(ctx, detail ? upd_names[std::min(J, 5)] : "wpe_chol_update");
                    const int ndiag = upd_ndiag[J];
                    const dim3 g((ndiag > 0 ? (F + 7) / 8 * 8 : 0) +
                                 xcd_grid((nupd - ndiag + UPD_WAVES - 1) / UPD_WAVES, F)), b(64 * UPD_WAVES);
                    const UpdTile *tl = upd_dev + upd_start[J];
                    hipLaunchKernelGGL((chol_update_kernel<1, 1, true>), g, b, 0, ctx->stream, R, P, F, n, D, upd_j0[J],
                                       std::min(upd_k[J], n - upd_j0[J]), tl, nupd, ndiag,
                                       (J + 1) * CH_NB, zero_pivots);
                    GSS_LAUNCH_CHECK(ctx, "chol_update_kernel");
                }
            }
            {
                GSS_PROF(ctx, "wpe_backsolve");
                hipLaunchKernelGGL(chol_backsolve_kernel, dim3(F), dim3(256), 0, ctx->stream, R, P, n,
                                   D);
                GSS_LAUNCH_CHECK(ctx, "chol_backsolve_kernel");
            }
        }
        {
            GSS_PROF(ctx, "wpe_apply");
            if (packed_fn) {
                const int wg_frames = 64 * apply_ph;
                hipLaunchKernelGGL(packed_fn, dim3(xcd_grid((int)((T + wg_frames - 1) / wg_frames), F)),
                                   dim3(256), packed_lds, ctx->stream, Y, P, F, T, D, n, c, X);
            } else {
                hipLaunchKernelGGL(apply_fn,
                                   dim3(xcd_grid((int)((T + apply_frames - 1) / apply_frames), F)),
                                   dim3(64 * apply_nwv), apply_lds, ctx->stream, Y, P, F, T, D, n, c, X);
            }
            GSS_LAUNCH_CHECK(ctx, "wpe_apply_kernel");
        }
    }
    if (part < 0)
        GSS_HIP_CHECK(ctx, hipMemcpyAsync(ctx->status_host + 2, zero_pivots, sizeof(int32_t),
                                          hipMemcpyDeviceToHost, ctx->stream));
    return GSS_OK;
}


int wpe_copy_zero_pivots(gss_ctx *ctx) {
    if (!ctx->wpe_tiles) return GSS_OK;
    const int32_t *zero_pivots =
        reinterpret_cast<const int32_t *>(reinterpret_cast<const CorrTile *>(ctx->wpe_tiles) + 1024 + 4096);
    GSS_HIP_CHECK(ctx, hipMemcpyAsync(ctx->status_host + 2, zero_pivots, sizeof(int32_t),
                                      hipMemcpyDeviceToHost, ctx->stream));
    return GSS_OK;
}

int selftest_mfma_run(gss_ctx *ctx) {
    double *out = nullptr;
    GSS_HIP_CHECK(ctx, hipMalloc(reinterpret_cast<void **>(&out), sizeof(double) * 256));
    hipLaunchKernelGGL(mfma_selftest_kernel, dim3(1), dim3(64), 0, ctx->stream, out);
    double host[256];
    hipError_t e = hipMemcpyAsync(host, out, sizeof(host), hipMemcpyDeviceToHost, ctx->stream);
    if (e == hipSuccess) e = hipStreamSynchronize(ctx->stream);
    (void)hipFree(out);
    if (e != hipSuccess) return gss_fail(ctx, GSS_ERR_HIP, "mfma selftest: %s", hipGetErrorString(e));
    for (int i = 0; i < 16; ++i)
        for (int j = 0; j < 16; ++j) {
            const double want = (double)(i + 1) * 100.0 * (double)(j + 1);
            if (host[i * 16 + j] != want)
                return gss_fail(ctx, GSS_ERR_UNSUPPORTED,
                                "f64 MFMA fragment layout mismatch at (%d,%d): got %g want %g", i,
                                j, host[i * 16 + j], want);
        }
    return GSS_OK;
}
```

Measured before the change: 1095.

## Restrict prediction to core frames, skip zero-mask tiles, trim per-call memsets

When context frames are dropped, the final CACGMM predict pass now runs only over the core frame range that the beamformer uses. The MVDR PSD accumulation gains a variant that skips tiles whose mask weights are all zero. Several small per-call overheads are also removed: the triangle table is cached across calls, the zero-pivot flag is cleared inside the power kernel, and the persistent correlation kernel resets its own counters, so the memsets are dropped. The risk is that gamma outside the core range is left stale, and the counter self-reset depends on every block reaching the exit path.

```diff
diff --git a/pb_chime5_amd/csrc/cacgmm.hip b/pb_chime5_amd/csrc/cacgmm.hip
--- a/pb_chime5_amd/csrc/cacgmm.hip
+++ b/pb_chime5_amd/csrc/cacgmm.hip
@@ -58,6 +58,7 @@
     int masked;
     double aff_eps;
     MsegPlan mseg;
+    int64_t predict_frames, predict_lo;
 };
 
 template <bool NORMALISE, int NV = 8>
@@ -130,8 +131,9 @@
     const int tl = tid & 63;
     const int g = __builtin_amdgcn_readfirstlane(tid >> 6);
     const int64_t T = a.T;
+    const int64_t TB = MODE == MODE_PREDICT ? a.predict_frames : T;
     const int64_t c0 = (int64_t)chunk * a.chunk_frames;
-    const int64_t c1 = c0 + a.chunk_frames < T ? c0 + a.chunk_frames : T;
+    const int64_t c1 = c0 + a.chunk_frames < TB ? c0 + a.chunk_frames : TB;
     const cplx *Yf = a.Y + (int64_t)f * T * D;
     const cplx *Mf = Mq + (int64_t)f * NE * K;
     const uint8_t *actf = a.act + (int64_t)f * a.act_fstride;
@@ -316,14 +318,15 @@
     constexpr int NE = D * (D + 1) / 2;
     const int64_t T = a.T;
     const int wpb = blockDim.x >> 6;
-    const int ntile = (int)((T + 64 * wpb - 1) / (64 * wpb));
+    const int64_t TB = MODE == MODE_PREDICT ? a.predict_frames : T;
+    const int ntile = (int)((TB + 64 * wpb - 1) / (64 * wpb));
     int f, tile;
     if (!xcd_group_map(ntile, a.F, f, tile)) return;
     const int lane = threadIdx.x & 63;
     const int wave = __builtin_amdgcn_readfirstlane(threadIdx.x >> 6);
     const int64_t t = ((int64_t)tile * wpb + wave) * 64 + lane;
-    const bool valid = t < T;
-    const int64_t tc = valid ? t : T - 1;
+    const bool valid = t < TB;
+    const int64_t tc = valid ? t : TB - 1;
     const cplx *Mf = Mq + (int64_t)f * NE * K;
     const cplx *yf = Yn + (int64_t)f * D * T + tc;
 
@@ -490,7 +493,8 @@
 #define WCOV_T(var)
 #endif
 
-template <int KW, bool NORMALISE, bool SRC_FDT, bool PREFETCH = false, int YP = 8, bool YEXACT = false>
+template <int KW, bool NORMALISE, bool SRC_FDT, bool PREFETCH = false, int YP = 8, bool YEXACT = false,
+          bool SKIPZERO = false>
 __global__ __launch_bounds__(256) void wcov_kernel(const cplx *__restrict__ Y,
                                                    const double *__restrict__ W, int F,
                                                    int64_t T, int D, int NE, int nch,
@@ -607,6 +611,18 @@
             }
             __syncthreads();
             if (PREFETCH && t0 + EM_TILE < c1) prefetch(t0 + EM_TILE);
+        } else if constexpr (SKIPZERO) {
+            static_assert(!NORMALISE, "load_tile<true> has barriers of its own");
+            int nonzero = 0;
+            for (int idx = tid; idx < KW * EM_TILE; idx += blockDim.x) {
+                const int k = idx / EM_TILE, j = idx - k * EM_TILE;
+                const double wv = t0 + j < c1 ? Wf[(int64_t)k * T + t0 + j] : 0.0;
+                wk[idx] = wv;
+                nonzero |= wv != 0.0 ? 1 : 0;
+            }
+            if (!__syncthreads_or(nonzero)) continue;
+            load_tile<NORMALISE, YP>(Yf, D, t0, c1, tl, g, ys, scratch);
+            __syncthreads();
         } else {
             load_tile<NORMALISE, YP>(Yf, D, t0, c1, tl, g, ys, scratch);
             for (int idx = tid; idx < KW * EM_TILE; idx += blockDim.x) {
@@ -1592,10 +1608,20 @@
     return GSS_OK;
 }
 
+EmArgs predict_args(const EmArgs &a) {
+    EmArgs p = a;
+    p.Y += a.predict_lo * a.D;
+    p.act += a.predict_lo;
+    p.gamma += a.predict_lo;
+    return p;
+}
+
 template <int K>
 int launch_estep(gss_ctx *ctx, int mode, const EmArgs &a, const cplx *Mq, int F) {
     const size_t lds = em_estep_lds(a.D, K);
-    dim3 grid(xcd_grid(a.nch, F)), block(256);
+    const int nch = mode == MODE_PREDICT
+                        ? (int)((a.predict_frames + a.chunk_frames - 1) / a.chunk_frames) : a.nch;
+    dim3 grid(xcd_grid(nch, F)), block(256);
     if (mode == MODE_FIRST) {
         GSS_PROF(ctx, "em_estep");
         hipLaunchKernelGGL((em_estep_kernel<K, MODE_FIRST>), grid, block, 0, ctx->stream, a, Mq);
@@ -1605,8 +1631,10 @@
         hipLaunchKernelGGL((em_estep_kernel<K, MODE_EM>), grid, block, lds, ctx->stream, a, Mq);
     } else {
         GSS_TRY(raise_lds_limit(ctx, em_estep_kernel<K, MODE_PREDICT>, lds));
+        EmArgs ap = predict_args(a);
+        ap.nch = nch;
         GSS_PROF(ctx, "em_predict");
-        hipLaunchKernelGGL((em_estep_kernel<K, MODE_PREDICT>), grid, block, lds, ctx->stream, a,
+        hipLaunchKernelGGL((em_estep_kernel<K, MODE_PREDICT>), grid, block, lds, ctx->stream, ap,
                            Mq);
     }
     GSS_LAUNCH_CHECK(ctx, "em_estep_kernel");
@@ -1628,7 +1656,8 @@
 int launch_estep_reg(gss_ctx *ctx, int mode, const EmArgs &a, const cplx *Mq, const cplx *Yn,
                      int F) {
     const int wpb = estep_waves_per_block(F, a.T);
-    const dim3 grid(xcd_grid((int)((a.T + 64 * wpb - 1) / (64 * wpb)), F)), block(64 * wpb);
+    const int64_t frames = mode == MODE_PREDICT ? a.predict_frames : a.T;
+    const dim3 grid(xcd_grid((int)((frames + 64 * wpb - 1) / (64 * wpb)), F)), block(64 * wpb);
     if (mode == MODE_EM) {
         GSS_PROF(ctx, "em_estep");
         hipLaunchKernelGGL((em_estep_reg_kernel<K, D, MODE_EM>), grid, block, 0, ctx->stream, a,
@@ -1636,7 +1665,7 @@
     } else {
         GSS_PROF(ctx, "em_predict");
         hipLaunchKernelGGL((em_estep_reg_kernel<K, D, MODE_PREDICT>), grid, block, 0, ctx->stream,
-                           a, Mq, Yn);
+                           predict_args(a), Mq, Yn + a.predict_lo);
     }
     GSS_LAUNCH_CHECK(ctx, "em_estep_reg_kernel");
     return GSS_OK;
@@ -1823,11 +1852,16 @@
 }
 
 int psd_partials_run(gss_ctx *ctx, const cplx *Y, int F, int64_t T, int D, const double *W2,
-                     int nch, int chunk_frames, cplx *part, int S) {
+                     int nch, int chunk_frames, cplx *part, int S, bool skip_zero_tiles) {
     const size_t lds = wcov_lds_layout(D, 2).total;
-    const wcov_fn_t fn = D <= 4 ? wcov_kernel<2, false, false, false, 1>
-                         : D <= 12 ? wcov_kernel<2, false, false, false, 3>
-                         : D <= 24 ? wcov_kernel<2, false, false, false, 6> : wcov_kernel<2, false, false>;
+    const wcov_fn_t fn =
+        skip_zero_tiles ? (D <= 4 ? wcov_kernel<2, false, false, false, 1, false, true>
+                           : D <= 12 ? wcov_kernel<2, false, false, false, 3, false, true>
+                           : D <= 24 ? wcov_kernel<2, false, false, false, 6, false, true>
+                                     : wcov_kernel<2, false, false, false, 8, false, true>)
+        : D <= 4 ? wcov_kernel<2, false, false, false, 1>
+        : D <= 12 ? wcov_kernel<2, false, false, false, 3>
+        : D <= 24 ? wcov_kernel<2, false, false, false, 6> : wcov_kernel<2, false, false>;
     GSS_TRY(raise_lds_limit(ctx, fn, lds));
     hipLaunchKernelGGL(fn, dim3(xcd_grid(nch, F), S), dim3(256), lds,
                        ctx->stream, Y, W2, F, T, D, tri_count(D), nch, chunk_frames, part, 2, 0,
@@ -1873,13 +1907,20 @@
 }
 
 int cacgmm_run(gss_ctx *ctx, const cplx *Y, int F, int64_t T, int D, const EmGuide &guide, int K,
-               int iterations, int iterations_post, double *gamma) {
+               int iterations, int iterations_post, double *gamma, int64_t predict_lo,
+               int64_t predict_hi) {
     const int NE = tri_count(D);
     const bool reg = estep_reg_supported(D, K) && !gss_variant_set("estep_lds");
     const bool onchip = D == 4 && K >= 2 && K <= 6 && reg && iterations > 0 &&
                         !gss_variant_set("em_unfused");
     const EmBlockPlan bplan = onchip ? EmBlockPlan{F, 1, 1} : em_block_plan(F, T, D, K);
     const EmStrides st = em_strides(bplan, F, T, D);
+    if (predict_hi < 0 || predict_lo < 0 || predict_lo >= predict_hi || predict_hi > T ||
+        bplan.nblocks > 1 || (guide.mask != nullptr && iterations_post == 0) ||
+        gss_variant_set("all_passes")) {
+        predict_lo = 0;
+        predict_hi = T;
+    }
 
     cplx *Mq = arena_alloc_t<cplx>(ctx, (size_t)F * NE * K);
     double *logdet = arena_alloc_t<double>(ctx, (size_t)F * K);
@@ -1906,9 +1947,20 @@
     const int m = D + (D & 1);
     const size_t eigh_lds = (sizeof(cplx) * 2 * m * m + sizeof(double) * m + 15) / 16 * 16;
     const int force_eigh = gss_variant_set("force_eigh");
-    if (!onchip) {
+    if (!onchip && gss_variant_set("all_passes")) {
         hipLaunchKernelGGL(tri_table_kernel, dim3(1), dim3(256), 0, ctx->stream, D, tri_tab);
         GSS_LAUNCH_CHECK(ctx, "tri_table_kernel");
+    } else if (!onchip) {
+        if (!ctx->tri_tab)
+            GSS_HIP_CHECK(ctx, hipMalloc(reinterpret_cast<void **>(&ctx->tri_tab),
+                                         sizeof(int) * 2 * tri_count(GSS_MAX_CHANNELS)));
+        if (ctx->tri_tab_D != D) {
+            GSS_REQUIRE(ctx, D <= GSS_MAX_CHANNELS, GSS_ERR_UNSUPPORTED, "cacgmm: D=%d", D);
+            hipLaunchKernelGGL(tri_table_kernel, dim3(1), dim3(256), 0, ctx->stream, D, ctx->tri_tab);
+            GSS_LAUNCH_CHECK(ctx, "tri_table_kernel");
+            ctx->tri_tab_D = D;
+        }
+        tri_tab = ctx->tri_tab;
     }
 
     auto make_block = [&](int f0, int Fb, hipStream_t stream, EmBlock *blk) -> int {
@@ -1925,6 +1977,8 @@
         a.init_stride = guide.init_k_stride;
         a.init_fstride = guide.init_f_stride;
         a.T = T;
+        a.predict_lo = predict_lo;
+        a.predict_frames = predict_hi - predict_lo;
         a.F = Fb;
         a.D = D;
         a.NE = NE;
diff --git a/pb_chime5_amd/csrc/gss_api.hip b/pb_chime5_amd/csrc/gss_api.hip
--- a/pb_chime5_amd/csrc/gss_api.hip
+++ b/pb_chime5_amd/csrc/gss_api.hip
@@ -35,6 +35,7 @@
 const char *const kVariantKeys[] = {
     "corr_ts", "corr_nw", "corr_blocked", "corr_p_tiles", "chol_diag_unfolded", "apply_ph",
     "apply_generic", "prof_detail", "corr_stg8", "corr_ksplit", "apply_gglobal", "wpe_halves",
+    "all_passes",
     "em_wgs", "estep_wpb", "estep_lds", "mstep_prefetch_d", "mstep_tiled", "mstep_plan_min_d",
     "mstep_chunked", "mstep_slots", "force_eigh", "em_unfused", "em_l3_mb", "em_l3_fit_mb",
     "em_streams", "mstep_maxseg", "em4_cold_eigh", "mstep_generic"};
@@ -183,6 +184,7 @@
     free_tables(ctx);
     if (ctx->arena) (void)hipFree(ctx->arena);
     if (ctx->wpe_tiles) (void)hipFree(ctx->wpe_tiles);
+    if (ctx->tri_tab) (void)hipFree(ctx->tri_tab);
     if (ctx->status_host) (void)hipHostFree(ctx->status_host);
     for (auto &p : ctx->prof_pending) {
         (void)hipEventDestroy(p.start);
@@ -873,7 +875,7 @@
 static int run_front(gss_ctx *ctx, const gss_params *p, const void *obs, int obs_type, int D,
                      int64_t N, const uint8_t *act, int K, int64_t N_act, int F, int64_t T,
                      int64_t T_act, const PipelineFront &fr, size_t mark,
-                     const EmGuide *guide = nullptr) {
+                     const EmGuide *guide = nullptr, int64_t gamma_lo = 0, int64_t gamma_hi = -1) {
     cplx *const Y = fr.Y, *const X = fr.X;
     GSS_TRY(stft_run(ctx, obs, obs_type, D, N, p->stft_fading, Y));
     if (!p->wpe)
@@ -890,9 +892,23 @@
     }
     if (!guide) GSS_TRY(activity_run(ctx, act, K, N_act, p->stft_fading, fr.actf));
     GSS_TRY(cacgmm_run(ctx, X, F, T, D, guide ? *guide : em_guide_from_activity(fr.actf, T_act), K,
-                       p->bss_iterations, p->bss_iterations_post, fr.gamma));
+                       p->bss_iterations, p->bss_iterations_post, fr.gamma, gamma_lo, gamma_hi));
     ctx->arena_off = mark;
     return GSS_OK;
+}
+
+static void mask_core_frames(int drop, int64_t sf, int64_t ef, int64_t T, int64_t *lo, int64_t *hi) {
+    *lo = 0;
+    *hi = T;
+    if (drop) {
+        *lo = sf >= 0 ? (sf < T ? sf : T) : (T + sf > 0 ? T + sf : 0);
+        if (ef > 0) *hi = T - ef > 0 ? T - ef : 0;
+    }
+}
+
+static bool gamma_core_only(const gss_params *p, const gss_debug_taps *taps, int64_t lo, int64_t hi) {
+    return p->bf_drop_context && (p->bf == 0 || p->bf == 3) && !(taps && taps->gamma) && lo < hi &&
+           !gss_variant_set("all_passes");
 }
 
 static int copy_tap(gss_ctx *ctx, void *dst, const void *src, size_t bytes) {
@@ -947,19 +963,24 @@
     int32_t *ref = arena_alloc_t<int32_t>(ctx, 4);
     GSS_REQUIRE(ctx, mx && mn && Xhat && ref, GSS_ERR_NOMEM, "workspace sizing bug");
     const size_t mark = ctx->arena_off;
-    GSS_TRY(run_front(ctx, p, obs, obs_type, D, N, act, K, N_act, F, T, T_act, fr, mark,
-                      guided ? &guide : nullptr));
-    cplx *const X = fr.X;
-
     int64_t sf = 0, ef = 0;
     if (p->bf_drop_context) {
         sf = gss_samples_to_stft_frames(start_ctx, size, shift, fading);
         ef = gss_samples_to_stft_frames(end_ctx, size, shift, fading);
     }
+    int64_t core_lo, core_hi;
+    mask_core_frames(p->bf_drop_context, sf, ef, T, &core_lo, &core_hi);
+    const bool core_only = gamma_core_only(p, taps, core_lo, core_hi);
+    GSS_TRY(run_front(ctx, p, obs, obs_type, D, N, act, K, N_act, F, T, T_act, fr, mark,
+                      guided ? &guide : nullptr, core_only ? core_lo : 0, core_only ? core_hi : -1));
+    cplx *const X = fr.X;
+
     GSS_TRY(masks_from_posteriors_run(ctx, fr.gamma, F, K, T, target, p->bf_drop_context, sf, ef,
                                       mx, mn));
     if (p->bf == 0 || p->bf == 3) {
-        GSS_TRY(mvdr_run(ctx, X, F, T, D, mx, mn, 1, Xhat, ref, p->bf == 3));
+        GSS_TRY(mvdr_run(ctx, X, F, T, D, mx, mn, 1, Xhat, ref, p->bf == 3,
+                         -1, 1, false,
+                         core_only));
         ctx->arena_off = mark;
     } else {
         GSS_TRY(channel_pick_run(ctx, X, F, T, D, p->bf, Xhat));
@@ -1015,9 +1036,6 @@
     int32_t *ref = arena_alloc_t<int32_t>(ctx, 4 * (size_t)S);
     GSS_REQUIRE(ctx, mx && mn && Xhat && ref, GSS_ERR_NOMEM, "workspace sizing bug");
     const size_t mark = ctx->arena_off;
-    GSS_TRY(run_front(ctx, p, obs, obs_type, D, N, act, K, N_act, F, T, T_act, fr, mark));
-    cplx *const X = fr.X;
-
     int64_t sf[GSS_MAX_CLASSES] = {}, ef[GSS_MAX_CLASSES] = {};
     if (p->bf_drop_context) {
         for (int s = 0; s < S; ++s) {
@@ -1025,12 +1043,25 @@
             ef[s] = gss_samples_to_stft_frames(end_ctx[s], size, shift, fading);
         }
     }
+    int64_t hull_lo = T, hull_hi = 0;
+    bool core_only = true;
+    for (int s = 0; s < S; ++s) {
+        int64_t lo, hi;
+        mask_core_frames(p->bf_drop_context, sf[s], ef[s], T, &lo, &hi);
+        core_only = core_only && gamma_core_only(p, taps, lo, hi);
+        hull_lo = std::min(hull_lo, lo);
+        hull_hi = std::max(hull_hi, hi);
+    }
+    GSS_TRY(run_front(ctx, p, obs, obs_type, D, N, act, K, N_act, F, T, T_act, fr, mark, nullptr,
+                      core_only ? hull_lo : 0, core_only ? hull_hi : -1));
+    cplx *const X = fr.X;
+
     GSS_TRY(masks_targets_run(ctx, fr.gamma, F, K, T, S, targets, p->bf_drop_context, sf, ef, mx,
                               mn));
     const bool beamformer = p->bf == 0 || p->bf == 3;
     if (beamformer) {
         GSS_TRY(mvdr_run(ctx, X, F, T, D, mx, mn, 1, Xhat, ref, p->bf == 3,
-                         -1, S, true));
+                         -1, S, true, core_only));
         ctx->arena_off = mark;
         if (p->postfilter == 1)
             GSS_TRY(mask_mul_targets_run(ctx, Xhat, (int64_t)F * T, Xhat, mx, F, T, S, 1));
diff --git a/pb_chime5_amd/csrc/gss_internal.h b/pb_chime5_amd/csrc/gss_internal.h
--- a/pb_chime5_amd/csrc/gss_internal.h
+++ b/pb_chime5_amd/csrc/gss_internal.h
@@ -131,6 +131,9 @@
 
     void *wpe_tiles = nullptr;
     int wpe_tiles_key[4] = {-1, -1, -1, -1};
+    bool corr_counters_clean[2] = {false, false};
+    int *tri_tab = nullptr;
+    int tri_tab_D = -1;
 
     bool profiling = false;
     std::vector<ProfEntry> prof_pending;
@@ -209,15 +212,17 @@
     return EmGuide{nullptr, act, 0, 0, 0, act_stride};
 }
 int cacgmm_run(gss_ctx *ctx, const cplx *Y, int F, int64_t T, int D, const EmGuide &guide, int K,
-               int iterations, int iterations_post, double *gamma);
+               int iterations, int iterations_post, double *gamma, int64_t predict_lo = 0,
+               int64_t predict_hi = -1);
 
 int psd_partials_run(gss_ctx *ctx, const cplx *Y, int F, int64_t T, int D, const double *W2,
-                     int nch, int chunk_frames, cplx *part, int S = 1);
+                     int nch, int chunk_frames, cplx *part, int S = 1,
+                     bool skip_zero_tiles = false);
 
 size_t mvdr_workspace_bytes(int F, int64_t T, int D, int S = 1);
 int mvdr_run(gss_ctx *ctx, const cplx *Y, int F, int64_t T, int D, const double *mx,
              const double *mn, int ban, cplx *Xhat, int32_t *ref_channel, int gev = 0,
-             int forced_ref = -1, int S = 1, bool targets = false);
+             int forced_ref = -1, int S = 1, bool targets = false, bool skip_zero_tiles = false);
 struct TargetMaskArgs {
     int S;
     int target[GSS_MAX_CLASSES];
diff --git a/pb_chime5_amd/csrc/mvdr.hip b/pb_chime5_amd/csrc/mvdr.hip
--- a/pb_chime5_amd/csrc/mvdr.hip
+++ b/pb_chime5_amd/csrc/mvdr.hip
@@ -682,7 +682,7 @@
 
 int mvdr_run(gss_ctx *ctx, const cplx *Y, int F, int64_t T, int D, const double *mx,
              const double *mn, int ban, cplx *Xhat, int32_t *ref_channel, int gev,
-             int forced_ref, int S, bool targets) {
+             int forced_ref, int S, bool targets, bool skip_zero_tiles) {
     const int NE = tri_count(D);
     int cf;
     const int nch = psd_chunks(F, T, &cf);
@@ -701,7 +701,7 @@
         hipLaunchKernelGGL(mask_pack_kernel, dim3(F, S), dim3(256), 0, ctx->stream, mx, mn, T, W2,
                            msum);
         GSS_LAUNCH_CHECK(ctx, "mask_pack_kernel");
-        GSS_TRY(psd_partials_run(ctx, Y, F, T, D, W2, nch, cf, part, S));
+        GSS_TRY(psd_partials_run(ctx, Y, F, T, D, W2, nch, cf, part, S, skip_zero_tiles));
     }
     if (gev) {
         GSS_PROF(ctx, targets ? "gev_solve_targets" : "gev_solve");
diff --git a/pb_chime5_amd/csrc/wpe.hip b/pb_chime5_amd/csrc/wpe.hip
--- a/pb_chime5_amd/csrc/wpe.hip
+++ b/pb_chime5_amd/csrc/wpe.hip
@@ -14,11 +14,13 @@
 __global__ __launch_bounds__(POW_FRAMES) void wpe_power_kernel(const cplx *__restrict__ X,
                                                                int64_t T, int D, int psd_context,
                                                                double *__restrict__ raw,
-                                                               double *__restrict__ w) {
+                                                               double *__restrict__ w,
+                                                               int32_t *__restrict__ zero_word) {
     extern __shared__ __attribute__((aligned(16))) char smem[];
     double *ps = reinterpret_cast<double *>(smem);
     __shared__ double red[POW_FRAMES / 64];
     const int f = blockIdx.x, tid = threadIdx.x;
+    if (zero_word != nullptr && f == 0 && tid == 0) *zero_word = 0;
     const cplx *Xf = X + (int64_t)f * T * D;
     double *wout = w + (int64_t)f * T;
     double *wf = psd_context > 0 ? raw + (int64_t)f * T : wout;
@@ -451,6 +453,16 @@
     return -1;
 }
 
+__device__ __forceinline__ void corr_leave(int *counters) {
+    if (threadIdx.x != 0) return;
+    int *done = counters + 8;
+    __threadfence();
+    if (atomicAdd(done, 1) == (int)gridDim.x - 1) {
+        for (int x = 0; x < 8; ++x) atomicExch(counters + 16 * x, 0);
+        atomicExch(done, 0);
+    }
+}
+
 template <int MASK, int NW, bool BLOCKED, class Issue>
 __device__ __forceinline__ void corr_item_dma(
     int64_t T, int D, int n, int c, int win, cplx *S0, double *w0, const CorrTile tl, bool active,
@@ -592,7 +604,10 @@
     };
 
     int item = __builtin_amdgcn_readfirstlane(ring[0]);
-    if (item < 0) return;
+    if (item < 0) {
+        corr_leave(counters);
+        return;
+    }
     int b = 0;
     issue(item >> 12, 0, 0);
     __syncthreads();
@@ -631,6 +646,7 @@
         }
 #endif
     }
+    corr_leave(counters);
 }
 
 #ifndef GSS_UPD_PREFETCH
@@ -1595,14 +1611,15 @@
 }
 
 static int wpe_power_launch(gss_ctx *ctx, const cplx *cur, int F, int64_t T, int D,
-                            int psd_context, double *raw, double *w) {
+                            int psd_context, double *raw, double *w,
+                            int32_t *zero_word = nullptr) {
     const size_t pow_lds = sizeof(double) * POW_FRAMES * (D + 1);
     if (pow_lds > 64 * 1024)
         GSS_HIP_CHECK(ctx, hipFuncSetAttribute(reinterpret_cast<const void *>(wpe_power_kernel),
                                                hipFuncAttributeMaxDynamicSharedMemorySize,
                                                (int)pow_lds));
     hipLaunchKernelGGL(wpe_power_kernel, dim3(F), dim3(POW_FRAMES), pow_lds, ctx->stream,
-                       cur, T, D, psd_context, raw, w);
+                       cur, T, D, psd_context, raw, w, zero_word);
     GSS_LAUNCH_CHECK(ctx, "wpe_power_kernel");
     return GSS_OK;
 }
@@ -1690,9 +1707,13 @@
     CorrTile *tiles_dev = reinterpret_cast<CorrTile *>(ctx->wpe_tiles);
     UpdTile *upd_dev = reinterpret_cast<UpdTile *>(tiles_dev + 1024);
     int32_t *zero_pivots = reinterpret_cast<int32_t *>(tiles_dev + 1024 + 4096);
-    if (part <= 0) GSS_HIP_CHECK(ctx, hipMemsetAsync(zero_pivots, 0, sizeof(int32_t), ctx->stream));
+    const bool all_passes = gss_variant_set("all_passes");
+    const bool zero_in_power = part < 0 && !all_passes;
+    if (part <= 0 && !zero_in_power)
+        GSS_HIP_CHECK(ctx, hipMemsetAsync(zero_pivots, 0, sizeof(int32_t), ctx->stream));
     if (part == 0) GSS_HIP_CHECK(ctx, hipEventRecord(ctx->ev_fork, ctx->stream));
     int *corr_counters = reinterpret_cast<int *>(tiles_dev + 1024 + 4096 + 1) + (part == 1 ? 128 : 0);
+    bool &counters_clean = ctx->corr_counters_clean[part == 1 ? 1 : 0];
 
     const int padf = corr_padf(D, 16 * corr_ts);
     const size_t corr_lds_probe = sizeof(cplx) * (size_t)(CORR_KT + c + corr_padf(D, 16 * corr_ts)) * D +
@@ -1843,15 +1864,19 @@
         const cplx *cur = it == 0 ? Y : X;
         {
             GSS_PROF(ctx, "wpe_power");
-            GSS_TRY(wpe_power_launch(ctx, cur, F, T, D, psd_context, raw, w));
+            GSS_TRY(wpe_power_launch(ctx, cur, F, T, D, psd_context, raw, w,
+                                     zero_in_power && it == 0 ? zero_pivots : nullptr));
         }
         if (corr_persist) {
-            GSS_HIP_CHECK(ctx, hipMemsetAsync(corr_counters, 0, 8 * 16 * sizeof(int), ctx->stream));
+            if (all_passes || !counters_clean)
+                GSS_HIP_CHECK(ctx, hipMemsetAsync(corr_counters, 0, 8 * 16 * sizeof(int), ctx->stream));
+            counters_clean = false;
             GSS_PROF(ctx, "wpe_corr");
             hipLaunchKernelGGL(corr_persist_fn, dim3(corr_slots), dim3(64 * corr_nw), corr_dma_lds,
                                ctx->stream, Y, w, F, T, D, n, c, corr_pieces, tiles_dev, ntiles,
                                corr_queue, corr_counters, R, P);
             GSS_LAUNCH_CHECK(ctx, "wpe_corr_persist_kernel");
+            counters_clean = true;
         } else {
             GSS_PROF(ctx, "wpe_corr");
             if (ksplit_fn)
```

New measurement: 1099 (median of 6 runs). No clear change (+0.4%).
